# xujiabo/SCREAM

Hardware: AMD Instinct MI355X
Metric: registration pairs/sec (higher is better)
Workload: dtype f32; 1 GPU; BASELINE configs[1]: synthetic 3DMatch_test-like pairs, voxel 0.0625 m, ~5k points/cloud, batch-of-pairs=32 per GPU, A1-A10 per pair (forward 6+6 layers d_model 256, 1-NN thresh 0.1, Kabsch, RE/TE), random-init weights seed 0; lanes=1, steps_in_flight=2, parallelism=dp1 (pairs sharded, metric-row all-gather), rccl_ranks=1, gemm_backend=h2

## Files before the change

### include/scream_hip.h

```cpp
#ifndef SCREAM_HIP_H
#define SCREAM_HIP_H

#include <stdint.h>

#ifdef __cplusplus
extern "C" {
#endif

#define SCREAM_ROW_TILE 128
#define SCREAM_D_MODEL 256
#define SCREAM_NHEAD 8
#define SCREAM_HEAD_DIM 32
#define SCREAM_KV_CHUNK 256

#define SCREAM_EINVAL (-1)
#define SCREAM_EUNSUPPORTED (-2)

enum {
    SCREAM_EPI_NONE = 0,
    SCREAM_EPI_ELU1 = 1,
    SCREAM_EPI_RELU = 2,
    SCREAM_EPI_BIAS_RELU = 3,
    SCREAM_EPI_RES_LN = 4,
    SCREAM_EPI_QKV = 5
};

#define SCREAM_LAYOUT_A_FRAG 1
#define SCREAM_LAYOUT_C_FRAG 2
int scream_act_layout(const float* src, float* dst, int64_t M, int32_t to_fragment, void* stream);

const char* scream_version(void);
int scream_abi_version(void);

int scream_gemm_f32(const float* A, int64_t lda, const float* W, float* C, int64_t ldc,
                    int64_t M, int32_t N, int32_t K, int32_t epilogue, int32_t n_act,
                    const float* bias, const float* residual, int64_t ldr,
                    const float* gamma, const float* beta, void* stream);

int scream_gemm_qkv_f32(const float* A, int64_t lda, const float* W, float* Q, int64_t ldq, int64_t M,
                        int32_t N, int32_t K, int32_t n_q, const int32_t* tile_cloud,
                        const int32_t* cloud_row0, const int32_t* cloud_len, int64_t row_base,
                        float* kv_partial, void* stream);
int scream_kv_finalize(const float* kv_partial, const int32_t* cloud_row0, const int32_t* cloud_len,
                       int64_t row_base, int32_t cloud_begin, int32_t n_kv, float* kv_out, void* stream);

#define SCREAM_SPLIT_H1 1
#define SCREAM_SPLIT_H2 2
#define SCREAM_SPLIT_BF3 3
int scream_pack_w_split(const float* W, int32_t N, int32_t K, int32_t split, int32_t w_exp, void* W_packed,
                        void* stream);
int scream_gemm_split_f32(const float* A, int64_t lda, const void* W_packed, float* C, int64_t ldc, int64_t M,
                          int32_t N, int32_t K, int32_t epilogue, int32_t n_act, const float* bias,
                          const float* residual, int64_t ldr, const float* gamma, const float* beta,
                          int32_t layout, int32_t split, int32_t a_exp, int32_t w_exp, void* stream);
int scream_gemm_qkv_split_f32(const float* A, int64_t lda, const void* W_packed, float* Q, int64_t ldq,
                              int64_t M, int32_t N, int32_t K, int32_t n_q, const int32_t* tile_cloud,
                              const int32_t* cloud_row0, const int32_t* cloud_len, int64_t row_base,
                              float* kv_partial, int32_t layout, int32_t split, int32_t a_exp, int32_t w_exp,
                              int32_t k_exp, int32_t v_exp, void* stream);

int64_t scream_proj_image_bytes(int32_t N, int32_t split);
int scream_pack_proj(const float* W, int32_t N, int32_t n_q, int32_t split, int32_t w_exp, void* proj_image, void* stream);
int scream_proj_qkv_f32(const float* x, const void* proj_image, float* Q, int64_t M, int32_t N, int32_t n_q,
                        const int32_t* tile_cloud, const int32_t* cloud_row0, const int32_t* cloud_len,
                        int64_t row_base, float* kv_partial, int32_t split, int32_t a_exp, int32_t w_exp, int32_t k_exp,
                        int32_t v_exp, void* stream);

typedef struct {
    int32_t e_att, e_wm, e_m1, e_w1, e_h, e_w2;
    int32_t e_y, e_wq;
    int32_t e_q;
} scream_tail_exps_t;
int64_t scream_tail_image_bytes(int32_t split, int32_t with_next_q);
int64_t scream_kv_image_bytes(void);
int scream_pack_tail(const float* Wm, const float* W1, const float* W2, const float* Wq_next, int32_t split,
                     const scream_tail_exps_t* exps, void* tail_image, void* stream);
int scream_kv_finalize_image(const float* kv_partial, const int32_t* cloud_row0, const int32_t* cloud_len,
                          int64_t row_base, int32_t cloud_begin, int32_t n_kv, void* kv_image, int32_t n_layers,
                          int64_t partial_layer_stride, int64_t image_layer_stride, int32_t split, void* stream);
int scream_layer_tail_f32(const float* Q, const void* kv_image, const int32_t* tile_cloud,
                          int32_t kv_cloud_offset, const int32_t* cloud_len, const float* x,
                          const void* tail_image, const float* g1, const float* b1, const float* g2,
                          const float* b2, float* y, float* q_next, int64_t M, int32_t split,
                          const scream_tail_exps_t* exps, void* stream);

int scream_pe_embed_ln(const float* xyz, const int32_t* tile_cloud, const float* center,
                       const float* dim_t, const float* emb_w, const float* emb_b,
                       const float* gamma, const float* beta, float* feats, int64_t rows,
                       void* stream);
int scream_pe_embed_ln_frag(const float* xyz, const int32_t* tile_cloud, const float* center,
                            const float* dim_t, const float* emb_w, const float* emb_b,
                            const float* gamma, const float* beta, float* feats, int64_t rows,
                            void* stream);

int scream_kv_reduce(const float* Kf, const float* Vf, int64_t ld, int64_t row_base,
                     const int32_t* cloud_row0, const int32_t* cloud_len, int32_t cloud_begin,
                     int32_t n_kv, int32_t max_chunks, float* partial, float* kv_out, void* stream);

int scream_attn_apply(const float* Qf, int64_t ldq, const float* kv, const int32_t* tile_cloud,
                      int32_t kv_cloud_offset, const int32_t* cloud_len, float* out, int64_t ldo,
                      int64_t rows, void* stream);

int scream_coor_head(const float* X, const float* W, const float* b, float* out, int64_t rows,
                     void* stream);

typedef struct {
    const float* wqkv;
    const float* wq;
    const float* wkv;
    const float* wm;
    const float* w1;
    const float* w2;
    const float* g1; const float* b1;
    const float* g2; const float* b2;
    const void* tail;
    int32_t e_xq, e_xkv, e_wqkv, e_wq;
    int32_t e_k, e_v;
    scream_tail_exps_t tail_exps;
    int32_t tail_next_q;
    const void* proj;
} scream_layer_t;

typedef struct {
    int32_t n_self;
    int32_t n_cross;
    const float* dim_t;
    const float* emb_w; const float* emb_b;
    const float* pre_g; const float* pre_b;
    const scream_layer_t* layers_host;
    const float* c0_w; const float* c0_b;
    const float* c2_w; const float* c2_b;
    const float* c4_w; const float* c4_b;
    const scream_layer_t* stem_tgt_layers_host;
    int32_t gemm_split;
    int32_t e_c0x, e_c0w, e_c2x, e_c2w;
    const float* wkv_cross;
    int32_t e_wkv_cross, e_k_cross, e_v_cross;
    const void* proj_cross;
} scream_model_t;

typedef struct {
    int32_t n_pairs;
    int64_t rows_src;
    int64_t rows_total;
    int32_t max_chunks;
    const float* xyz;
    const float* center;
    const int32_t* tile_cloud;
    const int32_t* cloud_row0;
    const int32_t* cloud_len;
} scream_batch_t;

int64_t scream_forward_workspace_bytes(int64_t rows_src, int64_t rows_total, int32_t n_pairs,
                                       int32_t max_chunks, int32_t gemm_split, int32_t n_cross);

int scream_forward(const scream_model_t* model, const scream_batch_t* batch, void* workspace,
                   int64_t workspace_bytes, float* src_pred, float* feats_out, void* trace,
                   void* stream);

void* scream_trace_create(int32_t capacity);
void scream_trace_destroy(void* trace);
int scream_trace_reset(void* trace);
int scream_trace_read(void* trace, int32_t max_records, float* ms, int32_t* kind, int64_t* m,
                      int32_t* n, int32_t* k);
int scream_trace_read_starts(void* trace, int32_t max_records, float* start_ms);

int scream_nn_search(const float* query, const float* ref, const int32_t* q_row0,
                     const int32_t* q_len, const int32_t* r_row0, const int32_t* r_len,
                     const float* s, int32_t n_pairs, int32_t max_q_len, int32_t max_r_len,
                     int64_t q_rows_total, int64_t r_rows_total, float thresh, float* ref_prep,
                     uint64_t* keys, int32_t* idx, float* dmin, uint8_t* valid, void* stream);

int scream_square_distance(const float* src, const float* dst, float* out, int32_t B, int32_t N,
                           int32_t M, void* stream);

int scream_kabsch_corr(const float* src, const float* ref, const int32_t* src_row0,
                       const int32_t* src_len, const int32_t* ref_row0, const int32_t* idx,
                       const uint8_t* valid, const float* s, const float* c, int32_t n_pairs,
                       float* T_out, int32_t* n_corr, void* stream);

int scream_rigid_transform_3d(const float* A, const float* B, const float* w,
                              float weight_threshold, int32_t bs, int32_t K, float* T_out,
                              void* stream);

int scream_transformation_error(const float* T_pred, const float* T_gt, int32_t n, float* re,
                                float* te, void* stream);

int scream_point_loss(const float* src_pred, const float* src, const int32_t* src_row0, const int32_t* src_len,
                      const float* rot, const float* trans, int32_t n_pairs, float* loss, void* stream);

int64_t scream_icp_workspace_bytes(int64_t src_rows_total, int64_t ref_rows_total, int32_t n_pairs);
int scream_icp_p2p_range(const float* src, const float* ref, const int32_t* src_row0, const int32_t* src_len,
                         const int32_t* ref_row0, const int32_t* ref_len, const float* s, const float* c,
                         int32_t n_pairs, int32_t max_src_len, int32_t max_ref_len, int64_t src_rows_total,
                         int64_t ref_rows_total, float max_corr_dist, int32_t max_iter, float rel_fitness,
                         float rel_rmse, float* T, float* fitness_rmse, int32_t* iters, int32_t it_begin, int32_t it_end,
                         int32_t* done_flags, void* workspace, int64_t workspace_bytes, void* stream);
int scream_icp_p2p(const float* src, const float* ref, const int32_t* src_row0, const int32_t* src_len,
                   const int32_t* ref_row0, const int32_t* ref_len, const float* s, const float* c,
                   int32_t n_pairs, int32_t max_src_len, int32_t max_ref_len, int64_t src_rows_total,
                   int64_t ref_rows_total, float max_corr_dist, int32_t max_iter, float rel_fitness,
                   float rel_rmse, float* T, float* fitness_rmse, int32_t* iters, void* workspace,
                   int64_t workspace_bytes, void* stream);

int64_t scream_wgrad_workspace_bytes(int64_t rows, int32_t N, int32_t K);
int scream_gemm_wgrad_f32(const float* dY, int64_t ldy, const float* X, int64_t ldx, int64_t rows, int32_t N,
                          int32_t K, float* dW, int32_t accumulate, float* colsum, void* workspace,
                          int64_t workspace_bytes, void* stream);
int64_t scream_wgrad_split_workspace_bytes(int64_t rows, int32_t N, int32_t K);
int scream_gemm_wgrad_split_f32(const float* dY, int64_t ldy, const float* X, int64_t ldx, int64_t rows, int32_t N,
                                int32_t K, float* dW, int32_t accumulate, float* colsum, int32_t split, void* workspace,
                                int64_t workspace_bytes, void* stream);
int scream_ln_fwd(const float* a, const float* b, const float* gamma, const float* beta, float* y, float* mean,
                  float* rstd, int64_t rows, void* stream);
int64_t scream_ln_bwd_workspace_bytes(int64_t rows);
int scream_ln_bwd(const float* dy, const float* a, const float* b, const float* mean, const float* rstd,
                  const float* gamma, float* dz, float* dsum, float* dgamma, float* dbeta, int32_t accumulate,
                  int64_t rows, void* workspace, int64_t workspace_bytes, void* stream);
int64_t scream_attn_bwd_workspace_bytes(int32_t n_q_clouds, int32_t max_chunks);
int scream_attn_bwd(const float* Qf, int64_t ldq, int64_t q_rows, int64_t q_row_base, const float* O,
                    const float* dO, const float* Kf, const float* Vf, int64_t ldkv, int64_t kv_rows,
                    int64_t kv_row_base, const float* kv, const int32_t* tile_cloud, const int32_t* cloud_row0,
                    const int32_t* cloud_len, int32_t q_cloud_begin, int32_t n_q_clouds, int32_t kv_cloud_offset,
                    int32_t max_chunks, float* dq, int64_t lddq, float* dk, float* dv, int64_t lddkv,
                    void* workspace, int64_t workspace_bytes, void* stream);
int scream_relu_bwd(float* dy, const float* y, int64_t n, void* stream);
int scream_add_f32(float* y, const float* x, int64_t n, void* stream);
int scream_transpose_f32(const float* in, int32_t R, int32_t C, float* out, void* stream);
int scream_coor_head_bwd(const float* dout, const float* W, const float* H, float* dH, int64_t rows, void* stream);
int64_t scream_grad3_workspace_bytes(int64_t rows);
int scream_grad3(const float* w, const float* s, const float* center, const int32_t* tile_cloud, int64_t rows,
                 float* dW, int32_t transpose_w, float* col_w, float* col_s, int32_t accumulate, void* workspace,
                 int64_t workspace_bytes, void* stream);
int scream_pe_embed(const float* xyz, const int32_t* tile_cloud, const float* center, const float* dim_t,
                    const float* emb_w, const float* emb_b, float* z, int64_t rows, void* stream);

int64_t scream_render_workspace_bytes(int32_t n_pairs, int32_t n_views, int32_t w, int64_t src_rows_total);
int scream_render_depth(const float* src, const int32_t* s_row0, const int32_t* s_len, const float* tgt,
                        const int32_t* t_row0, const int32_t* t_len, int32_t n_pairs, int32_t max_s_len, int32_t max_t_len,
                        int64_t src_rows_total, const float* rot, int32_t n_views, int32_t w, float rho, float* imgs,
                        int32_t* argmax, void* workspace, int64_t workspace_bytes, void* stream);
int scream_render_depth_bwd(const float* src, const int32_t* s_row0, const int32_t* s_len, int32_t n_pairs, int32_t max_s_len,
                            int64_t src_rows_total, const float* rot, int32_t n_views, int32_t w, float rho,
                            const float* dimgs, const int32_t* argmax, void* workspace, int64_t workspace_bytes, float* dsrc,
                            void* stream);

int64_t scream_voxel_workspace_bytes(int64_t rows_total, int32_t n_clouds);
int scream_voxel_down_sample(const float* xyz, const int32_t* row0, const int32_t* len, int32_t n_clouds, int32_t max_len,
                             const double* voxel, float* out_xyz, int32_t* out_len, int32_t* out_count, void* workspace,
                             int64_t workspace_bytes, void* stream);

int64_t scream_dsm_workspace_bytes(int64_t patch_rows_total, int32_t n_clouds, int32_t max_p_len);
int scream_dsm_extract(const float* patch, const int32_t* p_row0, const int32_t* p_len, int32_t max_p_len,
                       int64_t patch_rows_total, const float* dem, const int32_t* d_row0, const int32_t* d_len, int32_t max_d_len,
                       int64_t dem_rows_total, int32_t n_clouds, float radius, float* out_xyz, int32_t* out_idx, void* workspace,
                       int64_t workspace_bytes, void* stream);
int scream_dsm_dem_assemble(const float* dsm, const float* dem, const int32_t* row0, const int32_t* len, int32_t n_clouds,
                            int32_t max_len, int64_t rows_total, float* out, float* centre, void* stream);

#ifdef __cplusplus
}
#endif
#endif
```

### scream_amd/_lib.py

```python
from __future__ import annotations

import ctypes as C
import os
from typing import Optional

_HERE = os.path.dirname(os.path.abspath(__file__))
LIB_PATH = os.environ.get("SCREAM_LIB") or os.path.join(_HERE, "libscream_hip.so")
ABI_VERSION = 21

c_f32p = C.POINTER(C.c_float)
c_i32p = C.POINTER(C.c_int32)
c_u8p = C.POINTER(C.c_uint8)
c_u64p = C.POINTER(C.c_uint64)


SPLIT_H1, SPLIT_H2, SPLIT_BF3 = 1, 2, 3


class TailExpsT(C.Structure):
    _fields_ = [(n, C.c_int32) for n in ("e_att", "e_wm", "e_m1", "e_w1", "e_h", "e_w2", "e_y", "e_wq", "e_q")]


class LayerT(C.Structure):
    _fields_ = ([(n, C.c_void_p) for n in ("wqkv", "wq", "wkv", "wm", "w1", "w2", "g1", "b1", "g2", "b2", "tail")] +
                [(n, C.c_int32) for n in ("e_xq", "e_xkv", "e_wqkv", "e_wq", "e_k", "e_v")] +
                [("tail_exps", TailExpsT), ("tail_next_q", C.c_int32), ("proj", C.c_void_p)])


class ModelT(C.Structure):
    _fields_ = [("n_self", C.c_int32), ("n_cross", C.c_int32), ("dim_t", C.c_void_p), ("emb_w", C.c_void_p),
                ("emb_b", C.c_void_p), ("pre_g", C.c_void_p), ("pre_b", C.c_void_p),
                ("layers_host", C.POINTER(LayerT)), ("c0_w", C.c_void_p), ("c0_b", C.c_void_p),
                ("c2_w", C.c_void_p), ("c2_b", C.c_void_p), ("c4_w", C.c_void_p), ("c4_b", C.c_void_p),
                ("stem_tgt_layers_host", C.POINTER(LayerT)), ("gemm_split", C.c_int32),
                ("e_c0x", C.c_int32), ("e_c0w", C.c_int32), ("e_c2x", C.c_int32), ("e_c2w", C.c_int32),
                ("wkv_cross", C.c_void_p), ("e_wkv_cross", C.c_int32), ("e_k_cross", C.c_int32), ("e_v_cross", C.c_int32),
                ("proj_cross", C.c_void_p)]


class BatchT(C.Structure):
    _fields_ = [("n_pairs", C.c_int32), ("rows_src", C.c_int64), ("rows_total", C.c_int64),
                ("max_chunks", C.c_int32), ("xyz", C.c_void_p), ("center", C.c_void_p),
                ("tile_cloud", C.c_void_p), ("cloud_row0", C.c_void_p), ("cloud_len", C.c_void_p)]


V, I32, I64, F32 = C.c_void_p, C.c_int32, C.c_int64, C.c_float
SIGNATURES = {
    "scream_version": (C.c_char_p, []),
    "scream_abi_version": (C.c_int, []),
    "scream_gemm_f32": (C.c_int, [V, I64, V, V, I64, I64, I32, I32, I32, I32, V, V, I64, V, V, V]),
    "scream_gemm_qkv_f32": (C.c_int, [V, I64, V, V, I64, I64, I32, I32, I32, V, V, V, I64, V, V]),
    "scream_kv_finalize": (C.c_int, [V, V, V, I64, I32, I32, V, V]),
    "scream_pack_w_split": (C.c_int, [V, I32, I32, I32, I32, V, V]),
    "scream_gemm_split_f32": (C.c_int, [V, I64, V, V, I64, I64, I32, I32, I32, I32, V, V, I64, V, V, I32, I32, I32, I32, V]),
    "scream_gemm_qkv_split_f32": (C.c_int, [V, I64, V, V, I64, I64, I32, I32, I32, V, V, V, I64, V, I32, I32, I32, I32, I32, I32, V]),
    "scream_proj_image_bytes": (C.c_int64, [I32, I32]),
    "scream_pack_proj": (C.c_int, [V, I32, I32, I32, I32, V, V]),
    "scream_proj_qkv_f32": (C.c_int, [V, V, V, I64, I32, I32, V, V, V, I64, V, I32, I32, I32, I32, I32, V]),
    "scream_tail_image_bytes": (C.c_int64, [I32, I32]),
    "scream_kv_image_bytes": (C.c_int64, []),
    "scream_pack_tail": (C.c_int, [V, V, V, V, I32, C.POINTER(TailExpsT), V, V]),
    "scream_kv_finalize_image": (C.c_int, [V, V, V, I64, I32, I32, V, I32, I64, I64, I32, V]),
    "scream_layer_tail_f32": (C.c_int, [V, V, V, I32, V, V, V, V, V, V, V, V, V, I64, I32, C.POINTER(TailExpsT), V]),
    "scream_act_layout": (C.c_int, [V, V, I64, I32, V]),
    "scream_pe_embed_ln": (C.c_int, [V, V, V, V, V, V, V, V, V, I64, V]),
    "scream_pe_embed_ln_frag": (C.c_int, [V, V, V, V, V, V, V, V, V, I64, V]),
    "scream_kv_reduce": (C.c_int, [V, V, I64, I64, V, V, I32, I32, I32, V, V, V]),
    "scream_attn_apply": (C.c_int, [V, I64, V, V, I32, V, V, I64, I64, V]),
    "scream_coor_head": (C.c_int, [V, V, V, V, I64, V]),
    "scream_forward_workspace_bytes": (C.c_int64, [I64, I64, I32, I32, I32, I32]),
    "scream_forward": (C.c_int, [C.POINTER(ModelT), C.POINTER(BatchT), V, I64, V, V, V, V]),
    "scream_trace_create": (C.c_void_p, [I32]),
    "scream_trace_destroy": (None, [V]),
    "scream_trace_reset": (C.c_int, [V]),
    "scream_trace_read": (C.c_int, [V, I32, V, V, V, V, V]),
    "scream_trace_read_starts": (C.c_int, [V, I32, V]),
    "scream_nn_search": (C.c_int, [V, V, V, V, V, V, V, I32, I32, I32, I64, I64, F32, V, V, V, V, V, V]),
    "scream_square_distance": (C.c_int, [V, V, V, I32, I32, I32, V]),
    "scream_kabsch_corr": (C.c_int, [V, V, V, V, V, V, V, V, V, I32, V, V, V]),
    "scream_rigid_transform_3d": (C.c_int, [V, V, V, F32, I32, I32, V, V]),
    "scream_transformation_error": (C.c_int, [V, V, I32, V, V, V]),
    "scream_point_loss": (C.c_int, [V, V, V, V, V, V, I32, V, V]),
    "scream_icp_workspace_bytes": (C.c_int64, [I64, I64, I32]),
    "scream_icp_p2p": (C.c_int, [V, V, V, V, V, V, V, V, I32, I32, I32, I64, I64, F32, I32, F32, F32, V, V, V, V, I64, V]),
    "scream_wgrad_workspace_bytes": (C.c_int64, [I64, I32, I32]),
    "scream_gemm_wgrad_f32": (C.c_int, [V, I64, V, I64, I64, I32, I32, V, I32, V, V, I64, V]),
    "scream_wgrad_split_workspace_bytes": (C.c_int64, [I64, I32, I32]),
    "scream_gemm_wgrad_split_f32": (C.c_int, [V, I64, V, I64, I64, I32, I32, V, I32, V, I32, V, I64, V]),
    "scream_ln_fwd": (C.c_int, [V, V, V, V, V, V, V, I64, V]),
    "scream_ln_bwd_workspace_bytes": (C.c_int64, [I64]),
    "scream_ln_bwd": (C.c_int, [V, V, V, V, V, V, V, V, V, V, I32, I64, V, I64, V]),
    "scream_attn_bwd_workspace_bytes": (C.c_int64, [I32, I32]),
    "scream_attn_bwd": (C.c_int, [V, I64, I64, I64, V, V, V, V, I64, I64, I64, V, V, V, V, I32, I32, I32, I32, V, I64, V, V, I64,
                                  V, I64, V]),
    "scream_relu_bwd": (C.c_int, [V, V, I64, V]),
    "scream_add_f32": (C.c_int, [V, V, I64, V]),
    "scream_transpose_f32": (C.c_int, [V, I32, I32, V, V]),
    "scream_coor_head_bwd": (C.c_int, [V, V, V, V, I64, V]),
    "scream_grad3_workspace_bytes": (C.c_int64, [I64]),
    "scream_grad3": (C.c_int, [V, V, V, V, I64, V, I32, V, V, I32, V, I64, V]),
    "scream_pe_embed": (C.c_int, [V, V, V, V, V, V, V, I64, V]),
    "scream_icp_p2p_range": (C.c_int, [V, V, V, V, V, V, V, V, I32, I32, I32, I64, I64, F32, I32, F32, F32, V, V, V, I32, I32, V, V, I64, V]),
    "scream_render_workspace_bytes": (C.c_int64, [I32, I32, I32, I64]),
    "scream_render_depth": (C.c_int, [V, V, V, V, V, V, I32, I32, I32, I64, V, I32, I32, F32, V, V, V, I64, V]),
    "scream_render_depth_bwd": (C.c_int, [V, V, V, I32, I32, I64, V, I32, I32, F32, V, V, V, I64, V, V]),
    "scream_voxel_workspace_bytes": (C.c_int64, [I64, I32]),
    "scream_voxel_down_sample": (C.c_int, [V, V, V, I32, I32, V, V, V, V, V, I64, V]),
    "scream_dsm_workspace_bytes": (C.c_int64, [I64, I32, I32]),
    "scream_dsm_extract": (C.c_int, [V, V, V, I32, I64, V, V, V, I32, I64, I32, F32, V, V, V, I64, V]),
    "scream_dsm_dem_assemble": (C.c_int, [V, V, V, V, I32, I32, I64, V, V, V]),
}

_lib: Optional[C.CDLL] = None


class ScreamHipError(RuntimeError):
    pass


def load() -> C.CDLL:
    global _lib
    if _lib is not None:
        return _lib
    if os.environ.get("SCREAM_NO_BUILD", "0") != "1" and not os.environ.get("SCREAM_LIB"):
        try:
            from . import build as _build
            _build.build()
        except Exception as e:
            if not os.path.exists(LIB_PATH):
                raise ScreamHipError("libscream_hip.so is missing and could not be built: %s" % e) from e
    if not os.path.exists(LIB_PATH):
        raise ScreamHipError("libscream_hip.so not found at %s (run `python -m scream_amd.build`)" % LIB_PATH)
    lib = C.CDLL(LIB_PATH)
    for name, (res, args) in SIGNATURES.items():
        try:
            fn = getattr(lib, name)
        except AttributeError as e:
            raise ScreamHipError("libscream_hip.so does not export %s" % name) from e
        fn.restype = res
        fn.argtypes = args
    if lib.scream_abi_version() != ABI_VERSION:
        raise ScreamHipError("libscream_hip.so ABI %d != binding ABI %d" % (lib.scream_abi_version(), ABI_VERSION))
    _lib = lib
    return lib


def check(rc: int, what: str) -> None:
    if rc == 0:
        return
    if rc == -1:
        raise ScreamHipError("%s: invalid argument (SCREAM_EINVAL)" % what)
    if rc == -2:
        raise ScreamHipError("%s: unsupported shape (SCREAM_EUNSUPPORTED)" % what)
    raise ScreamHipError("%s: HIP error %d" % (what, rc))
```

### scream_amd/csrc/forward.hip

```cpp
#include <vector>

#include "common.h"

namespace {

constexpr int D = SCREAM_D_MODEL;
constexpr int KV_ELEMS = (SCREAM_HEAD_DIM + 1) * SCREAM_HEAD_DIM;

struct Workspace {
    float *x0, *x1, *q, *att, *m1, *hid, *kvp, *kv;
    char* kvimg;
    float* kvp_cross;
    char* kvimg_cross;
    int64_t kvp_cross_stride, kvimg_cross_stride;
    int64_t bytes;
};

Workspace carve(void* base, int64_t rows_src, int64_t rows_total, int32_t n_pairs, int32_t max_chunks, int split, int32_t n_cross) {
    Workspace w;
    float* p = reinterpret_cast<float*>(base);
    auto take = [&](int64_t n) {
        float* r = p;
        p += (n + 63) / 64 * 64;
        return r;
    };
    const int64_t n_cross_batched = split ? n_cross : 0;
    w.x0 = take(rows_total * D);
    w.x1 = take(rows_total * D);
    w.q = take(rows_total * D);
    w.att = split ? nullptr : take(rows_total * D);
    w.m1 = split ? nullptr : take(rows_total * D);
    w.hid = split ? nullptr : take(rows_total * 4 * D);
    w.kvp = take(rows_total / SCREAM_ROW_TILE * SCREAM_NHEAD * KV_ELEMS);
    w.kv = take((int64_t)2 * n_pairs * SCREAM_NHEAD * KV_ELEMS);
    w.kvimg = reinterpret_cast<char*>(take((int64_t)2 * n_pairs * scream_kv_image_bytes() / 4));
    w.kvp_cross_stride = (rows_total - rows_src) / SCREAM_ROW_TILE * SCREAM_NHEAD * KV_ELEMS;
    w.kvimg_cross_stride = (int64_t)n_pairs * scream_kv_image_bytes();
    w.kvp_cross = take(n_cross_batched * w.kvp_cross_stride);
    w.kvimg_cross = reinterpret_cast<char*>(take(n_cross_batched * w.kvimg_cross_stride / 4));
    w.bytes = (p - reinterpret_cast<float*>(base)) * (int64_t)sizeof(float);
    return w;
}

struct Trace {
    std::vector<hipEvent_t> ev;
    std::vector<int32_t> kind, n, k;
    std::vector<int64_t> m;
    int count = 0;
    int capacity = 0;
};

struct Scope {
    Trace* t;
    int slot = -1;
    hipStream_t st;
    Scope(Trace* t_, int kind, int64_t m, int n, int k, void* stream) : t(t_), st(as_stream(stream)) {
        if (!t || t->count >= t->capacity) return;
        slot = t->count++;
        t->kind[slot] = kind;
        t->m[slot] = m;
        t->n[slot] = n;
        t->k[slot] = k;
        (void)hipEventRecord(t->ev[2 * slot], st);
    }
    ~Scope() {
        if (slot >= 0) (void)hipEventRecord(t->ev[2 * slot + 1], st);
    }
};

#define TRY(call)                 \
    do {                          \
        int rc_ = (call);         \
        if (rc_ != 0) return rc_; \
    } while (0)

enum { TR_TAIL_FUSED = 7, TR_EMBED = 100, TR_KV_REDUCE = 101, TR_ATTN_APPLY = 102, TR_COOR_HEAD = 103 };

struct Ctx {
    void* st;
    Trace* tr;
    int split;
    bool fp16() const { return split == SCREAM_SPLIT_H2 || split == SCREAM_SPLIT_H1; }
};

bool valid_split(int s) { return s == 0 || s == SCREAM_SPLIT_H1 || s == SCREAM_SPLIT_H2 || s == SCREAM_SPLIT_BF3; }

bool layer_ok(const Ctx& c, const scream_layer_t& L, bool cross, bool cross_stage_self) {
    if ((L.tail != nullptr) != (c.split != 0)) return false;
    if ((L.tail_next_q != 0) != (c.fp16() && cross_stage_self)) return false;
    if (c.fp16()) return cross || L.proj;
    if (c.split) return cross ? L.wq != nullptr : L.wqkv != nullptr;
    return L.wm && L.w1 && L.w2 && (cross ? L.wq && L.wkv : L.wqkv != nullptr);
}

bool model_ok(const Ctx& c, const scream_model_t& m) {
    for (int i = 0; i < m.n_self; ++i) {
        if (!layer_ok(c, m.layers_host[i], false, false)) return false;
        if (m.stem_tgt_layers_host && !layer_ok(c, m.stem_tgt_layers_host[i], false, false)) return false;
    }
    for (int i = 0; i < 2 * m.n_cross; ++i)
        if (!layer_ok(c, m.layers_host[m.n_self + i], i % 2 == 1, i % 2 == 0)) return false;
    if (m.n_cross == 0 || c.split == 0) return true;
    return c.fp16() ? m.proj_cross != nullptr : m.wkv_cross != nullptr;
}

int gemm(const Ctx& c, const float* A, int64_t lda, const float* W, float* C, int64_t ldc, int64_t M, int N, int K,
         int epi, int n_act, const float* bias, const float* res, const float* g, const float* b, int a_exp, int w_exp,
         int layout = 0) {
    Scope sc(c.tr, epi, M, N, K, c.st);
    if (c.split)
        return scream_gemm_split_f32(A, lda, W, C, ldc, M, N, K, epi, n_act, bias, res, D, g, b, layout, c.split, a_exp, w_exp, c.st);
    return scream_gemm_f32(A, lda, W, C, ldc, M, N, K, epi, n_act, bias, res, D, g, b, c.st);
}

int gemm_qkv(const Ctx& c, const float* A, const float* W, const void* proj, float* Q, int64_t M, int N, int n_q, const scream_batch_t& b,
             int64_t row_base, float* kvp, int a_exp, int w_exp, int k_exp, int v_exp) {
    Scope sc(c.tr, 5, M, N, D, c.st);
    if (c.fp16())
        return scream_proj_qkv_f32(A, proj, Q, M, N, n_q, b.tile_cloud, b.cloud_row0, b.cloud_len, row_base, kvp, c.split, a_exp, w_exp,
                                   k_exp, v_exp, c.st);
    if (c.split)
        return scream_gemm_qkv_split_f32(A, D, W, Q, D, M, N, D, n_q, b.tile_cloud, b.cloud_row0, b.cloud_len, row_base, kvp,
                                         SCREAM_LAYOUT_A_FRAG | (n_q ? SCREAM_LAYOUT_C_FRAG : 0), c.split, a_exp, w_exp, k_exp, v_exp,
                                         c.st);
    return scream_gemm_qkv_f32(A, D, W, Q, D, M, N, D, n_q, b.tile_cloud, b.cloud_row0, b.cloud_len, row_base, kvp, c.st);
}

int apply_and_tail_f32(const Ctx& c, const scream_layer_t& L, const scream_batch_t& b, const Workspace& w, const float* x, float* y,
                       int64_t row0, int64_t rows, int32_t kv_cloud_offset) {
    float* att = w.att + row0 * D;
    float* m1 = w.m1 + row0 * D;
    float* hid = w.hid + row0 * 4 * D;
    {
        Scope sc(c.tr, TR_ATTN_APPLY, rows, 0, 0, c.st);
        TRY(scream_attn_apply(w.q + row0 * D, D, w.kv, b.tile_cloud + row0 / SCREAM_ROW_TILE, kv_cloud_offset, b.cloud_len, att, D, rows,
                              c.st));
    }
    TRY(gemm(c, att, D, L.wm, m1, D, rows, D, D, SCREAM_EPI_RES_LN, 0, nullptr, x, L.g1, L.b1, 0, 0));
    TRY(gemm(c, m1, D, L.w1, hid, 4 * D, rows, 4 * D, D, SCREAM_EPI_RELU, 0, nullptr, nullptr, nullptr, nullptr, 0, 0));
    TRY(gemm(c, hid, 4 * D, L.w2, y, D, rows, D, 4 * D, SCREAM_EPI_RES_LN, 0, nullptr, x, L.g2, L.b2, 0, 0));
    return 0;
}

int mha_self(const Ctx& c, const scream_layer_t& L, const scream_batch_t& b, const Workspace& w, const float* x,
             float* y, int64_t row0, int64_t rows, int32_t cloud_begin, int32_t n_clouds) {
    const float* xr = x + row0 * D;
    float* qr = w.q + row0 * D;
    float* kvp = w.kvp + row0 / SCREAM_ROW_TILE * SCREAM_NHEAD * KV_ELEMS;
    TRY(gemm_qkv(c, xr, L.wqkv, L.proj, qr, rows, 3 * D, D, b, row0, kvp, L.e_xq, L.e_wqkv, L.e_k, L.e_v));
    if (c.split) {
        {
            Scope sc(c.tr, TR_KV_REDUCE, rows, 0, 0, c.st);
            TRY(scream_kv_finalize_image(kvp, b.cloud_row0, b.cloud_len, row0, cloud_begin, n_clouds, w.kvimg, 1, 0, 0, c.split, c.st));
        }
        Scope sc(c.tr, TR_TAIL_FUSED, rows, (L.tail_next_q ? 10 : 9) * D, D, c.st);
        return scream_layer_tail_f32(qr, w.kvimg, b.tile_cloud + row0 / SCREAM_ROW_TILE, 0, b.cloud_len, xr, L.tail, L.g1,
                                     L.b1, L.g2, L.b2, y + row0 * D, L.tail_next_q ? qr : nullptr, rows, c.split, &L.tail_exps, c.st);
    }
    {
        Scope sc(c.tr, TR_KV_REDUCE, rows, 0, 0, c.st);
        TRY(scream_kv_finalize(kvp, b.cloud_row0, b.cloud_len, row0, cloud_begin, n_clouds, w.kv, c.st));
    }
    return apply_and_tail_f32(c, L, b, w, xr, y + row0 * D, row0, rows, 0);
}

int cross_kv_all(const Ctx& c, const scream_model_t& m, const scream_batch_t& b, const Workspace& w, const float* x_tgt) {
    const int64_t rs = b.rows_src, rt = b.rows_total - b.rows_src;
    const scream_layer_t& L0 = m.layers_host[m.n_self + 1];
    TRY(gemm_qkv(c, x_tgt, m.wkv_cross, m.proj_cross, nullptr, rt, 2 * D * m.n_cross, 0, b, rs, w.kvp_cross, L0.e_xkv, m.e_wkv_cross, m.e_k_cross,
                 m.e_v_cross));
    Scope sc(c.tr, TR_KV_REDUCE, rt, 0, 0, c.st);
    return scream_kv_finalize_image(w.kvp_cross, b.cloud_row0, b.cloud_len, rs, b.n_pairs, b.n_pairs,
                                 w.kvimg_cross - (int64_t)b.n_pairs * scream_kv_image_bytes(), m.n_cross, w.kvp_cross_stride,
                                 w.kvimg_cross_stride, c.split, c.st);
}

int mha_cross(const Ctx& c, const scream_layer_t& L, const scream_batch_t& b, const Workspace& w, const float* x_src,
              const float* x_tgt, float* y, const char* kvimg_layer) {
    const int64_t rs = b.rows_src, rt = b.rows_total - b.rows_src;
    if (!c.fp16())
        TRY(gemm(c, x_src, D, L.wq, w.q, D, rs, D, D, SCREAM_EPI_ELU1, D, nullptr, nullptr, nullptr, nullptr, L.e_xq, L.e_wq,
                 c.split ? (SCREAM_LAYOUT_A_FRAG | SCREAM_LAYOUT_C_FRAG) : 0));
    if (c.split) {
        Scope sc(c.tr, TR_TAIL_FUSED, rs, 9 * D, D, c.st);
        return scream_layer_tail_f32(w.q, kvimg_layer, b.tile_cloud, 0, b.cloud_len + b.n_pairs, x_src, L.tail, L.g1, L.b1, L.g2,
                                     L.b2, y, nullptr, rs, c.split, &L.tail_exps, c.st);
    }
    TRY(gemm_qkv(c, x_tgt, L.wkv, nullptr, nullptr, rt, 2 * D, 0, b, rs, w.kvp, 0, 0, 0, 0));
    {
        Scope sc(c.tr, TR_KV_REDUCE, rt, 0, 0, c.st);
        TRY(scream_kv_finalize(w.kvp, b.cloud_row0, b.cloud_len, rs, b.n_pairs, b.n_pairs, w.kv, c.st));
    }
    return apply_and_tail_f32(c, L, b, w, x_src, y, 0, rs, b.n_pairs);
}

}

extern "C" const char* scream_version(void) { return "scream_hip gfx950 abi21"; }
extern "C" int scream_abi_version(void) { return 21; }

extern "C" void* scream_trace_create(int32_t capacity) {
    if (capacity <= 0) return nullptr;
    Trace* t = new Trace();
    t->capacity = capacity;
    t->ev.resize(2 * (size_t)capacity);
    t->kind.resize(capacity);
    t->n.resize(capacity);
    t->k.resize(capacity);
    t->m.resize(capacity);
    for (auto& e : t->ev) {
        if (hipEventCreate(&e) != hipSuccess) {
            delete t;
            return nullptr;
        }
    }
    return t;
}

extern "C" void scream_trace_destroy(void* trace) {
    Trace* t = reinterpret_cast<Trace*>(trace);
    if (!t) return;
    for (auto& e : t->ev) (void)hipEventDestroy(e);
    delete t;
}

extern "C" int scream_trace_reset(void* trace) {
    SCREAM_REQUIRE(trace, SCREAM_EINVAL);
    reinterpret_cast<Trace*>(trace)->count = 0;
    return 0;
}

extern "C" int scream_trace_read(void* trace, int32_t max_records, float* ms, int32_t* kind, int64_t* m, int32_t* n,
                                 int32_t* k) {
    SCREAM_REQUIRE(trace && ms && kind && m && n && k && max_records >= 0, SCREAM_EINVAL);
    Trace* t = reinterpret_cast<Trace*>(trace);
    const int cnt = t->count < max_records ? t->count : max_records;
    for (int i = 0; i < cnt; ++i) {
        if (hipEventElapsedTime(&ms[i], t->ev[2 * i], t->ev[2 * i + 1]) != hipSuccess) return SCREAM_EINVAL;
        kind[i] = t->kind[i];
        m[i] = t->m[i];
        n[i] = t->n[i];
        k[i] = t->k[i];
    }
    return cnt;
}

extern "C" int scream_trace_read_starts(void* trace, int32_t max_records, float* start_ms) {
    SCREAM_REQUIRE(trace && start_ms && max_records >= 0, SCREAM_EINVAL);
    Trace* t = reinterpret_cast<Trace*>(trace);
    const int cnt = t->count < max_records ? t->count : max_records;
    for (int i = 0; i < cnt; ++i)
        if (hipEventElapsedTime(&start_ms[i], t->ev[0], t->ev[2 * i]) != hipSuccess) return SCREAM_EINVAL;
    return cnt;
}

extern "C" int64_t scream_forward_workspace_bytes(int64_t rows_src, int64_t rows_total, int32_t n_pairs,
                                                  int32_t max_chunks, int32_t gemm_split, int32_t n_cross) {
    if (rows_src < 0 || rows_total < rows_src || n_pairs < 0 || max_chunks < 0 || !valid_split(gemm_split) || n_cross < 0) return SCREAM_EINVAL;
    return carve(nullptr, rows_src, rows_total, n_pairs, max_chunks, gemm_split, n_cross).bytes + 256;
}

extern "C" int scream_forward(const scream_model_t* model, const scream_batch_t* batch, void* workspace,
                              int64_t workspace_bytes, float* src_pred, float* feats_out, void* trace, void* stream) {
    SCREAM_REQUIRE(model && batch && workspace && src_pred, SCREAM_EINVAL);
    const scream_model_t& m = *model;
    const scream_batch_t& b = *batch;
    SCREAM_REQUIRE(m.layers_host && m.n_self >= 0 && m.n_cross >= 0 && valid_split(m.gemm_split), SCREAM_EINVAL);
    SCREAM_REQUIRE(b.n_pairs > 0 && b.rows_src > 0 && b.rows_total > b.rows_src && b.max_chunks > 0, SCREAM_EINVAL);
    SCREAM_REQUIRE(b.rows_src % SCREAM_ROW_TILE == 0 && b.rows_total % SCREAM_ROW_TILE == 0, SCREAM_EUNSUPPORTED);
    SCREAM_REQUIRE(b.xyz && b.center && b.tile_cloud && b.cloud_row0 && b.cloud_len, SCREAM_EINVAL);
    const Ctx c{stream, reinterpret_cast<Trace*>(trace), m.gemm_split};
    SCREAM_REQUIRE(model_ok(c, m), SCREAM_EINVAL);
    uintptr_t base = (reinterpret_cast<uintptr_t>(workspace) + 255) & ~(uintptr_t)255;
    const Workspace w = carve(reinterpret_cast<void*>(base), b.rows_src, b.rows_total, b.n_pairs, b.max_chunks, c.split, m.n_cross);
    SCREAM_REQUIRE((int64_t)(base - reinterpret_cast<uintptr_t>(workspace)) + w.bytes <= workspace_bytes, SCREAM_EINVAL);

    const int64_t rs = b.rows_src, ra = b.rows_total;
    {
        Scope sc(c.tr, TR_EMBED, ra, 0, 0, stream);
        if (c.split)
            TRY(scream_pe_embed_ln_frag(b.xyz, b.tile_cloud, b.center, m.dim_t, m.emb_w, m.emb_b, m.pre_g, m.pre_b, w.x0, ra, stream));
        else
            TRY(scream_pe_embed_ln(b.xyz, b.tile_cloud, b.center, m.dim_t, m.emb_w, m.emb_b, m.pre_g, m.pre_b, w.x0, ra, stream));
    }
    float* cur = w.x0;
    float* nxt = w.x1;
    for (int i = 0; i < m.n_self; ++i) {
        if (!m.stem_tgt_layers_host) {
            TRY(mha_self(c, m.layers_host[i], b, w, cur, nxt, 0, ra, 0, 2 * b.n_pairs));
        } else {
            TRY(mha_self(c, m.layers_host[i], b, w, cur, nxt, 0, rs, 0, b.n_pairs));
            TRY(mha_self(c, m.stem_tgt_layers_host[i], b, w, cur, nxt, rs, ra - rs, b.n_pairs, b.n_pairs));
        }
        float* t = cur;
        cur = nxt;
        nxt = t;
    }
    const float* x_tgt = cur + rs * D;
    if (c.split && m.n_cross > 0) TRY(cross_kv_all(c, m, b, w, x_tgt));
    for (int i = 0; i < 2 * m.n_cross; ++i) {
        const scream_layer_t& L = m.layers_host[m.n_self + i];
        if (i % 2 == 0)
            TRY(mha_self(c, L, b, w, cur, nxt, 0, rs, 0, b.n_pairs));
        else
            TRY(mha_cross(c, L, b, w, cur, x_tgt, nxt, c.split ? w.kvimg_cross + (i / 2) * w.kvimg_cross_stride : nullptr));
        float* t = cur;
        cur = nxt;
        nxt = t;
    }
    float* c_mid = c.split ? w.q : w.m1;
    float* c_out = c.split ? nxt : w.att;
    TRY(gemm(c, cur, D, m.c0_w, c_mid, D, rs, D, D, SCREAM_EPI_BIAS_RELU, 0, m.c0_b, nullptr, nullptr, nullptr, m.e_c0x, m.e_c0w,
             c.split ? SCREAM_LAYOUT_A_FRAG : 0));
    TRY(gemm(c, c_mid, D, m.c2_w, c_out, D, rs, D, D, SCREAM_EPI_BIAS_RELU, 0, m.c2_b, nullptr, nullptr, nullptr, m.e_c2x, m.e_c2w));
    {
        Scope sc(c.tr, TR_COOR_HEAD, rs, 0, 0, stream);
        TRY(scream_coor_head(c_out, m.c4_w, m.c4_b, src_pred, rs, stream));
    }
    if (feats_out && c.split) {
        TRY(scream_act_layout(cur, feats_out, rs, 0, stream));
    } else if (feats_out) {
        hipError_t e = hipMemcpyAsync(feats_out, cur, (size_t)rs * D * sizeof(float), hipMemcpyDeviceToDevice,
                                      as_stream(stream));
        if (e != hipSuccess) return (int)e;
    }
    return 0;
}
```

### scream_amd/csrc/tail_split.hip

```cpp
#include <type_traits>

#include "ring.h"

namespace {

constexpr int T_RIDE0 = 3;
constexpr int T_STASH = 3;
constexpr int T_DEFER_H2 = 2;

constexpr int TAIL_STAGES = 72;
constexpr int NEXT_Q_STAGES = 8;
constexpr int KV_PLANES_BYTES = 8 * 3 * 2 * 1024;
constexpr int KV_IMAGE_BYTES = KV_PLANES_BYTES + 8 * 32 * 4;

constexpr int KV_H2_HEAD_BYTES = 2 * 2 * 1024;
constexpr int KV_H2_SCALE_OFF = 8 * KV_H2_HEAD_BYTES;

struct HeadOps {
    f32x4 kv[6];
    f32x4 ks[4];
    f32x4 sc;
};

struct TailScales {
    float s_att;
    int e_q;
    int e_att;
    float c1;
    float eps1;
    float s_m1;
    float ch;
    float c2;
    float eps2;
    float s_y;
    float cq;
};

__device__ __forceinline__ constexpr int xadd_slot(int h, int g, int nd) {
    int n = 0;
    for (int c = 15 - nd; c >= 8; --c) {
        if ((c >> 1) == h - 1) continue;
        if (c == g) return n < 4 ? n : -1;
        ++n;
    }
    return -1;
}

template <class SP, bool NQ>
__global__ __launch_bounds__(TT, 1) void tail_kernel(const float* __restrict__ Q,
                                                     const char* __restrict__ kvimg,
                                                     const int32_t* __restrict__ tile_cloud, int kv_cloud_offset,
                                                     const int32_t* __restrict__ cloud_len,
                                                     const float* __restrict__ xres,
                                                     const char* __restrict__ Wimg,
                                                     const float* __restrict__ g1, const float* __restrict__ b1,
                                                     const float* __restrict__ g2, const float* __restrict__ b2,
                                                     float* __restrict__ y,
                                                     float* q_next,
                                                     int n_tiles, TailScales sc) {
    static_assert(!NQ || SP::SCALED, "the next-layer query projection is built for the fp16 splits");
    constexpr int N_STAGES = TAIL_STAGES + (NQ ? NEXT_Q_STAGES : 0);
    typedef typename SP::vec V;
    constexpr int NP = SP::NP;
    constexpr int STAGE = stage_bytes<SP>();
    constexpr int PIECES = wave_pieces<SP>();
    constexpr bool APPLY_H2 = SP::SCALED;
    constexpr int NV_MERGE = SP::NPROD >= 6 ? 6 : 8;
    constexpr int ND = SP::NPROD >= 6 ? 1 : T_DEFER_H2;
    constexpr int NG = 16 - ND;
    constexpr int NSTASH = NP == 2 ? T_STASH : 0;
    __shared__ __attribute__((aligned(16))) char smem[T_SLOTS * STAGE + 4096 + NSTASH * 16384];
    const int tid = threadIdx.x, lane = tid & 63;
    const int wave = __builtin_amdgcn_readfirstlane(tid >> 6);
    const int half = lane >> 5;
    float* lnp = reinterpret_cast<float*>(smem + T_SLOTS * STAGE);
    f32x4* stash = reinterpret_cast<f32x4*>(smem + T_SLOTS * STAGE + 4096 + wave * (NSTASH * 4096)) + lane;
    lnp[tid] = SP::SCALED ? g1[tid] * sc.s_m1 : g1[tid];
    lnp[256 + tid] = SP::SCALED ? b1[tid] * sc.s_m1 : b1[tid];
    lnp[512 + tid] = g2[tid];
    lnp[768 + tid] = b2[tid];
    const float eps1 = SP::SCALED ? sc.eps1 : 1e-5f, eps2 = SP::SCALED ? sc.eps2 : 1e-5f;
    const unsigned v_lane16 = lane * 16, v_half16 = half * 16;
    auto dma_piece = [&](unsigned q, int u) {
        const unsigned src = q % (unsigned)N_STAGES, slot = q % (unsigned)T_SLOTS;
        const char* sbase = Wimg + (size_t)src * STAGE + (wave * PIECES + (u & ~3)) * 1024;
        dma_1k(sbase + v_lane16, smem + slot * STAGE + (wave * PIECES + (u & ~3)) * 1024, u & 3);
    };
    unsigned q = 0;
#pragma unroll
    for (int u = 0; u < PIECES; ++u) dma_piece(0, u);
#pragma unroll
    for (int u = 0; u < PIECES; ++u) dma_piece(1, u);

    auto seg_base = [&](const float* base, int64_t grp, int seg) { return base + grp + seg * 1024; };
    auto req_q = [&](f32x4 (&qb)[4], int64_t grp, int h) {
        ld_asm4<1024, true>(qb, seg_base(Q, grp, h), v_lane16);
    };
    auto req_head = [&](HeadOps& o, const char* kvc, int h) {
        f32x4 (&kv4)[4] = reinterpret_cast<f32x4 (&)[4]>(o.kv[0]);
        if (APPLY_H2) {
            ld_asm4<1024>(kv4, kvc + h * KV_H2_HEAD_BYTES, v_lane16);
            asm volatile("global_load_dwordx4 %0, %1, %2" : "=v"(o.sc) : "v"(v_half16), "s"(kvc + KV_H2_SCALE_OFF + 32 * h));
        } else {
            const char* kp = kvc + h * (3 * 2 * 1024);
            ld_asm4<1024>(kv4, kp, v_lane16);
            ld_asm2k(o.kv[4], o.kv[5], kp + 4 * 1024, v_lane16);
        }
        ld_asm4<32>(o.ks, kvc + KV_PLANES_BYTES + 128 * h, v_half16);
    };
    auto req_x = [&](f32x4 (&xs)[4], int64_t grp, int blk, auto second) {
        ld_asm4<1024, decltype(second)::value>(xs, seg_base(xres, grp, blk), v_lane16);
    };
    auto pin_head = [&](HeadOps& o) {
#pragma unroll
        for (int a = 0; a < 4; ++a) pin(o.ks[a]);
#pragma unroll
        for (int f = 0; f < (APPLY_H2 ? 4 : 6); ++f) pin(o.kv[f]);
        if (APPLY_H2) pin(o.sc);
    };
    auto add_x4 = [&](f32x16& t, const f32x4 (&xs)[4], int a, float c) {
#pragma unroll
        for (int k = 0; k < 4; ++k) t[4 * a + k] = SP::SCALED ? __builtin_fmaf(xs[a][k], c, t[4 * a + k]) : t[4 * a + k] + xs[a][k];
    };
    auto pin_x = [&](f32x4 (&xs)[4]) {
#pragma unroll
        for (int a = 0; a < 4; ++a) pin(xs[a]);
    };
    auto add_x = [&](f32x16& t, const f32x4 (&xs)[4], float c) {
#pragma unroll
        for (int a = 0; a < 4; ++a) add_x4(t, xs, a, c);
    };

    HeadOps op;
    f32x4 qA[4], qB[4];
    f32x4 xs[4], xs2[4];
    V apA[2][NP], apB[2][NP];
    f32x16 aT;
    bf16x8 qp[2][3];
    f16x8 qph[2][2];
    float Zs = 0.f;
    int tq = 0;

    auto apply_qscale = [&](const f32x4 (&qb)[4]) {
        float m = 0.f;
#pragma unroll
        for (int a = 0; a < 4; ++a)
#pragma unroll
            for (int k = 0; k < 4; ++k) m = fmaxf(m, qb[a][k]);
        m = fmaxf(m, __shfl_xor(m, 32));
        const int hb = (int)(__float_as_uint(op.sc[0]) >> 23);
        tq = min(max(14 - ((int)(__float_as_uint(m) >> 23) - 127), sc.e_q), min(127, sc.e_att + hb - 1));
    };
    auto apply_qsplit = [&](f32x4 (&qb)[4], int s2) {
        const f32x4 lo = qb[2 * s2], hi = qb[2 * s2 + 1];
        if (APPLY_H2) split8s<SplitH2>(lo, hi, __uint_as_float((uint32_t)(tq + 127) << 23), qph[s2]);
        else split8<SplitBf3>(lo, hi, qp[s2]);
    };
    auto apply_mfma = [&](int s2) {
        if (APPLY_H2) {
            f16x8 w[2];
#pragma unroll
            for (int p = 0; p < 2; ++p) w[p] = __builtin_bit_cast(f16x8, op.kv[p * 2 + s2]);
            mfma_group<SplitH2, -1>(aT, w, qph[s2], s2 == 0);
        } else {
            bf16x8 w[3];
#pragma unroll
            for (int p = 0; p < 3; ++p) w[p] = __builtin_bit_cast(bf16x8, op.kv[p * 2 + s2]);
            mfma_group<SplitBf3, -1>(aT, w, qp[s2], s2 == 0);
        }
    };
    auto apply_z = [&](f32x4 (&qb)[4]) {
        float zp = 0.f;
#pragma unroll
        for (int a = 0; a < 4; ++a)
#pragma unroll
            for (int k = 0; k < 4; ++k) zp += qb[a][k] * op.ks[a][k];
        zp += __shfl_xor(zp, 32);
        Zs = 1.0f / (zp + 1e-6f);
        if (APPLY_H2) Zs *= __uint_as_float((uint32_t)(sc.e_att - tq + (int)(__float_as_uint(op.sc[0]) >> 23)) << 23);
        else if (SP::SCALED) Zs *= sc.s_att;
    };
    auto apply_split_pair = [&](int k, V (&ap)[2][NP], float S) {
        const int s2 = k >> 2, j = (2 * k) & 7;
#pragma unroll
        for (int e = 0; e < 2; ++e) SP::split1((aT[2 * k + e] * Zs) * S, j + e, ap[s2]);
    };
    auto apply_ride = [&](f32x4 (&qb)[4], int g, V (&ap)[2][NP], float S) {
        if (g == 0 && APPLY_H2) apply_qscale(qb);
        if (g == 0) apply_qsplit(qb, 0);
        if (g == 1) apply_qsplit(qb, 1);
        if (g == 1) apply_mfma(0);
        if (g == 2) apply_mfma(1);
        if (g == 3) apply_z(qb);
        if (g >= 4 && g < 12) apply_split_pair(g - 4, ap, S);
    };

    int tile = blockIdx.x;
    int64_t grp = ((int64_t)tile * 128 + wave * 32) * SCREAM_D_MODEL;
    const char* kvc = nullptr;
    float S = 1.f;
    if (tile < n_tiles) {
        const int cl = tile_cloud[tile] + kv_cloud_offset;
        kvc = kvimg + (size_t)cl * KV_IMAGE_BYTES;
        S = (float)cloud_len[cl];
    }
    if (tile < n_tiles) {
#pragma unroll
        for (int h = 0; h < 2; ++h) {
            req_q(qA, grp, h);
            req_head(op, kvc, h);
            VM_WAIT(0);
            pin_x(qA);
            pin_head(op);
#pragma unroll
            for (int g = 0; g < 12; ++g) apply_ride(qA, g, h == 0 ? apA : apB, S);
        }
    }

    while (tile < n_tiles) {
        V wfd[ND][NP];
        f32x16 acc[8];
        auto ring_groups = [&](auto flush, auto body) __attribute__((always_inline)) {
            const char* wb = smem + (q % T_SLOTS) * STAGE + lane * 16;
            V wf[T_PF][NP];
#pragma unroll
            for (int g0 = 0; g0 < T_PF - 1; ++g0)
#pragma unroll
                for (int p = 0; p < NP; ++p) wf[g0][p] = ld_frag<V>(wb + (p * 16 + g0) * 1024);
            flush();
#pragma unroll
            for (int g = 0; g < NG; ++g) {
                if (g + T_PF - 1 < 16) {
#pragma unroll
                    for (int p = 0; p < NP; ++p)
                        (g + T_PF - 1 >= NG ? wfd[g + T_PF - 1 - NG][p] : wf[(g + T_PF - 1) % T_PF][p]) = ld_frag<V>(wb + (p * 16 + g + T_PF - 1) * 1024);
                }
                body(g, wf[g % T_PF]);
            }
            ++q;
        };
        const int tile_next = tile + (int)gridDim.x;
        const bool has_next = tile_next < n_tiles;
        const int64_t grp_next = ((int64_t)(has_next ? tile_next : tile) * 128 + wave * 32) * SCREAM_D_MODEL;
        const char* kvc_next = kvc;
        float S_next = 1.f;
        if (has_next) {
            const int cl = tile_cloud[tile_next] + kv_cloud_offset;
            kvc_next = kvimg + (size_t)cl * KV_IMAGE_BYTES;
            S_next = (float)cloud_len[cl];
        }

        auto stage_merge = [&](auto hh, V (&ap)[2][NP], V (&ap_next)[2][NP], f32x4 (&q_cons)[4], f32x4 (&q_req)[4], auto flush) {
            constexpr int h = decltype(hh)::value;
            constexpr bool RIDE = h >= 1 && h <= 6;
            if (h == 0) { if (NQ) ring_barrier<0>(); else lds_only_barrier(); }
            else ring_barrier<PIECES>();
            __builtin_amdgcn_sched_barrier(0);
            f32x4 (&x_prev)[4] = (h & 1) ? xs : xs2;
            f32x4 (&x_req)[4] = (h & 1) ? xs2 : xs;
            if (h > 0) {
                pin_x(x_prev);
                if (h - 1 < NSTASH) {
#pragma unroll
                    for (int a = 0; a < 4; ++a) stash[((h - 1) * 4 + a) * 64] = x_prev[a];
                }
                if (RIDE) {
                    pin_head(op);
                    pin_x(q_cons);
                }
            }
            __builtin_amdgcn_sched_barrier(0);
            req_x(x_req, grp, h, std::false_type{});
            if (h + 2 < 8) req_q(q_req, grp, h + 2);
            if (h == 0) req_head(op, kvc, 2);
            __builtin_amdgcn_sched_barrier(0);
            ring_groups(flush, [&](int g, const V (&w)[NP]) __attribute__((always_inline)) {
                if (g == 4 && RIDE && h + 2 < 8) {
                    __builtin_amdgcn_sched_barrier(0);
                    req_head(op, kvc, h + 2);
                    __builtin_amdgcn_sched_barrier(0);
                }
                if (g >= 4 && g - 4 < PIECES) dma_piece(q + 2, g - 4);
                if (PIECES == 12 && g == 14) dma_piece(q + 2, 11);
                if (RIDE) apply_ride(q_cons, g, ap_next, S);
                if (h > 0) {
                    const int pc = xadd_slot(h, g, ND);
                    if (pc >= 0) add_x4(acc[h > 0 ? h - 1 : 0], x_prev, pc, sc.c1);
                }
                mfma_group<SP, (h > 0 ? NV_MERGE : 0)>(acc[g >> 1], w, ap[g & 1], h == 0 && (g & 1) == 0);
            });
        };
        constexpr std::integral_constant<bool, true> yes{};
        constexpr std::integral_constant<bool, false> no{};
#define HEAD(n) std::integral_constant<int, n>{}
        auto flush_none = [&]() {};
        auto flush_acc7 = [&](V (&b)[2][NP], bool first) {
#pragma unroll
            for (int i = 0; i < ND; ++i) mfma_group<SP, -1>(acc[7], wfd[i], b[(NG + i) & 1], first && ((NG + i) & 1) == 0);
        };
        auto flush_mergeA = [&]() { flush_acc7(apA, false); };
        auto flush_mergeB = [&]() { flush_acc7(apB, false); };
        auto flush_mergeA0 = [&]() { flush_acc7(apA, true); };
        stage_merge(HEAD(0), apA, apB, qB, qA, flush_none);
        stage_merge(HEAD(1), apB, apA, qA, qB, flush_mergeA0);
        stage_merge(HEAD(2), apA, apB, qB, qA, flush_mergeB);
        stage_merge(HEAD(3), apB, apA, qA, qB, flush_mergeA);
        stage_merge(HEAD(4), apA, apB, qB, qA, flush_mergeB);
        stage_merge(HEAD(5), apB, apA, qA, qB, flush_mergeA);
        stage_merge(HEAD(6), apA, apB, qB, qA, flush_mergeB);
        stage_merge(HEAD(7), apB, apA, qA, qB, flush_mergeA);
        flush_mergeB();
        vm_wait<PIECES>();
        pin_x(xs2);
        add_x(acc[7], xs2, sc.c1);

        V mp[16][NP];
        {
            float sum = 0.f;
#pragma unroll
            for (int b = 0; b < 8; ++b)
#pragma unroll
                for (int e = 0; e < 16; ++e) sum += acc[b][e];
            sum += __shfl_xor(sum, 32);
            const float mean = sum * (1.0f / 256.0f);
            float var = 0.f;
#pragma unroll
            for (int b = 0; b < 8; ++b)
#pragma unroll
                for (int e = 0; e < 16; ++e) {
                    acc[b][e] -= mean;
                    var += acc[b][e] * acc[b][e];
                }
            var += __shfl_xor(var, 32);
            const float rstd = 1.0f / sqrtf(var * (1.0f / 256.0f) + eps1);
            const float* gp = lnp + 4 * half;
            const float* bp = lnp + 256 + 4 * half;
#pragma unroll
            for (int b = 0; b < 8; ++b)
#pragma unroll
                for (int s2 = 0; s2 < 2; ++s2) {
                    f32x4 v[2];
#pragma unroll
                    for (int a2 = 0; a2 < 2; ++a2) {
                        const int a = 2 * s2 + a2;
                        const f32x4 g4 = ld4(gp + 32 * b + 8 * a), b4 = ld4(bp + 32 * b + 8 * a);
#pragma unroll
                        for (int k = 0; k < 4; ++k) v[a2][k] = acc[b][4 * a + k] * rstd * g4[k] + b4[k];
                    }
                    split8<SP>(v[0], v[1], mp[2 * b + s2]);
                }
        }

        f32x16 hT;
        V hpA[2][NP], hpB[2][NP];
        auto split_pair = [&](int k, V (&hout)[2][NP]) {
            const int s2 = k >> 2, j = (2 * k) & 7;
            float x0, x1;
            asm("v_max_f32 %0, 0, %1" : "=v"(x0) : "v"(hT[2 * k]));
            asm("v_max_f32 %0, 0, %1" : "=v"(x1) : "v"(hT[2 * k + 1]));
            if constexpr (SP::SCALED) {
                SP::split2s(x0, x1, sc.ch, j, hout[s2]);
            } else {
                SP::split1(x0, j, hout[s2]);
                SP::split1(x1, j + 1, hout[s2]);
            }
        };
        auto stage_up = [&](auto first, auto xload, auto flush) {
            constexpr int XLOAD = decltype(xload)::value;
            if (decltype(first)::value) ring_barrier<0>(); else ring_barrier<PIECES>();
            __builtin_amdgcn_sched_barrier(0);
            if (XLOAD >= 0 && XLOAD < NSTASH) {
#pragma unroll
                for (int a = 0; a < 4; ++a) xs[a] = stash[(XLOAD * 4 + a) * 64];
            } else if (XLOAD >= 0) req_x(xs, grp, XLOAD, std::true_type{});
            __builtin_amdgcn_sched_barrier(0);
            ring_groups(flush, [&](int g, const V (&w)[NP]) __attribute__((always_inline)) {
                if (g < PIECES) dma_piece(q + 2, g);
                mfma_group<SP>(hT, w, mp[g], g == 0);
            });
        };
        auto stage_down = [&](V (&hin)[2][NP], V (&hout)[2][NP], auto with_split, auto xadd, auto ride, auto flush) {
            constexpr int XADD = decltype(xadd)::value;
            constexpr int RIDE = decltype(ride)::value;
            ring_barrier<PIECES>();
            __builtin_amdgcn_sched_barrier(0);
            if (XADD == 0) {
                pin_x(xs);
#pragma unroll
                for (int a = 0; a < 4; ++a)
#pragma unroll
                    for (int k = 0; k < 4; ++k) acc[0][4 * a + k] = SP::SCALED ? xs[a][k] * sc.c2 : xs[a][k];
            } else if (XADD > 0) {
                pin_x(xs);
                add_x(acc[XADD > 0 ? XADD : 0], xs, sc.c2);
            }
            if (RIDE == 2) {
                pin_head(op);
                pin_x(qA);
            }
            __builtin_amdgcn_sched_barrier(0);
            if (RIDE == 1) {
                req_q(qA, grp_next, 0);
                req_head(op, kvc_next, 0);
            }
            __builtin_amdgcn_sched_barrier(0);
            ring_groups(flush, [&](int g, const V (&w)[NP]) __attribute__((always_inline)) {
                if (RIDE == 2 && g == 4) {
                    __builtin_amdgcn_sched_barrier(0);
                    req_q(qA, grp_next, 1);
                    req_head(op, kvc_next, 1);
                    __builtin_amdgcn_sched_barrier(0);
                }
                if (RIDE == 2) {
                    if (g >= 4 && g - 4 < PIECES) dma_piece(q + 2, g - 4);
                    if (PIECES == 12 && g == 14) dma_piece(q + 2, 11);
                } else {
                    if (g < PIECES) dma_piece(q + 2, g);
                }
                if (RIDE == 2) apply_ride(qA, g, apA, S_next);
                if (decltype(with_split)::value && (ND == 1 ? (g & 1) == 0 : (g >= T_RIDE0 && g < T_RIDE0 + 8))) split_pair(ND == 1 ? g >> 1 : g - T_RIDE0, hout);
                mfma_group<SP>(acc[g >> 1], w, hin[g & 1], XADD == 0 && g >= 2 && (g & 1) == 0);
            });
        };
        constexpr std::integral_constant<int, -1> none{};
        constexpr std::integral_constant<int, 0> ride0{};
        auto flush_up = [&]() {
#pragma unroll
            for (int i = 0; i < ND; ++i) mfma_group<SP, -1>(hT, wfd[i], mp[NG + i]);
        };
        auto flush_downA = [&]() { flush_acc7(hpA, false); };
        auto flush_downB = [&]() { flush_acc7(hpB, false); };
        auto flush_downA0 = [&]() { flush_acc7(hpA, true); };
        stage_up(yes, none, flush_none);
        flush_up();
#pragma unroll
        for (int k = 0; k < 8; ++k) split_pair(k, hpA);
#define PAIR(c, fl, flA)                                                                    \
        stage_up(no, HEAD((c) - 1), fl);                                        \
        stage_down(hpA, hpB, yes, HEAD((c) - 1), ride0, flush_up);  \
        stage_up(no, HEAD(c), flA);                                         \
        stage_down(hpB, hpA, yes, HEAD(c), ride0, flush_up);
        PAIR(1, flush_none, flush_downA0) PAIR(3, flush_downB, flush_downA) PAIR(5, flush_downB, flush_downA) PAIR(7, flush_downB, flush_downA)
#undef PAIR
        for (int c = 9; c < 31; c += 2) {
            stage_up(no, none, flush_downB);
            stage_down(hpA, hpB, yes, none, ride0, flush_up);
            stage_up(no, none, flush_downA);
            stage_down(hpB, hpA, yes, none, ride0, flush_up);
        }
        stage_up(no, none, flush_downB);
        stage_down(hpA, hpB, yes, none, HEAD(1), flush_up);
        stage_down(hpB, hpA, no, none, HEAD(2), flush_downA);
        flush_downB();
#undef HEAD
        VM_WAIT(0);
        if (has_next) {
            pin_head(op);
            pin_x(qA);
#pragma unroll
            for (int g = 0; g < 12; ++g) apply_ride(qA, g, apB, S_next);
        }

        V yp[NQ ? 16 : 1][NP];
        {
            float sum = 0.f;
#pragma unroll
            for (int b = 0; b < 8; ++b)
#pragma unroll
                for (int e = 0; e < 16; ++e) sum += acc[b][e];
            sum += __shfl_xor(sum, 32);
            const float mean = sum * (1.0f / 256.0f);
            float var = 0.f;
#pragma unroll
            for (int b = 0; b < 8; ++b)
#pragma unroll
                for (int e = 0; e < 16; ++e) {
                    acc[b][e] -= mean;
                    var += acc[b][e] * acc[b][e];
                }
            var += __shfl_xor(var, 32);
            const float rstd = 1.0f / sqrtf(var * (1.0f / 256.0f) + eps2);
            const float* gp = lnp + 512 + 4 * half;
            const float* bp = lnp + 768 + 4 * half;
            float* yg = y + grp + lane * 4;
#pragma unroll
            for (int b = 0; b < 8; ++b)
#pragma unroll
                for (int s2 = 0; s2 < 2; ++s2) {
                    f32x4 o2[2];
#pragma unroll
                    for (int a2 = 0; a2 < 2; ++a2) {
                        const int a = 2 * s2 + a2;
                        const f32x4 g4 = ld4(gp + 32 * b + 8 * a), b4 = ld4(bp + 32 * b + 8 * a);
                        f32x4 o;
#pragma unroll
                        for (int k = 0; k < 4; ++k) o[k] = acc[b][4 * a + k] * rstd * g4[k] + b4[k];
                        __builtin_nontemporal_store(o, reinterpret_cast<f32x4*>(yg + (b * 4 + a) * 256));
                        o2[a2] = o;
                    }
                    if (NQ) split8<SP>(o2[0] * sc.s_y, o2[1] * sc.s_y, yp[NQ ? 2 * b + s2 : 0]);
                }
        }
        if constexpr (NQ) {
            f32x16 hq[2];
            f32x4 oq[4];
            float* qg = q_next + grp + lane * 4;
            auto elu_pair = [&](int k, const f32x16& h) {
#pragma unroll
                for (int e = 0; e < 2; ++e) {
                    const int i = 2 * k + e;
                    const float x = h[i] * sc.cq;
                    oq[i >> 2][i & 3] = elu1(x);
                }
            };
            auto store_chunk = [&](int j) {
#pragma unroll
                for (int a = 0; a < 4; ++a) __builtin_nontemporal_store(oq[a], reinterpret_cast<f32x4*>(qg + (j * 4 + a) * 256));
            };
            constexpr int PP = (PIECES + NG - 9) / (NG - 8);
            auto stage_q = [&](auto jj) {
                constexpr int j = decltype(jj)::value;
                if (j == 0) lds_only_barrier(); else ring_barrier<PIECES>();
                __builtin_amdgcn_sched_barrier(0);
                auto flush_q = [&]() {
                    if (j > 0) {
#pragma unroll
                        for (int i = 0; i < ND; ++i) mfma_group<SP, -1>(hq[(j + 1) & 1], wfd[i], yp[NG + i]);
                    }
                };
                ring_groups(flush_q, [&](int g, const V (&w)[NP]) __attribute__((always_inline)) {
                    if (j > 0 && g < 8) elu_pair(g, hq[(j + 1) & 1]);
                    if (g == 8) {
                        __builtin_amdgcn_sched_barrier(0);
                        if (j > 0) store_chunk(j - 1);
                        __builtin_amdgcn_sched_barrier(0);
                    }
                    if (g >= 8) {
#pragma unroll
                        for (int u = (g - 8) * PP; u < (g - 7) * PP; ++u)
                            if (u < PIECES) dma_piece(q + 2, u);
                    }
                    mfma_group<SP, 8>(hq[j & 1], w, yp[g], g == 0);
                });
            };
            stage_q(std::integral_constant<int, 0>{});
            stage_q(std::integral_constant<int, 1>{});
            stage_q(std::integral_constant<int, 2>{});
            stage_q(std::integral_constant<int, 3>{});
            stage_q(std::integral_constant<int, 4>{});
            stage_q(std::integral_constant<int, 5>{});
            stage_q(std::integral_constant<int, 6>{});
            stage_q(std::integral_constant<int, 7>{});
#pragma unroll
            for (int i = 0; i < ND; ++i) mfma_group<SP, -1>(hq[1], wfd[i], yp[NG + i]);
#pragma unroll
            for (int k = 0; k < 8; ++k) elu_pair(k, hq[1]);
            store_chunk(7);
        }
        tile = tile_next;
        grp = ((int64_t)tile_next * 128 + wave * 32) * SCREAM_D_MODEL;
        kvc = kvc_next;
        S = S_next;
    }
    VM_WAIT(0);
}

__global__ __launch_bounds__(256) void act_layout_kernel(const float* __restrict__ src, float* __restrict__ dst, int to_frag) {
    __shared__ float tile[32][260];
    const int t = threadIdx.x;
    const float* s = src + (int64_t)blockIdx.x * 8192;
    float* d = dst + (int64_t)blockIdx.x * 8192;
#pragma unroll
    for (int i = 0; i < 8; ++i) {
        const int e = t + 256 * i;
        const f32x4 v = *reinterpret_cast<const f32x4*>(s + e * 4);
        int row, col;
        if (to_frag) {
            row = e >> 6, col = (e & 63) * 4;
        } else {
            const int ln = e & 63, a = (e >> 6) & 3, blk = e >> 8;
            row = ln & 31, col = 32 * blk + 8 * a + 4 * (ln >> 5);
        }
        *reinterpret_cast<f32x4*>(&tile[row][col]) = v;
    }
    __syncthreads();
#pragma unroll
    for (int i = 0; i < 8; ++i) {
        const int e = t + 256 * i;
        int row, col;
        if (to_frag) {
            const int ln = e & 63, a = (e >> 6) & 3, blk = e >> 8;
            row = ln & 31, col = 32 * blk + 8 * a + 4 * (ln >> 5);
        } else {
            row = e >> 6, col = (e & 63) * 4;
        }
        *reinterpret_cast<f32x4*>(d + e * 4) = *reinterpret_cast<const f32x4*>(&tile[row][col]);
    }
}

template <class SP>
__global__ void pack_tail_kernel(const float* __restrict__ Wm, const float* __restrict__ W1, const float* __restrict__ W2,
                                 const float* __restrict__ Wq_next, float s_wm, float s_w1, float s_w2, float s_wq,
                                 typename SP::vec* __restrict__ out) {
    const int t = blockIdx.x * blockDim.x + threadIdx.x;
    if (t >= (TAIL_STAGES + (Wq_next ? NEXT_Q_STAGES : 0)) * 16 * 64) return;
    const int lane = t & 63, frag = (t >> 6) & 15, stage = t >> 10;
    const int m = lane & 31, half = lane >> 5;
    float v[8];
    float s;
    if (stage < 8) {
        s = s_wm;
#pragma unroll
        for (int j = 0; j < 8; ++j) v[j] = Wm[(int64_t)(32 * (frag >> 1) + m) * 256 + 32 * stage + chunk_k(frag & 1, half, j)];
    } else if (stage >= TAIL_STAGES) {
        s = s_wq;
#pragma unroll
        for (int j = 0; j < 8; ++j) v[j] = Wq_next[(int64_t)(32 * (stage - TAIL_STAGES) + m) * 256 + 32 * (frag >> 1) + chunk_k(frag & 1, half, j)];
    } else {
        const int st = stage - 8;
        const bool up = st == 0 || (st < 63 && (st & 1));
        const int c = st == 0 ? 0 : st == 63 ? 31 : up ? (st + 1) / 2 : st / 2 - 1;
        s = up ? s_w1 : s_w2;
        if (up) {
#pragma unroll
            for (int j = 0; j < 8; ++j) v[j] = W1[(int64_t)(32 * c + m) * 256 + 32 * (frag >> 1) + chunk_k(frag & 1, half, j)];
        } else {
#pragma unroll
            for (int j = 0; j < 8; ++j) v[j] = W2[(int64_t)(32 * (frag >> 1) + m) * 1024 + 32 * c + chunk_k(frag & 1, half, j)];
        }
    }
    typename SP::vec p[SP::NP];
#pragma unroll
    for (int j = 0; j < 8; ++j) SP::split1(SP::SCALED ? v[j] * s : v[j], j, p);
#pragma unroll
    for (int pl = 0; pl < SP::NP; ++pl) out[(((int64_t)stage * SP::NP + pl) * 16 + frag) * 64 + lane] = p[pl];
}

constexpr int KVF_THREADS = 320;

template <bool H2>
__global__ __launch_bounds__(KVF_THREADS) void kv_finalize_image_kernel(const float* __restrict__ partial,
                                                                      const int32_t* __restrict__ cloud_row0,
                                                                      const int32_t* __restrict__ cloud_len, int64_t row_base,
                                                                      int cloud_begin, char* __restrict__ kvimg,
                                                                      int64_t partial_layer_stride, int64_t image_layer_stride) {
    constexpr int KV_ELEMS = (SCREAM_HEAD_DIM + 1) * SCREAM_HEAD_DIM;
    static_assert(KV_ELEMS % 4 == 0 && KV_ELEMS / 4 <= KVF_THREADS, "");
    __shared__ float wmax[KVF_THREADS / 64];
    const int i4 = threadIdx.x;
    const bool active = i4 < KV_ELEMS / 4;
    const int kvi = blockIdx.x / SCREAM_NHEAD, h = blockIdx.x % SCREAM_NHEAD;
    const int cloud = cloud_begin + kvi;
    partial += (int64_t)blockIdx.y * partial_layer_stride;
    kvimg += (int64_t)blockIdx.y * image_layer_stride;
    const int t0 = (int)((cloud_row0[cloud] - row_base) / SCREAM_ROW_TILE);
    const int nt = (cloud_len[cloud] + SCREAM_ROW_TILE - 1) / SCREAM_ROW_TILE;
    const float* p = partial + ((int64_t)t0 * SCREAM_NHEAD + h) * KV_ELEMS + 4 * (active ? i4 : 0);
    char* img = kvimg + (size_t)cloud * KV_IMAGE_BYTES;
    const float S = (float)cloud_len[cloud];
    f32x4 s8[16];
#pragma unroll
    for (int u = 0; u < 16; ++u) s8[u] = f32x4{0.f, 0.f, 0.f, 0.f};
    if (active) {
        for (int c = 0; c < nt; c += 16) {
#pragma unroll
            for (int u = 0; u < 16; ++u)
                if (c + u < nt) s8[u] += *reinterpret_cast<const f32x4*>(p + (int64_t)(c + u) * SCREAM_NHEAD * KV_ELEMS);
        }
    }
#pragma unroll
    for (int u = 0; u < 8; ++u) s8[u] += s8[u + 8];
    const f32x4 s4 = ((s8[0] + s8[1]) + (s8[2] + s8[3])) + ((s8[4] + s8[5]) + (s8[6] + s8[7]));
    const bool is_kv = 4 * i4 < 32 * 32;
    f32x4 x4;
#pragma unroll
    for (int e = 0; e < 4; ++e) x4[e] = s4[e] / S;
    float scale = 1.f;
    if (H2) {
        float m = (active && is_kv) ? fmaxf(fmaxf(fabsf(x4[0]), fabsf(x4[1])), fmaxf(fabsf(x4[2]), fabsf(x4[3]))) : 0.f;
#pragma unroll
        for (int o = 32; o >= 1; o >>= 1) m = fmaxf(m, __shfl_xor(m, o));
        if ((threadIdx.x & 63) == 0) wmax[threadIdx.x >> 6] = m;
        __syncthreads();
        m = wmax[0];
#pragma unroll
        for (int w = 1; w < KVF_THREADS / 64; ++w) m = fmaxf(m, wmax[w]);
        const uint32_t mb = __float_as_uint(m);
        int eh = 15 - ((int)(mb >> 23) - 127) - ((mb & 0x7fffffu) ? 1 : 0);
        if (!(m >= 1.17549435e-38f) || eh > 40) eh = 40;
        if (eh < -30) eh = -30;
        scale = __uint_as_float((uint32_t)(eh + 127) << 23);
        if (threadIdx.x < 8) reinterpret_cast<float*>(img + KV_H2_SCALE_OFF)[h * 8 + threadIdx.x] = __uint_as_float((uint32_t)(127 - eh) << 23);
    }
    if (!active) return;
#pragma unroll
    for (int e = 0; e < 4; ++e) {
        const int i = 4 * i4 + e;
        if (is_kv) {
            const int d = i >> 5, v = i & 31;
            const float x = x4[e];
            const int s2 = d >> 4, hf = (d >> 2) & 1, j = 4 * ((d >> 3) & 1) + (d & 3);
            if (H2) {
                const _Float16 a = (_Float16)(x * scale);
                const _Float16 b = (_Float16)__builtin_fmaf(x, scale, -(float)a);
                _Float16* base = reinterpret_cast<_Float16*>(img) + ((size_t)(h * 2) * 2 + s2) * 512 + (v + 32 * hf) * 8 + j;
                base[0] = a;
                base[2 * 512] = b;
            } else {
                const __bf16 a = (__bf16)x;
                const float r1 = x - (float)a;
                const __bf16 b = (__bf16)r1;
                const __bf16 cc = (__bf16)(r1 - (float)b);
                __bf16* base = reinterpret_cast<__bf16*>(img) + ((size_t)(h * 3) * 2 + s2) * 512 + (v + 32 * hf) * 8 + j;
                base[0] = a;
                base[2 * 512] = b;
                base[4 * 512] = cc;
            }
        } else {
            reinterpret_cast<float*>(img + KV_PLANES_BYTES)[h * 32 + (i - 32 * 32)] = s4[e];
        }
    }
}

bool split_ok(int32_t split) { return split == SCREAM_SPLIT_BF3 || split == SCREAM_SPLIT_H2 || split == SCREAM_SPLIT_H1; }

bool tail_scales(const scream_tail_exps_t* ex, TailScales* sc) {
    if (!ex) return false;
    const int es[6] = {ex->e_att, ex->e_wm, ex->e_m1, ex->e_w1, ex->e_h, ex->e_w2};
    for (int e : es)
        if (e < -40 || e > 40) return false;
    const int e1 = ex->e_wm + ex->e_att, e2 = ex->e_w2 + ex->e_h, eh = ex->e_h - ex->e_w1 - ex->e_m1;
    if (e1 < -44 || e1 > 44 || e2 < -44 || e2 > 44 || eh < -100 || eh > 100) return false;
    if (ex->e_q < -40 || ex->e_q > 40) return false;
    sc->s_att = exp2i(ex->e_att);
    sc->e_q = ex->e_q;
    sc->e_att = ex->e_att;
    sc->c1 = exp2i(e1);
    sc->eps1 = 1e-5f * exp2i(2 * e1);
    sc->s_m1 = exp2i(ex->e_m1);
    sc->ch = exp2i(eh);
    sc->c2 = exp2i(e2);
    sc->eps2 = 1e-5f * exp2i(2 * e2);
    if (ex->e_y < -40 || ex->e_y > 40 || ex->e_wq < -40 || ex->e_wq > 40) return false;
    sc->s_y = exp2i(ex->e_y);
    sc->cq = exp2i(-ex->e_y - ex->e_wq);
    return true;
}

}

extern "C" int64_t scream_tail_image_bytes(int32_t split, int32_t with_next_q) {
    if (!split_ok(split) || (with_next_q && split == SCREAM_SPLIT_BF3)) return SCREAM_EINVAL;
    return (int64_t)(TAIL_STAGES + (with_next_q ? NEXT_Q_STAGES : 0)) * split * 16 * 1024;
}
extern "C" int64_t scream_kv_image_bytes(void) { return KV_IMAGE_BYTES; }

extern "C" int scream_pack_tail(const float* Wm, const float* W1, const float* W2, const float* Wq_next, int32_t split,
                                const scream_tail_exps_t* exps, void* image, void* stream) {
    SCREAM_REQUIRE(Wm && W1 && W2 && image && split_ok(split), SCREAM_EINVAL);
    SCREAM_REQUIRE(!Wq_next || split != SCREAM_SPLIT_BF3, SCREAM_EUNSUPPORTED);
    SCREAM_REQUIRE((reinterpret_cast<uintptr_t>(image) & 15) == 0, SCREAM_EINVAL);
    const dim3 grid((TAIL_STAGES + (Wq_next ? NEXT_Q_STAGES : 0)) * 16 * 64 / 256), block(256);
    if (split != SCREAM_SPLIT_BF3) {
        TailScales sc;
        SCREAM_REQUIRE(tail_scales(exps, &sc), SCREAM_EINVAL);
        if (split == SCREAM_SPLIT_H2)
            pack_tail_kernel<SplitH2><<<grid, block, 0, as_stream(stream)>>>(Wm, W1, W2, Wq_next, exp2i(exps->e_wm), exp2i(exps->e_w1),
                                                                             exp2i(exps->e_w2), exp2i(exps->e_wq), reinterpret_cast<f16x8*>(image));
        else
            pack_tail_kernel<SplitH1><<<grid, block, 0, as_stream(stream)>>>(Wm, W1, W2, Wq_next, exp2i(exps->e_wm), exp2i(exps->e_w1),
                                                                             exp2i(exps->e_w2), exp2i(exps->e_wq), reinterpret_cast<f16x8*>(image));
    } else {
        pack_tail_kernel<SplitBf3><<<grid, block, 0, as_stream(stream)>>>(Wm, W1, W2, nullptr, 1.f, 1.f, 1.f, 1.f, reinterpret_cast<bf16x8*>(image));
    }
    SCREAM_LAUNCH_CHECK();
    return 0;
}

extern "C" int scream_kv_finalize_image(const float* kv_partial, const int32_t* cloud_row0, const int32_t* cloud_len,
                                        int64_t row_base, int32_t cloud_begin, int32_t n_kv, void* kv_image, int32_t n_layers,
                                        int64_t partial_layer_stride, int64_t image_layer_stride, int32_t split, void* stream) {
    SCREAM_REQUIRE(kv_partial && cloud_row0 && cloud_len && kv_image && split_ok(split), SCREAM_EINVAL);
    SCREAM_REQUIRE(n_kv >= 0 && cloud_begin >= 0 && row_base >= 0 && n_layers >= 1 && n_layers <= 65535, SCREAM_EINVAL);
    SCREAM_REQUIRE(n_layers == 1 || (partial_layer_stride > 0 && image_layer_stride > 0 && image_layer_stride % 16 == 0), SCREAM_EINVAL);
    SCREAM_REQUIRE(((reinterpret_cast<uintptr_t>(kv_image) | reinterpret_cast<uintptr_t>(kv_partial)) & 15) == 0 && partial_layer_stride % 4 == 0,
                   SCREAM_EINVAL);
    if (n_kv == 0) return 0;
    const dim3 grid(n_kv * SCREAM_NHEAD, n_layers), block(KVF_THREADS);
    if (split != SCREAM_SPLIT_BF3)
        kv_finalize_image_kernel<true><<<grid, block, 0, as_stream(stream)>>>(kv_partial, cloud_row0, cloud_len, row_base, cloud_begin,
                                                                              reinterpret_cast<char*>(kv_image), partial_layer_stride, image_layer_stride);
    else
        kv_finalize_image_kernel<false><<<grid, block, 0, as_stream(stream)>>>(kv_partial, cloud_row0, cloud_len, row_base, cloud_begin,
                                                                               reinterpret_cast<char*>(kv_image), partial_layer_stride, image_layer_stride);
    SCREAM_LAUNCH_CHECK();
    return 0;
}

namespace {
template <class SP, bool NQ>
void launch_tail(unsigned grid, hipStream_t st, const float* Q, const void* kv_image, const int32_t* tile_cloud, int32_t kv_cloud_offset,
                 const int32_t* cloud_len, const float* x, const void* tail_image, const float* g1, const float* b1, const float* g2,
                 const float* b2, float* y, float* q_next, int tiles, const TailScales& sc) {
    tail_kernel<SP, NQ><<<dim3(grid), dim3(TT), 0, st>>>(Q, reinterpret_cast<const char*>(kv_image), tile_cloud, kv_cloud_offset, cloud_len, x,
                                                     reinterpret_cast<const char*>(tail_image), g1, b1, g2, b2, y, q_next, tiles, sc);
}
}

extern "C" int scream_layer_tail_f32(const float* Q, const void* kv_image, const int32_t* tile_cloud,
                                     int32_t kv_cloud_offset, const int32_t* cloud_len, const float* x,
                                     const void* tail_image, const float* g1, const float* b1, const float* g2,
                                     const float* b2, float* y, float* q_next, int64_t M, int32_t split,
                                     const scream_tail_exps_t* exps, void* stream) {
    SCREAM_REQUIRE(Q && kv_image && tile_cloud && cloud_len && x && tail_image && g1 && b1 && g2 && b2 && y && split_ok(split), SCREAM_EINVAL);
    SCREAM_REQUIRE(M >= 0 && M % SCREAM_ROW_TILE == 0, SCREAM_EUNSUPPORTED);
    SCREAM_REQUIRE(((reinterpret_cast<uintptr_t>(Q) | reinterpret_cast<uintptr_t>(kv_image) | reinterpret_cast<uintptr_t>(x) |
                     reinterpret_cast<uintptr_t>(tail_image) | reinterpret_cast<uintptr_t>(g1) | reinterpret_cast<uintptr_t>(b1) |
                     reinterpret_cast<uintptr_t>(g2) | reinterpret_cast<uintptr_t>(b2) | reinterpret_cast<uintptr_t>(y) |
                     reinterpret_cast<uintptr_t>(q_next)) & 15) == 0, SCREAM_EINVAL);
    SCREAM_REQUIRE(x != y, SCREAM_EINVAL);
    SCREAM_REQUIRE(!q_next || (split != SCREAM_SPLIT_BF3 && q_next != x && q_next != y), SCREAM_EINVAL);
    TailScales sc{1.f, 0, 0, 1.f, 1e-5f, 1.f, 1.f, 1.f, 1e-5f, 1.f, 1.f};
    if (split != SCREAM_SPLIT_BF3) SCREAM_REQUIRE(tail_scales(exps, &sc), SCREAM_EINVAL);
    const int64_t tiles = M / SCREAM_ROW_TILE;
    if (tiles == 0) return 0;
    SCREAM_REQUIRE(tiles < (1ll << 31), SCREAM_EUNSUPPORTED);
    const unsigned grid = tiles < T_MAX_GRID ? (unsigned)tiles : (unsigned)T_MAX_GRID;
    hipStream_t st = as_stream(stream);
#define TAIL_ARGS grid, st, Q, kv_image, tile_cloud, kv_cloud_offset, cloud_len, x, tail_image, g1, b1, g2, b2, y, q_next, (int)tiles, sc
    if (split == SCREAM_SPLIT_H2) {
        if (q_next) launch_tail<SplitH2, true>(TAIL_ARGS);
        else launch_tail<SplitH2, false>(TAIL_ARGS);
    } else if (split == SCREAM_SPLIT_H1) {
        if (q_next) launch_tail<SplitH1, true>(TAIL_ARGS);
        else launch_tail<SplitH1, false>(TAIL_ARGS);
    } else {
        launch_tail<SplitBf3, false>(TAIL_ARGS);
    }
#undef TAIL_ARGS
    SCREAM_LAUNCH_CHECK();
    return 0;
}

extern "C" int scream_act_layout(const float* src, float* dst, int64_t M, int32_t to_fragment, void* stream) {
    SCREAM_REQUIRE(src && dst && src != dst, SCREAM_EINVAL);
    SCREAM_REQUIRE(M >= 0 && M % 32 == 0 && M / 32 < (1ll << 31), SCREAM_EUNSUPPORTED);
    SCREAM_REQUIRE(((reinterpret_cast<uintptr_t>(src) | reinterpret_cast<uintptr_t>(dst)) & 15) == 0, SCREAM_EINVAL);
    if (M == 0) return 0;
    act_layout_kernel<<<dim3((unsigned)(M / 32)), dim3(256), 0, as_stream(stream)>>>(src, dst, to_fragment ? 1 : 0);
    SCREAM_LAUNCH_CHECK();
    return 0;
}
```

### scream_amd/model.py

```python
from __future__ import annotations

import ctypes as C
import os
from typing import List, Optional, Sequence, Tuple

import torch
from torch import nn

from . import _lib, ops, scales
from .packing import PackedBatch
from .render import RegistrationRender

D_MODEL = 256
NHEAD = 8

for _retired in ("SCREAM_FUSED_TAIL", "SCREAM_BATCHED_CROSS_KV", "SCREAM_FUSE_NEXT_Q", "SCREAM_RING_PROJ"):
    if os.environ.get(_retired) == "0":
        raise ValueError("%s=0 no longer selects anything: the switch was removed and every forward runs the schedule it used to "
                         "default to; unset it" % _retired)


class _MHAParams(nn.Module):

    def __init__(self, d_model: int, nhead: int = NHEAD):
        super().__init__()
        self.q_proj = nn.Linear(d_model, d_model, bias=False)
        self.k_proj = nn.Linear(d_model, d_model, bias=False)
        self.v_proj = nn.Linear(d_model, d_model, bias=False)
        self.merge = nn.Linear(d_model, d_model, bias=False)
        self.mlp = nn.Sequential(nn.Linear(d_model, d_model * 4, bias=False), nn.ReLU(True),
                                 nn.Linear(d_model * 4, d_model, bias=False))
        self.norm1 = nn.LayerNorm(d_model)
        self.norm2 = nn.LayerNorm(d_model)


class _CrossParams(nn.Module):

    def __init__(self, d_model: int, nhead: int = NHEAD):
        super().__init__()
        self.layer = _MHAParams(d_model, nhead)
        for p in self.parameters():
            if p.dim() > 1:
                nn.init.xavier_uniform_(p)


def pe_dim_t(d_model: int = D_MODEL) -> torch.Tensor:
    npf = d_model // 3 // 2 * 2
    i = torch.arange(npf, dtype=torch.float32)
    return 10000 ** (2 * torch.trunc(torch.div(i, 2)) / npf)


class _Pack:

    def __init__(self, backend, sig, mt, layers, keep, event, streams):
        self.backend, self.sig, self.mt, self.layers, self.keep = backend, sig, mt, layers, keep
        self.event, self.streams = event, streams


class PointTransformer(nn.Module):
    def __init__(self, d_model: int = 256, self_layer_num: int = 6, cross_layer_num: int = 6):
        super().__init__()
        if d_model != D_MODEL:
            raise NotImplementedError("the gfx950 kernels are built for d_model=256 (8 heads x 32), the only "
                                      "configuration the reference evaluates (evaluate_3d_match.py:188)")
        self.embedding = nn.Conv1d(3, d_model, kernel_size=1, stride=1)
        self.pre_norm = nn.LayerNorm(d_model)
        self.self_layer_num = self_layer_num
        self.cross_layer_num = cross_layer_num
        self.stem = nn.ModuleList([_MHAParams(d_model) for _ in range(self_layer_num)])
        self.cross = nn.ModuleList()
        for _ in range(cross_layer_num):
            self.cross.append(_MHAParams(d_model))
            self.cross.append(_CrossParams(d_model))
        self.coor_mlp = nn.Sequential(nn.Conv1d(d_model, d_model, 1), nn.ReLU(), nn.Conv1d(d_model, d_model, 1),
                                      nn.ReLU(), nn.Conv1d(d_model, 3, 1))
        self.generator = RegistrationRender(rho=24, w=64)
        self._packs = {}
        self._ws = None

    def _layer_modules(self) -> List[_MHAParams]:
        mods = list(self.stem)
        for i, m in enumerate(self.cross):
            mods.append(m if i % 2 == 0 else m.layer)
        return mods

    def _stem_tgt_modules(self) -> Optional[List[_MHAParams]]:
        return None

    gemm_backend = os.environ.get("SCREAM_GEMM", "h2")

    TRAIN_BACKENDS = ("f32", "split")
    _train_backend_default = os.environ.get("SCREAM_TRAIN_GEMM", "f32")

    @classmethod
    def _check_train_backend(cls, value):
        if value not in cls.TRAIN_BACKENDS:
            raise ValueError("train_backend must be one of %s, got %r" % (", ".join(repr(b) for b in cls.TRAIN_BACKENDS), value))
        return value

    @property
    def train_backend(self) -> str:
        return self.__dict__.get("_train_backend", type(self)._train_backend_default)

    @train_backend.setter
    def train_backend(self, value: str) -> None:
        self.__dict__["_train_backend"] = self._check_train_backend(value)

    fused_tail = True
    fuse_next_q = True

    def _signature(self):
        return tuple((p.data_ptr(), p._version) for p in self.parameters())

    def _layer_inputs(self):
        ln = lambda n: (n.weight, n.bias)
        mods, tgt_mods = self._layer_modules(), self._stem_tgt_modules()
        ns = self.self_layer_num
        pre = ln(self.pre_norm)
        ins, prev = [], pre
        for i in range(ns):
            ins.append((prev, prev))
            prev = ln(mods[i].norm2)
        src_in = prev
        tgt_ins, prev_t = [], pre
        for m in (tgt_mods or []):
            tgt_ins.append((prev_t, prev_t))
            prev_t = ln(m.norm2)
        tgt_in = prev_t if tgt_mods else src_in
        for j in range(2 * self.cross_layer_num):
            ins.append((src_in, src_in if j % 2 == 0 else tgt_in))
            src_in = ln(mods[ns + j].norm2)
        return ins, tgt_ins, src_in

    def _pack_weights(self, backend: Optional[str] = None) -> "_Pack":
        backend = self.gemm_backend if backend is None else backend
        if backend not in ("h2", "x3", "f32", "h1"):
            raise ValueError("gemm_backend must be 'h2', 'x3', 'f32' or 'h1', got %r" % (backend,))
        sig = self._signature()
        if self._packs and next(iter(self._packs.values())).sig != sig:
            torch.cuda.synchronize(self.embedding.weight.device) if self.embedding.weight.is_cuda else None
            self._packs = {}
        pk = self._packs.get(backend)
        if pk is not None:
            return pk
        try:
            pk = self._build_pack(backend, sig)
        except scales.ScaleRangeError as e:
            if backend != "h2":
                raise
            import warnings
            warnings.warn("scream_amd: gemm_backend 'h2' cannot carry these weights (%s); using 'x3' (bf16 x 3 split, scale free, "
                          "same fp32-level accuracy at twice the matrix instructions)" % (e,), RuntimeWarning, stacklevel=3)
            pk = self._pack_weights("x3")
        self._packs[backend] = pk
        return pk

    def _build_pack(self, backend: str, sig) -> "_Pack":
        dev = self.embedding.weight.device
        if dev.type != "cuda":
            raise _lib.ScreamHipError("PointTransformer must be on the MI355X (net.to('cuda:0')) before forward; "
                                      "scream_amd has no CPU path")
        keep = []

        def dev_f32(t):
            t = t.detach().to(device=dev, dtype=torch.float32).contiguous()
            keep.append(t)
            return t.data_ptr()

        split = {"h2": _lib.SPLIT_H2, "x3": _lib.SPLIT_BF3, "f32": 0, "h1": _lib.SPLIT_H1}[backend]
        fp16_split = split in (_lib.SPLIT_H2, _lib.SPLIT_H1)
        f32 = lambda t: t.detach().to(device=dev, dtype=torch.float32)

        def dev_mat(t):
            if not split:
                return dev_f32(t), 0
            pw = ops.pack_w(f32(t), split)
            keep.append(pw.data)
            return pw.data_ptr(), pw.w_exp

        def dev_proj(t, n_q):
            pp = ops.pack_proj(f32(t), n_q, split)
            keep.append(pp.data)
            return pp.data_ptr(), pp.w_exp

        mods = self._layer_modules()
        tgt_mods = self._stem_tgt_modules() or []
        ins, tgt_ins, coor_in = self._layer_inputs()
        layers = (_lib.LayerT * len(mods))()
        tgt_layers = (_lib.LayerT * max(len(tgt_mods), 1))()
        ns = self.self_layer_num
        is_cross = [i >= ns and (i - ns) % 2 == 1 for i in range(len(mods))] + [False] * len(tgt_mods)
        next_cross = {id(mods[i]): i + 1 for i in range(ns, len(mods) - 1, 2)} if fp16_split else {}
        for L, m, (in_q, in_kv), cross in zip(list(layers) + list(tgt_layers), mods + tgt_mods, ins + tgt_ins, is_cross):
            k, v = m.k_proj.weight, m.v_proj.weight
            wkv = torch.cat([k[:128], v[:128], k[128:], v[128:]], dim=0)
            wqkv = torch.cat([m.q_proj.weight, wkv], dim=0)
            if fp16_split:
                if not cross:
                    L.proj, L.e_wqkv = dev_proj(wqkv, 256)
            elif split:
                if cross:
                    L.wq, L.e_wq = dev_mat(m.q_proj.weight)
                else:
                    L.wqkv, L.e_wqkv = dev_mat(wqkv)
            else:
                L.wqkv, L.wq, L.wkv = dev_f32(wqkv), dev_f32(m.q_proj.weight), dev_f32(wkv)
                L.wm, L.w1, L.w2 = dev_f32(m.merge.weight), dev_f32(m.mlp[0].weight), dev_f32(m.mlp[2].weight)
            ex = scales.layer_exps(m, in_q, in_kv) if fp16_split else {}
            L.e_xq, L.e_xkv, L.e_k, L.e_v = ex.get("e_xq", 0), ex.get("e_xkv", 0), ex.get("e_k", 0), ex.get("e_v", 0)
            wq_next = None
            if id(m) in next_cross:
                nxt = next_cross[id(m)]
                wq_next = mods[nxt].q_proj.weight
                ex.update(e_y=scales.exp_for(scales.ln_bound(*ins[nxt][0])), e_wq=scales.w_exp(wq_next))
            L.tail_exps = ops.tail_exps(**ex)
            L.tail_next_q = int(wq_next is not None)
            if split:
                img = ops.pack_tail(f32(m.merge.weight), f32(m.mlp[0].weight), f32(m.mlp[2].weight), split, L.tail_exps,
                                    Wq_next=None if wq_next is None else f32(wq_next))
                keep.append(img.data)
                L.tail = img.data_ptr()
            L.g1, L.b1 = dev_f32(m.norm1.weight), dev_f32(m.norm1.bias)
            L.g2, L.b2 = dev_f32(m.norm2.weight), dev_f32(m.norm2.bias)
        mt = _lib.ModelT()
        mt.n_self, mt.n_cross = self.self_layer_num, self.cross_layer_num
        mt.dim_t = dev_f32(pe_dim_t())
        mt.emb_w = dev_f32(self.embedding.weight[:, :, 0])
        mt.emb_b = dev_f32(self.embedding.bias)
        mt.pre_g, mt.pre_b = dev_f32(self.pre_norm.weight), dev_f32(self.pre_norm.bias)
        mt.layers_host = C.cast(layers, C.POINTER(_lib.LayerT))
        mt.stem_tgt_layers_host = C.cast(tgt_layers, C.POINTER(_lib.LayerT)) if tgt_mods else None
        mt.gemm_split = split
        c0w, c2w = self.coor_mlp[0].weight[:, :, 0], self.coor_mlp[2].weight[:, :, 0]
        (mt.c0_w, mt.e_c0w), mt.c0_b = dev_mat(c0w), dev_f32(self.coor_mlp[0].bias)
        (mt.c2_w, mt.e_c2w), mt.c2_b = dev_mat(c2w), dev_f32(self.coor_mlp[2].bias)
        mt.c4_w, mt.c4_b = dev_f32(self.coor_mlp[4].weight[:, :, 0]), dev_f32(self.coor_mlp[4].bias)
        if split and self.cross_layer_num > 0:
            cross = [m for i, m in enumerate(self.cross) if i % 2 == 1]
            stack = torch.cat([torch.cat([c.layer.k_proj.weight[:128], c.layer.v_proj.weight[:128], c.layer.k_proj.weight[128:],
                                          c.layer.v_proj.weight[128:]], dim=0) for c in cross], dim=0)
            if fp16_split:
                mt.proj_cross, mt.e_wkv_cross = dev_proj(stack, 0)
            else:
                mt.wkv_cross, mt.e_wkv_cross = dev_mat(stack)
            cross_L = [layers[self.self_layer_num + 2 * j + 1] for j in range(self.cross_layer_num)]
            mt.e_k_cross, mt.e_v_cross = min(L.e_k for L in cross_L), min(L.e_v for L in cross_L)
        if fp16_split:
            mt.e_c0x = scales.exp_for(scales.ln_bound(*coor_in))
            mt.e_c2x = scales.exp_for(scales.lin_bound(c0w, *coor_in, bias=self.coor_mlp[0].bias))
        event = torch.cuda.Event()
        event.record(torch.cuda.current_stream(dev))
        return _Pack(backend, sig, mt, (layers, tgt_layers), keep, event, {torch.cuda.current_stream(dev).cuda_stream})

    def forward_packed(self, batch: PackedBatch, return_feats: bool = False, trace=None, backend: Optional[str] = None):
        pk = self._pack_weights(backend)
        mt = pk.mt
        lib = _lib.load()
        dev = batch.xyz.device
        if ops._stream() not in pk.streams:
            torch.cuda.current_stream(dev).wait_event(pk.event)
            pk.streams.add(ops._stream())
        need = lib.scream_forward_workspace_bytes(batch.rows_src, batch.rows_total, batch.n_pairs, batch.max_chunks, mt.gemm_split,
                                                  mt.n_cross)
        if self._ws is None:
            self._ws = {}
        key = (dev, ops._stream())
        ws = self._ws.get(key)
        if ws is None or ws.numel() < need:
            ws = self._ws[key] = torch.empty(need, device=dev, dtype=torch.uint8)
        bt = _lib.BatchT()
        bt.n_pairs, bt.rows_src, bt.rows_total, bt.max_chunks = batch.n_pairs, batch.rows_src, batch.rows_total, batch.max_chunks
        bt.xyz, bt.center = ops._p(batch.xyz), ops._p(batch.center)
        bt.tile_cloud = ops._p(batch.tile_cloud, torch.int32)
        bt.cloud_row0 = ops._p(batch.cloud_row0, torch.int32)
        bt.cloud_len = ops._p(batch.cloud_len, torch.int32)
        src_pred = torch.empty(batch.rows_src, 3, device=dev, dtype=torch.float32)
        feats = torch.empty(batch.rows_src, D_MODEL, device=dev, dtype=torch.float32) if return_feats else None
        _lib.check(lib.scream_forward(C.byref(mt), C.byref(bt), ws.data_ptr(), ws.numel(),
                                      src_pred.data_ptr(), feats.data_ptr() if return_feats else None,
                                      trace, ops._stream()), "scream_forward")
        return (src_pred, feats) if return_feats else src_pred

    def forward_batch(self, srcs: Sequence[torch.Tensor], tgts: Sequence[torch.Tensor],
                      centers: Optional[Sequence[Optional[torch.Tensor]]] = None) -> List[torch.Tensor]:
        batch = PackedBatch.from_pairs(srcs, tgts, centers)
        return [t.clone() for t in batch.unpack_src(self.forward_packed(batch))]

    def train(self, mode: bool = True):
        if mode:
            self._check_train_backend(self.train_backend)
        super().train(mode)
        self._grad_train = bool(mode)
        return self

    def _trains(self) -> bool:
        return getattr(self, "_grad_train", False) and torch.is_grad_enabled()

    def forward_packed_train(self, batch: PackedBatch) -> torch.Tensor:
        if type(self) not in (PointTransformer, DEMTransformer):
            raise NotImplementedError("training is implemented for PointTransformer and DEMTransformer only")
        from . import train as _train
        return _train.apply(self, batch)

    def forward(self, src, tgt, src_center=None, s=1, get_imgs=False, get_transform=False, filter=None):
        if self._trains():
            return self._forward_train(src, tgt, src_center, s, get_imgs, get_transform, filter)
        with torch.no_grad():
            return self._forward_infer(src, tgt, src_center, s, get_imgs, get_transform, filter)

    def _forward_train(self, src, tgt, src_center, s, get_imgs, get_transform, filter):
        assert src.shape[0] == 1, "batch size must 1"
        assert tgt.shape[0] == 1, "batch size must 1"
        center = None if src_center is None else src_center.reshape(3)
        batch = PackedBatch.from_pairs([src[0].detach()], [tgt[0].detach()], [None if center is None else center.detach()])
        src_ = self.forward_packed_train(batch)[: src.shape[1]].unsqueeze(0)
        imgs = self.generator(src_[0], tgt[0].detach()) if get_imgs else None
        transform = None
        if get_transform:
            from .geometry import register_from_prediction
            with torch.no_grad():
                ref = tgt[0] if filter is None else filter[0]
                transform = register_from_prediction(src[0], src_[0].detach(), ref, float(s), 0.075)
        return src_, imgs, transform

    def _forward_infer(self, src, tgt, src_center=None, s=1, get_imgs=False, get_transform=False, filter=None):
        assert src.shape[0] == 1, "batch size must 1"
        assert tgt.shape[0] == 1, "batch size must 1"
        center = None if src_center is None else src_center.reshape(3)
        batch = PackedBatch.from_pairs([src[0]], [tgt[0]], [center])
        src_ = self.forward_packed(batch)[: src.shape[1]].unsqueeze(0).clone()
        imgs = self.generator(src_[0], tgt[0]) if get_imgs else None
        transform = None
        if get_transform:
            from .geometry import register_from_prediction
            ref = tgt[0] if filter is None else filter[0]
            transform = register_from_prediction(src[0], src_[0], ref, float(s), 0.075)
        return src_, imgs, transform

    def loss(self, src_pred, src_pcd, rot_gt, trans_gt):
        reg = (torch.matmul(rot_gt, src_pcd.permute([0, 2, 1])) + trans_gt).permute([0, 2, 1])
        return torch.mean(torch.sum(torch.abs(src_pred - reg), dim=-1), dim=1).mean(dim=0)


class DEMTransformer(PointTransformer):

    def __init__(self, d_model: int = 256, self_layer_num: int = 6, cross_layer_num: int = 6):
        nn.Module.__init__(self)
        if d_model != D_MODEL:
            raise NotImplementedError("the gfx950 kernels are built for d_model=256")
        self.embedding = nn.Conv1d(3, d_model, kernel_size=1, stride=1)
        self.pre_norm = nn.LayerNorm(d_model)
        self.self_layer_num = self_layer_num
        self.cross_layer_num = cross_layer_num
        self.stem_dsm = nn.ModuleList([_MHAParams(d_model) for _ in range(self_layer_num)])
        self.stem_dem = nn.ModuleList([_MHAParams(d_model) for _ in range(self_layer_num)])
        self.cross = nn.ModuleList()
        for _ in range(cross_layer_num):
            self.cross.append(_MHAParams(d_model))
            self.cross.append(_CrossParams(d_model))
        self.coor_mlp = nn.Sequential(nn.Conv1d(d_model, d_model, 1), nn.ReLU(), nn.Conv1d(d_model, d_model, 1),
                                      nn.ReLU(), nn.Conv1d(d_model, 3, 1))
        self.generator = RegistrationRender(rho=24, w=64, view="single")
        self._packs = {}
        self._ws = None

    def _layer_modules(self) -> List[_MHAParams]:
        mods = list(self.stem_dsm)
        for i, m in enumerate(self.cross):
            mods.append(m if i % 2 == 0 else m.layer)
        return mods

    def _stem_tgt_modules(self) -> Optional[List[_MHAParams]]:
        return list(self.stem_dem)

    def forward(self, dsm, dem_coarse, get_imgs=False):
        if self._trains():
            return self._forward_train(dsm, dem_coarse, get_imgs)
        with torch.no_grad():
            return self._forward_infer(dsm, dem_coarse, get_imgs)

    def _forward_train(self, dsm, dem_coarse, get_imgs=False):
        assert dsm.shape[0] == 1, "batch size must 1"
        assert dem_coarse.shape[0] == 1, "batch size must 1"
        zero = torch.zeros(3, device=dsm.device)
        batch = PackedBatch.from_pairs([dsm[0].detach()], [dem_coarse[0].detach()], [zero])
        dem_ = self.forward_packed_train(batch)[: dsm.shape[1]].unsqueeze(0)
        imgs = self.generator(dem_[0], dem_coarse[0].detach()) if get_imgs else None
        return dem_, imgs

    def _forward_infer(self, dsm, dem_coarse, get_imgs=False):
        assert dsm.shape[0] == 1, "batch size must 1"
        assert dem_coarse.shape[0] == 1, "batch size must 1"
        zero = torch.zeros(3, device=dsm.device)
        batch = PackedBatch.from_pairs([dsm[0]], [dem_coarse[0]], [zero])
        dem_ = self.forward_packed(batch)[: dsm.shape[1]].unsqueeze(0).clone()
        imgs = self.generator(dem_[0], dem_coarse[0]) if get_imgs else None
        return dem_, imgs

    def forward_batch(self, dsms, dems, centers=None):
        zero = torch.zeros(3, device=dsms[0].device)
        return super().forward_batch(dsms, dems, [zero] * len(dsms))

    def loss(self, dem_pred, dem):
        return torch.mean(torch.sum(torch.abs(dem_pred - dem), dim=-1), dim=1).mean(dim=0)
```

### scream_amd/ops.py

```python
from __future__ import annotations

import ctypes as C
import os
from dataclasses import dataclass
from typing import Optional, Tuple

import torch

from . import _lib, scales
from ._lib import SPLIT_BF3, SPLIT_H1, SPLIT_H2, check

EPI_NONE, EPI_ELU1, EPI_RELU, EPI_BIAS_RELU, EPI_RES_LN, EPI_QKV = 0, 1, 2, 3, 4, 5
ROW_TILE = 128
KV_CHUNK = 256
KV_ELEMS = 33 * 32
D_MODEL = 256


def _stream() -> int:
    return torch.cuda.current_stream().cuda_stream


def _p(t: Optional[torch.Tensor], dtype=torch.float32) -> Optional[int]:
    if t is None:
        return None
    if not t.is_cuda:
        raise _lib.ScreamHipError("scream_amd ops need tensors on the MI355X (got device %s); there is no CPU path" % t.device)
    if t.dtype != dtype:
        raise TypeError("expected %s, got %s" % (dtype, t.dtype))
    if not t.is_contiguous():
        raise ValueError("tensor must be contiguous")
    return t.data_ptr()


def gemm_f32(A: torch.Tensor, W: torch.Tensor, epilogue: int = EPI_NONE, n_act: int = 0,
             bias: Optional[torch.Tensor] = None, residual: Optional[torch.Tensor] = None,
             gamma: Optional[torch.Tensor] = None, beta: Optional[torch.Tensor] = None,
             out: Optional[torch.Tensor] = None) -> torch.Tensor:
    M, K = A.shape
    N = W.shape[0]
    assert W.shape[1] == K
    if out is None:
        out = torch.empty(M, N, device=A.device, dtype=torch.float32)
    lib = _lib.load()
    check(lib.scream_gemm_f32(_p(A), A.stride(0), _p(W), _p(out), out.stride(0), M, N, K, epilogue, n_act,
                              _p(bias), _p(residual), residual.stride(0) if residual is not None else 0,
                              _p(gamma), _p(beta), _stream()), "scream_gemm_f32")
    return out


@dataclass
class PackedW:
    data: torch.Tensor
    split: int
    w_exp: int
    N: int
    K: int
    row_l1: Optional[torch.Tensor] = None

    def data_ptr(self) -> int:
        return self.data.data_ptr()


@dataclass
class PackedTail:
    data: torch.Tensor
    split: int
    exps: _lib.TailExpsT
    next_q: bool = False

    def data_ptr(self) -> int:
        return self.data.data_ptr()


def default_split() -> int:
    return SPLIT_BF3 if os.environ.get("SCREAM_GEMM", "h2") == "x3" else SPLIT_H2


def pack_w(W: torch.Tensor, split: Optional[int] = None, w_exp: Optional[int] = None) -> PackedW:
    split = default_split() if split is None else split
    W = W.detach().to(torch.float32).contiguous()
    N, K = W.shape
    if split in (SPLIT_H2, SPLIT_H1) and w_exp is None:
        w_exp = scales.w_exp(W)
    w_exp = int(w_exp or 0)
    dt = torch.float16 if split in (SPLIT_H2, SPLIT_H1) else torch.bfloat16
    out = torch.empty(split, K // 32, N, 32, device=W.device, dtype=dt)
    check(_lib.load().scream_pack_w_split(_p(W), N, K, split, w_exp, _p(out, dt), _stream()), "scream_pack_w_split")
    return PackedW(out, split, w_exp, N, K, W.abs().sum(dim=1).cpu() if split != SPLIT_BF3 else None)


LAYOUT_A_FRAG, LAYOUT_C_FRAG = 1, 2


def act_layout(X: torch.Tensor, to_fragment: bool) -> torch.Tensor:
    M = X.shape[0]
    assert X.shape[1] == D_MODEL
    out = torch.empty_like(X)
    check(_lib.load().scream_act_layout(_p(X), _p(out), M, int(to_fragment), _stream()), "scream_act_layout")
    return out


def _a_exp(A: torch.Tensor, Wp, a_exp: Optional[int]) -> int:
    if Wp.split == SPLIT_BF3:
        return 0
    return scales.exp_for(A.abs().max().item()) if a_exp is None else int(a_exp)


def gemm_split(A: torch.Tensor, Wp: PackedW, epilogue: int = EPI_NONE, n_act: int = 0,
               bias: Optional[torch.Tensor] = None, residual: Optional[torch.Tensor] = None,
               gamma: Optional[torch.Tensor] = None, beta: Optional[torch.Tensor] = None,
               out: Optional[torch.Tensor] = None, layout: int = 0, a_exp: Optional[int] = None) -> torch.Tensor:
    M, K = A.shape
    assert K == Wp.K
    if out is None:
        out = torch.empty(M, Wp.N, device=A.device, dtype=torch.float32)
    check(_lib.load().scream_gemm_split_f32(_p(A), A.stride(0), Wp.data_ptr(), _p(out), out.stride(0), M, Wp.N, K,
                                            epilogue, n_act, _p(bias), _p(residual),
                                            residual.stride(0) if residual is not None else 0, _p(gamma), _p(beta), layout,
                                            Wp.split, _a_exp(A, Wp, a_exp), Wp.w_exp, _stream()),
          "scream_gemm_split_f32")
    return out


def tail_exps(**kw) -> _lib.TailExpsT:
    e = _lib.TailExpsT()
    for k in ("e_att", "e_wm", "e_m1", "e_w1", "e_h", "e_w2", "e_y", "e_wq", "e_q"):
        setattr(e, k, int(kw.get(k, 0)))
    return e


def pack_tail(Wm: torch.Tensor, W1: torch.Tensor, W2: torch.Tensor, split: Optional[int] = None,
              exps: Optional[_lib.TailExpsT] = None, Wq_next: Optional[torch.Tensor] = None) -> PackedTail:
    split = default_split() if split is None else split
    Wm, W1, W2 = (w.detach().to(torch.float32).contiguous() for w in (Wm, W1, W2))
    assert Wm.shape == (D_MODEL, D_MODEL) and W1.shape == (4 * D_MODEL, D_MODEL) and W2.shape == (D_MODEL, 4 * D_MODEL)
    if split != SPLIT_BF3 and exps is None:
        raise ValueError("pack_tail on an fp16 split needs the operand exponents (scream_amd/scales.py)")
    exps = exps if exps is not None else tail_exps()
    lib = _lib.load()
    if Wq_next is not None:
        Wq_next = Wq_next.detach().to(torch.float32).contiguous()
        assert Wq_next.shape == (D_MODEL, D_MODEL)
    nbytes = lib.scream_tail_image_bytes(split, int(Wq_next is not None))
    if nbytes < 0:
        raise _lib.ScreamHipError("scream_tail_image_bytes returned %d (a next-layer query projection needs an fp16 split)" % nbytes)
    out = torch.empty(nbytes, device=Wm.device, dtype=torch.uint8)
    check(lib.scream_pack_tail(_p(Wm), _p(W1), _p(W2), _p(Wq_next), split, C.byref(exps), _p(out, torch.uint8), _stream()), "scream_pack_tail")
    return PackedTail(out, split, exps, Wq_next is not None)


def kv_finalize_image(partial: torch.Tensor, cloud_row0, cloud_len, row_base: int, cloud_begin: int, n_kv: int,
                   n_clouds: int, out: Optional[torch.Tensor] = None, split: Optional[int] = None) -> torch.Tensor:
    split = default_split() if split is None else split
    lib = _lib.load()
    L = partial.shape[0] if partial.dim() == 4 else 1
    img = lib.scream_kv_image_bytes()
    if out is None:
        out = torch.zeros((L, n_clouds, img) if partial.dim() == 4 else (n_clouds, img), device=partial.device, dtype=torch.uint8)
    check(lib.scream_kv_finalize_image(_p(partial), _p(cloud_row0, torch.int32), _p(cloud_len, torch.int32), row_base,
                                    cloud_begin, n_kv, _p(out, torch.uint8), L, partial[0].numel() if L > 1 else 0,
                                    n_clouds * img if L > 1 else 0, split, _stream()), "scream_kv_finalize_image")
    return out


def layer_tail(Q: torch.Tensor, kv_image: torch.Tensor, tile_cloud, kv_cloud_offset: int, cloud_len, x: torch.Tensor,
               tail: PackedTail, g1, b1, g2, b2, out: Optional[torch.Tensor] = None,
               q_next: Optional[torch.Tensor] = None) -> torch.Tensor:
    M = x.shape[0]
    assert x.shape[1] == D_MODEL and (Q is None or x.shape == Q.shape)
    assert (q_next is not None) == tail.next_q, "q_next goes with an image that carries the next layer's query stages"
    if out is None:
        out = torch.empty(M, D_MODEL, device=x.device, dtype=torch.float32)
    check(_lib.load().scream_layer_tail_f32(_p(Q), _p(kv_image, torch.uint8), _p(tile_cloud, torch.int32),
                                            kv_cloud_offset, _p(cloud_len, torch.int32), _p(x),
                                            tail.data_ptr(), _p(g1), _p(b1), _p(g2), _p(b2), _p(out), _p(q_next),
                                            M, tail.split, C.byref(tail.exps), _stream()), "scream_layer_tail_f32")
    return out


def gemm_qkv(A: torch.Tensor, W, n_q: int, tile_cloud, cloud_row0, cloud_len, row_base: int, layout: int = 0,
             a_exp: Optional[int] = None, k_exp: Optional[int] = None, v_exp: Optional[int] = None):
    M, K = A.shape
    sp = isinstance(W, PackedW)
    N = W.N if sp else W.shape[0]
    Q = torch.empty(M, n_q, device=A.device, dtype=torch.float32) if n_q else None
    L = (N - n_q) // 512
    part = torch.empty((L, M // ROW_TILE, 8, KV_ELEMS) if L > 1 else (M // ROW_TILE, 8, KV_ELEMS), device=A.device, dtype=torch.float32)
    args = (_p(A), A.stride(0), W.data_ptr() if sp else _p(W), _p(Q), n_q, M, N, K, n_q,
            _p(tile_cloud, torch.int32), _p(cloud_row0, torch.int32), _p(cloud_len, torch.int32), row_base, _p(part))
    if sp:
        if W.split != SPLIT_BF3 and (k_exp is None or v_exp is None):
            amax = float(A.abs().max().item())
            rl = W.row_l1[n_q:].view(-1, 2, 128)
            k_exp = scales.exp_for(1.0 + amax * float(rl[:, 0].max())) if k_exp is None else k_exp
            v_exp = scales.exp_for(amax * float(rl[:, 1].max())) if v_exp is None else v_exp
        check(_lib.load().scream_gemm_qkv_split_f32(*args, layout, W.split, _a_exp(A, W, a_exp), W.w_exp, int(k_exp or 0),
                                                    int(v_exp or 0), _stream()),
              "scream_gemm_qkv_split_f32")
    else:
        assert layout == 0
        check(_lib.load().scream_gemm_qkv_f32(*args, _stream()), "scream_gemm_qkv")
    return Q, part


@dataclass
class PackedProj:
    data: torch.Tensor
    split: int
    w_exp: int
    N: int
    n_q: int
    row_l1: Optional[torch.Tensor] = None

    def data_ptr(self) -> int:
        return self.data.data_ptr()


def pack_proj(W: torch.Tensor, n_q: int, split: Optional[int] = None, w_exp: Optional[int] = None) -> PackedProj:
    split = SPLIT_H2 if split is None else split
    W = W.detach().to(torch.float32).contiguous()
    N, K = W.shape
    assert K == D_MODEL
    w_exp = scales.w_exp(W) if w_exp is None else int(w_exp)
    nbytes = _lib.load().scream_proj_image_bytes(N, split)
    if nbytes <= 0:
        raise _lib.ScreamHipError("scream_proj_image_bytes(%d, %d) = %d" % (N, split, nbytes))
    out = torch.empty(nbytes, device=W.device, dtype=torch.uint8)
    check(_lib.load().scream_pack_proj(_p(W), N, n_q, split, w_exp, _p(out, torch.uint8), _stream()), "scream_pack_proj")
    return PackedProj(out, split, w_exp, N, n_q, W.abs().sum(dim=1).cpu())


def proj_qkv(x_frag: torch.Tensor, P: PackedProj, tile_cloud, cloud_row0, cloud_len, row_base: int,
             a_exp: Optional[int] = None, k_exp: Optional[int] = None, v_exp: Optional[int] = None):
    M = x_frag.shape[0]
    Q = torch.empty(M, D_MODEL, device=x_frag.device, dtype=torch.float32) if P.n_q else None
    L = (P.N - P.n_q) // 512
    part = torch.empty((L, M // ROW_TILE, 8, KV_ELEMS) if L > 1 else (M // ROW_TILE, 8, KV_ELEMS), device=x_frag.device, dtype=torch.float32)
    if a_exp is None or k_exp is None or v_exp is None:
        amax = float(x_frag.abs().max().item())
        rl = P.row_l1[P.n_q:].view(-1, 2, 128)
        a_exp = scales.exp_for(amax) if a_exp is None else a_exp
        k_exp = scales.exp_for(1.0 + amax * float(rl[:, 0].max())) if k_exp is None else k_exp
        v_exp = scales.exp_for(amax * float(rl[:, 1].max())) if v_exp is None else v_exp
    check(_lib.load().scream_proj_qkv_f32(_p(x_frag), P.data_ptr(), _p(Q), M, P.N, P.n_q, _p(tile_cloud, torch.int32),
                                          _p(cloud_row0, torch.int32), _p(cloud_len, torch.int32), row_base, _p(part), P.split,
                                          int(a_exp), P.w_exp, int(k_exp), int(v_exp), _stream()), "scream_proj_qkv_f32")
    return Q, part


def kv_finalize(part, cloud_row0, cloud_len, row_base: int, cloud_begin: int, n_kv: int, n_clouds: int) -> torch.Tensor:
    kv = torch.zeros(n_clouds, 8, KV_ELEMS, device=part.device, dtype=torch.float32)
    check(_lib.load().scream_kv_finalize(_p(part), _p(cloud_row0, torch.int32), _p(cloud_len, torch.int32), row_base,
                                         cloud_begin, n_kv, _p(kv), _stream()), "scream_kv_finalize")
    return kv


def pe_embed_ln(xyz, tile_cloud, center, dim_t, emb_w, emb_b, gamma, beta, frag: bool = False) -> torch.Tensor:
    rows = xyz.shape[0]
    feats = torch.empty(rows, D_MODEL, device=xyz.device, dtype=torch.float32)
    lib = _lib.load()
    fn, name = (lib.scream_pe_embed_ln_frag, "scream_pe_embed_ln_frag") if frag else (lib.scream_pe_embed_ln, "scream_pe_embed_ln")
    check(fn(_p(xyz), _p(tile_cloud, torch.int32), _p(center), _p(dim_t), _p(emb_w),
             _p(emb_b), _p(gamma), _p(beta), _p(feats), rows, _stream()), name)
    return feats


def kv_reduce(Kf: torch.Tensor, Vf: torch.Tensor, ld: int, row_base: int, cloud_row0, cloud_len, cloud_begin: int,
              n_kv: int, max_chunks: int, n_clouds: int) -> torch.Tensor:
    dev = Kf.device
    partial = torch.empty(max(n_kv * max_chunks * 8 * KV_ELEMS, 1), device=dev, dtype=torch.float32)
    kv = torch.zeros(n_clouds, 8, KV_ELEMS, device=dev, dtype=torch.float32)
    for t in (Kf, Vf):
        if not t.is_cuda or t.dtype != torch.float32:
            raise TypeError("kv_reduce needs fp32 device tensors")
    check(_lib.load().scream_kv_reduce(Kf.data_ptr(), Vf.data_ptr(), ld, row_base, _p(cloud_row0, torch.int32),
                                       _p(cloud_len, torch.int32), cloud_begin, n_kv, max_chunks, _p(partial),
                                       _p(kv), _stream()), "scream_kv_reduce")
    return kv


def attn_apply(Qf: torch.Tensor, ldq: int, kv, tile_cloud, kv_cloud_offset: int, cloud_len, rows: int) -> torch.Tensor:
    out = torch.empty(rows, D_MODEL, device=kv.device, dtype=torch.float32)
    check(_lib.load().scream_attn_apply(Qf.data_ptr(), ldq, _p(kv), _p(tile_cloud, torch.int32), kv_cloud_offset,
                                        _p(cloud_len, torch.int32), _p(out), D_MODEL, rows, _stream()),
          "scream_attn_apply")
    return out


def coor_head(X: torch.Tensor, W: torch.Tensor, b: torch.Tensor) -> torch.Tensor:
    rows = X.shape[0]
    out = torch.empty(rows, 3, device=X.device, dtype=torch.float32)
    check(_lib.load().scream_coor_head(_p(X), _p(W), _p(b), _p(out), rows, _stream()), "scream_coor_head")
    return out


def nn_search(query: torch.Tensor, ref: torch.Tensor, q_row0, q_len, r_row0, r_len, s: torch.Tensor,
              max_q_len: int, max_r_len: int, thresh: float) -> Tuple[torch.Tensor, torch.Tensor, torch.Tensor]:
    dev = query.device
    qn, rn = query.shape[0], ref.shape[0]
    n_pairs = s.shape[0]
    ref_prep = torch.empty(max(rn, 1), 4, device=dev, dtype=torch.float32)
    keys = torch.empty(max(qn, 1), device=dev, dtype=torch.int64)
    idx = torch.empty(qn, device=dev, dtype=torch.int32)
    dmin = torch.empty(qn, device=dev, dtype=torch.float32)
    valid = torch.empty(qn, device=dev, dtype=torch.uint8)
    check(_lib.load().scream_nn_search(_p(query), _p(ref), _p(q_row0, torch.int32), _p(q_len, torch.int32),
                                       _p(r_row0, torch.int32), _p(r_len, torch.int32), _p(s), n_pairs, max_q_len,
                                       max_r_len, qn, rn, float(thresh), _p(ref_prep), _p(keys, torch.int64),
                                       _p(idx, torch.int32), _p(dmin), _p(valid, torch.uint8), _stream()),
          "scream_nn_search")
    return idx, dmin, valid


def render_workspace(n_pairs: int, n_views: int, w: int, src_rows_total: int, device) -> torch.Tensor:
    need = _lib.load().scream_render_workspace_bytes(n_pairs, n_views, w, src_rows_total)
    if need < 0:
        raise _lib.ScreamHipError("scream_render_workspace_bytes(%d, %d, %d, %d): invalid argument" % (n_pairs, n_views, w, src_rows_total))
    return torch.empty(max(need, 16), device=device, dtype=torch.uint8)


def render_depth(src: torch.Tensor, s_row0, s_len, tgt: torch.Tensor, t_row0, t_len, max_s_len: int, max_t_len: int,
                 rot: torch.Tensor, w: int, rho: float, workspace: Optional[torch.Tensor] = None) -> Tuple[torch.Tensor, torch.Tensor]:
    n_pairs, V = s_row0.shape[0], rot.shape[0]
    dev = src.device
    if workspace is None:
        workspace = render_workspace(n_pairs, V, w, src.shape[0], dev)
    imgs = torch.empty(n_pairs, V, 2, w, w, device=dev, dtype=torch.float32)
    argmax = torch.empty(n_pairs, V, 2, w, w, device=dev, dtype=torch.int32)
    check(_lib.load().scream_render_depth(_p(src), _p(s_row0, torch.int32), _p(s_len, torch.int32), _p(tgt), _p(t_row0, torch.int32),
                                          _p(t_len, torch.int32), n_pairs, int(max_s_len), int(max_t_len), src.shape[0],
                                          _p(rot.reshape(V, 9)), V, int(w), float(rho), _p(imgs), _p(argmax, torch.int32),
                                          _p(workspace, torch.uint8), workspace.numel(), _stream()), "scream_render_depth")
    return imgs, argmax


def render_depth_bwd(dimgs: torch.Tensor, argmax: torch.Tensor, src: torch.Tensor, s_row0, s_len, max_s_len: int,
                     rot: torch.Tensor, w: int, rho: float, workspace: torch.Tensor) -> torch.Tensor:
    n_pairs, V = s_row0.shape[0], rot.shape[0]
    dsrc = torch.zeros(src.shape[0], 3, device=src.device, dtype=torch.float32)
    check(_lib.load().scream_render_depth_bwd(_p(src), _p(s_row0, torch.int32), _p(s_len, torch.int32), n_pairs, int(max_s_len),
                                              src.shape[0], _p(rot.reshape(V, 9)), V, int(w), float(rho), _p(dimgs),
                                              _p(argmax, torch.int32), _p(workspace, torch.uint8), workspace.numel(), _p(dsrc),
                                              _stream()), "scream_render_depth_bwd")
    return dsrc


def voxel_down_sample_packed(xyz: torch.Tensor, row0: torch.Tensor, length: torch.Tensor, max_len: int, voxel: torch.Tensor,
                             want_counts: bool = False) -> Tuple[torch.Tensor, torch.Tensor, Optional[torch.Tensor]]:
    n_clouds, rows, dev = row0.shape[0], xyz.shape[0], xyz.device
    need = _lib.load().scream_voxel_workspace_bytes(rows, n_clouds)
    if need < 0:
        raise _lib.ScreamHipError("scream_voxel_workspace_bytes(%d, %d): invalid argument" % (rows, n_clouds))
    workspace = torch.empty(max(need, 16), device=dev, dtype=torch.uint8)
    out_xyz = torch.empty(max(rows, 1), 3, device=dev, dtype=torch.float32)
    out_len = torch.empty(max(n_clouds, 1), device=dev, dtype=torch.int32)
    out_count = torch.empty(max(rows, 1), device=dev, dtype=torch.int32) if want_counts else None
    xyz_p = _p(xyz) if rows else out_xyz.data_ptr()
    check(_lib.load().scream_voxel_down_sample(xyz_p, _p(row0, torch.int32), _p(length, torch.int32), n_clouds, int(max_len),
                                               _p(voxel, torch.float64), _p(out_xyz), _p(out_len, torch.int32),
                                               _p(out_count, torch.int32), _p(workspace, torch.uint8), workspace.numel(), _stream()),
          "scream_voxel_down_sample")
    return out_xyz[:rows], out_len[:n_clouds], (out_count[:rows] if want_counts else None)


def dsm_extract_packed(patch: torch.Tensor, p_row0: torch.Tensor, p_len: torch.Tensor, max_p_len: int, dem: torch.Tensor,
                       d_row0: torch.Tensor, d_len: torch.Tensor, max_d_len: int, radius: float) -> Tuple[torch.Tensor, torch.Tensor]:
    n_clouds, P, D, dev = p_row0.shape[0], patch.shape[0], dem.shape[0], dem.device
    lib = _lib.load()
    need = lib.scream_dsm_workspace_bytes(P, n_clouds, int(max_p_len))
    if need < 0:
        raise _lib.ScreamHipError("scream_dsm_workspace_bytes(%d, %d, %d): invalid argument" % (P, n_clouds, max_p_len))
    workspace = torch.empty(max(need, 16), device=dev, dtype=torch.uint8)
    out_xyz = torch.empty(max(D, 1), 3, device=dev, dtype=torch.float32)
    out_idx = torch.empty(max(D, 1), device=dev, dtype=torch.int32)
    patch_p = _p(patch) if P else _p(workspace, torch.uint8)
    dem_p = _p(dem) if D else out_xyz.data_ptr()
    check(lib.scream_dsm_extract(patch_p, _p(p_row0, torch.int32), _p(p_len, torch.int32), int(max_p_len), P, dem_p,
                                 _p(d_row0, torch.int32), _p(d_len, torch.int32), int(max_d_len), D, n_clouds, float(radius),
                                 _p(out_xyz), _p(out_idx, torch.int32), _p(workspace, torch.uint8), workspace.numel(), _stream()),
          "scream_dsm_extract")
    return out_xyz[:D], out_idx[:D]


def dsm_dem_assemble_packed(dsm: torch.Tensor, dem: torch.Tensor, row0: torch.Tensor, length: torch.Tensor,
                            max_len: int) -> Tuple[torch.Tensor, torch.Tensor]:
    n_clouds, rows, dev = row0.shape[0], dem.shape[0], dem.device
    out = torch.empty(max(rows, 1), 6, device=dev, dtype=torch.float32)
    centre = torch.empty(max(n_clouds, 1), 3, device=dev, dtype=torch.float32)
    check(_lib.load().scream_dsm_dem_assemble(_p(dsm) if rows else out.data_ptr(), _p(dem) if rows else out.data_ptr(),
                                              _p(row0, torch.int32), _p(length, torch.int32), n_clouds, int(max_len), rows,
                                              _p(out), _p(centre), _stream()), "scream_dsm_dem_assemble")
    return out[:rows], centre[:n_clouds]


def kabsch_corr(src, ref, src_row0, src_len, ref_row0, idx, valid, s, c) -> Tuple[torch.Tensor, torch.Tensor]:
    n_pairs = s.shape[0]
    T = torch.empty(n_pairs, 4, 4, device=src.device, dtype=torch.float32)
    n_corr = torch.empty(n_pairs, device=src.device, dtype=torch.int32)
    check(_lib.load().scream_kabsch_corr(_p(src), _p(ref), _p(src_row0, torch.int32), _p(src_len, torch.int32),
                                         _p(ref_row0, torch.int32), _p(idx, torch.int32), _p(valid, torch.uint8),
                                         _p(s), _p(c), n_pairs, _p(T), _p(n_corr, torch.int32), _stream()),
          "scream_kabsch_corr")
    return T, n_corr


def rigid_transform_3d_dense(A: torch.Tensor, B: torch.Tensor, w: Optional[torch.Tensor], thr: float) -> torch.Tensor:
    bs, K = A.shape[0], A.shape[1]
    T = torch.empty(bs, 4, 4, device=A.device, dtype=torch.float32)
    check(_lib.load().scream_rigid_transform_3d(_p(A) if K else None, _p(B) if K else None, _p(w), float(thr), bs, K,
                                                _p(T), _stream()), "scream_rigid_transform_3d")
    return T


def transformation_error_batched(T_pred: torch.Tensor, T_gt: torch.Tensor) -> Tuple[torch.Tensor, torch.Tensor]:
    n = T_pred.shape[0]
    re = torch.empty(n, device=T_pred.device, dtype=torch.float32)
    te = torch.empty(n, device=T_pred.device, dtype=torch.float32)
    check(_lib.load().scream_transformation_error(_p(T_pred), _p(T_gt), n, _p(re), _p(te), _stream()),
          "scream_transformation_error")
    return re, te


def point_loss(src_pred: torch.Tensor, src: torch.Tensor, src_row0, src_len, rot: torch.Tensor, trans: torch.Tensor) -> torch.Tensor:
    B = rot.shape[0]
    out = torch.empty(B, device=src_pred.device, dtype=torch.float32)
    check(_lib.load().scream_point_loss(_p(src_pred), _p(src), _p(src_row0, torch.int32), _p(src_len, torch.int32),
                                        _p(rot.reshape(B, 9).contiguous()), _p(trans.reshape(B, 3).contiguous()), B, _p(out), _stream()),
          "scream_point_loss")
    return out


def icp_p2p(src, ref, src_row0, src_len, ref_row0, ref_len, s, c, T_init, max_src_len: int, max_ref_len: int,
            max_corr_dist: float, max_iter: int = 30, rel_fitness: float = 1e-6, rel_rmse: float = 1e-6):
    lib = _lib.load()
    n_pairs = s.shape[0]
    dev = src.device
    T = T_init.detach().clone().contiguous().float()
    fr = torch.empty(n_pairs, 2, device=dev, dtype=torch.float32)
    iters = torch.empty(n_pairs, device=dev, dtype=torch.int32)
    need = lib.scream_icp_workspace_bytes(src.shape[0], ref.shape[0], n_pairs)
    ws = torch.empty(need, device=dev, dtype=torch.uint8)
    check(lib.scream_icp_p2p(_p(src), _p(ref), _p(src_row0, torch.int32), _p(src_len, torch.int32),
                             _p(ref_row0, torch.int32), _p(ref_len, torch.int32), _p(s), _p(c), n_pairs, max_src_len,
                             max_ref_len, src.shape[0], ref.shape[0], float(max_corr_dist), int(max_iter),
                             float(rel_fitness), float(rel_rmse), _p(T), _p(fr), _p(iters, torch.int32),
                             ws.data_ptr(), need, _stream()), "scream_icp_p2p")
    return T, fr, iters


ICP_ASYNC_ITERS = 64


class IcpRun:

    def __init__(self, src, ref, src_row0, src_len, ref_row0, ref_len, s, c, T_init, max_src_len: int, max_ref_len: int,
                 max_corr_dist: float, max_iter: int, rel_fitness: float = 1e-6, rel_rmse: float = 1e-6):
        self.lib = _lib.load()
        n = s.shape[0]
        dev = src.device
        self.n, self.max_iter, self.next_it = n, int(max_iter), 0
        self.T = T_init.detach().clone().contiguous().float()
        self.fr = torch.empty(n, 2, device=dev, dtype=torch.float32)
        self.iters = torch.empty(n, device=dev, dtype=torch.int32)
        self.flags = torch.zeros(n, device=dev, dtype=torch.int32)
        self.flags_host = torch.zeros(n, dtype=torch.int32, pin_memory=True)
        need = self.lib.scream_icp_workspace_bytes(src.shape[0], ref.shape[0], n)
        self.ws = torch.empty(need, device=dev, dtype=torch.uint8)
        self._keep = (src, ref, src_row0, src_len, ref_row0, ref_len, s, c)
        self._args = (_p(src), _p(ref), _p(src_row0, torch.int32), _p(src_len, torch.int32), _p(ref_row0, torch.int32),
                      _p(ref_len, torch.int32), _p(s), _p(c), n, int(max_src_len), int(max_ref_len), src.shape[0], ref.shape[0],
                      float(max_corr_dist), int(max_iter), float(rel_fitness), float(rel_rmse), _p(self.T), _p(self.fr),
                      _p(self.iters, torch.int32))
        self.event = None

    @property
    def launches_left(self) -> int:
        return self.max_iter + 2 - self.next_it

    def advance(self, n_launches: int) -> None:
        end = min(self.next_it + int(n_launches), self.max_iter + 2)
        check(self.lib.scream_icp_p2p_range(*self._args, self.next_it, end, _p(self.flags, torch.int32), self.ws.data_ptr(),
                                            self.ws.numel(), _stream()), "scream_icp_p2p_range")
        self.next_it = end
        self.flags_host.copy_(self.flags, non_blocking=True)
        self.event = torch.cuda.Event()
        self.event.record(torch.cuda.current_stream(self.T.device))

    def all_stopped(self) -> bool:
        self.event.synchronize()
        return self.launches_left == 0 or bool(self.flags_host.all())
```

### scream_amd/scales.py

```python
from __future__ import annotations

import math
from typing import Dict, Optional

import torch

TOP = 2.0 ** 15
E_MIN, E_MAX = -24, 24


class ScaleRangeError(ValueError):
    """No power-of-two scale inside the kernels' checked range keeps |x| 2^e <= 2^15 for this operand: the fp16 x 2 split cannot
    carry these weights.  PointTransformer falls back to gemm_backend 'x3' (bf16 x 3, scale free) when it sees this."""


def exp_for(bound: float) -> int:
    b = float(bound)
    if not math.isfinite(b):
        raise ScaleRangeError("non-finite weights: no fp16 operand scale exists (use gemm_backend='x3')")
    if b <= 0.0:
        return E_MAX
    e = math.floor(math.log2(TOP / b))
    while b * 2.0 ** e > TOP:
        e -= 1
    if e < E_MIN:
        raise ScaleRangeError("operand bound %.3g needs the exponent %d < %d: outside the range the fp16 x 2 kernels were checked "
                              "for (use gemm_backend='x3')" % (b, e, E_MIN))
    return min(E_MAX, e)


def w_exp(W: torch.Tensor) -> int:
    return exp_for(W.detach().double().abs().max().item())


def ln_bound(gamma: torch.Tensor, beta: torch.Tensor) -> float:
    return (16.0 * gamma.detach().double().abs() + beta.detach().double().abs()).max().item()


def lin_bound(W: torch.Tensor, gamma: torch.Tensor, beta: torch.Tensor, bias: Optional[torch.Tensor] = None) -> float:
    W, g, b = W.detach().double(), gamma.detach().double(), beta.detach().double()
    out = 16.0 * (W * g).norm(dim=1) + (W @ b).abs()
    if bias is not None:
        out = out + bias.detach().double().abs()
    return out.max().item()


def tail_exps(Wm, W1, W2, g1, b1, v_bound: float, q_bound: float) -> Dict[str, int]:
    e_att = exp_for(v_bound)
    e_q = exp_for(1.0 + q_bound)
    e_m1 = exp_for(ln_bound(g1, b1))
    e_h = exp_for(lin_bound(W1, g1, b1))
    e_wm, e_w1, e_w2 = w_exp(Wm), w_exp(W1), w_exp(W2)
    e_att = min(e_att, 40 - e_wm)
    e_h = min(e_h, 40 - e_w2)
    for name, e in (("merge", e_wm + e_att), ("FFN-down", e_w2 + e_h)):
        if e < -44:
            raise ScaleRangeError("the %s accumulators would be in units of 2^%d: outside the range the layer-tail kernel's LayerNorm "
                                  "arithmetic was checked for (use gemm_backend='x3')" % (name, e))
    return {"e_att": e_att, "e_wm": e_wm, "e_m1": e_m1, "e_w1": e_w1, "e_h": e_h, "e_w2": e_w2, "e_q": e_q}


def layer_exps(m, in_q, in_kv) -> Dict[str, int]:
    ex = tail_exps(m.merge.weight, m.mlp[0].weight, m.mlp[2].weight, m.norm1.weight, m.norm1.bias, lin_bound(m.v_proj.weight, *in_kv),
                   lin_bound(m.q_proj.weight, *in_q))
    ex.update(e_xq=exp_for(ln_bound(*in_q)), e_xkv=exp_for(ln_bound(*in_kv)),
              e_k=exp_for(1.0 + lin_bound(m.k_proj.weight, *in_kv)), e_v=exp_for(lin_bound(m.v_proj.weight, *in_kv)))
    return ex
```

Before: 1876 pairs/s.

## Fold merge projection into per-cloud KV image for linear attention tail

Replaces the per-tile KV·Q MFMA product followed by the merge GEMM with a per-cloud precomputed image that already folds the merge weight into the KV state (Wm·KV). The tail kernel now scales Q by the key sum, normalizes, and streams the folded merge stages from the per-cloud image instead of the shared weight image. This removes the attention-apply MFMAs and the dynamic q-scale logic per tile. The cost is a larger per-cloud KV image (8 merge stages per cloud), a new merge-image kernel, and extra scale bounds (e_p) that may fail for some weights.

```diff
diff --git a/include/scream_hip.h b/include/scream_hip.h
--- a/include/scream_hip.h
+++ b/include/scream_hip.h
@@ -70,6 +70,7 @@
     int32_t e_att, e_wm, e_m1, e_w1, e_h, e_w2;
     int32_t e_y, e_wq;
     int32_t e_q;
+    int32_t e_p;
 } scream_tail_exps_t;
 int64_t scream_tail_image_bytes(int32_t split, int32_t with_next_q);
 int64_t scream_kv_image_bytes(void);
@@ -78,6 +79,12 @@
 int scream_kv_finalize_image(const float* kv_partial, const int32_t* cloud_row0, const int32_t* cloud_len,
                           int64_t row_base, int32_t cloud_begin, int32_t n_kv, void* kv_image, int32_t n_layers,
                           int64_t partial_layer_stride, int64_t image_layer_stride, int32_t split, void* stream);
+#define SCREAM_MAX_MERGE_LAYERS 16
+int scream_kv_merge_image(const float* kv_partial, const int32_t* cloud_row0, const int32_t* cloud_len, int64_t row_base,
+                          int32_t cloud_begin, int32_t n_kv, void* merge_image, int32_t n_layers, int64_t partial_layer_stride,
+                          int64_t image_layer_stride, const float* const* wm, const int32_t* e_p, int32_t split, void* stream);
+int scream_merge_image_from_sums(const void* kv_sums, int32_t n_clouds, const float* wm, int32_t e_p, void* merge_image,
+                                 int32_t split, void* stream);
 int scream_layer_tail_f32(const float* Q, const void* kv_image, const int32_t* tile_cloud,
                           int32_t kv_cloud_offset, const int32_t* cloud_len, const float* x,
                           const void* tail_image, const float* g1, const float* b1, const float* g2,
@@ -119,6 +126,7 @@
     scream_tail_exps_t tail_exps;
     int32_t tail_next_q;
     const void* proj;
+    const float* tail_wm;
 } scream_layer_t;
 
 typedef struct {
diff --git a/scream_amd/_lib.py b/scream_amd/_lib.py
--- a/scream_amd/_lib.py
+++ b/scream_amd/_lib.py
@@ -18,13 +18,13 @@
 
 
 class TailExpsT(C.Structure):
-    _fields_ = [(n, C.c_int32) for n in ("e_att", "e_wm", "e_m1", "e_w1", "e_h", "e_w2", "e_y", "e_wq", "e_q")]
+    _fields_ = [(n, C.c_int32) for n in ("e_att", "e_wm", "e_m1", "e_w1", "e_h", "e_w2", "e_y", "e_wq", "e_q", "e_p")]
 
 
 class LayerT(C.Structure):
     _fields_ = ([(n, C.c_void_p) for n in ("wqkv", "wq", "wkv", "wm", "w1", "w2", "g1", "b1", "g2", "b2", "tail")] +
                 [(n, C.c_int32) for n in ("e_xq", "e_xkv", "e_wqkv", "e_wq", "e_k", "e_v")] +
-                [("tail_exps", TailExpsT), ("tail_next_q", C.c_int32), ("proj", C.c_void_p)])
+                [("tail_exps", TailExpsT), ("tail_next_q", C.c_int32), ("proj", C.c_void_p), ("tail_wm", C.c_void_p)])
 
 
 class ModelT(C.Structure):
@@ -61,6 +61,8 @@
     "scream_kv_image_bytes": (C.c_int64, []),
     "scream_pack_tail": (C.c_int, [V, V, V, V, I32, C.POINTER(TailExpsT), V, V]),
     "scream_kv_finalize_image": (C.c_int, [V, V, V, I64, I32, I32, V, I32, I64, I64, I32, V]),
+    "scream_kv_merge_image": (C.c_int, [V, V, V, I64, I32, I32, V, I32, I64, I64, V, V, I32, V]),
+    "scream_merge_image_from_sums": (C.c_int, [V, I32, V, I32, V, I32, V]),
     "scream_layer_tail_f32": (C.c_int, [V, V, V, I32, V, V, V, V, V, V, V, V, V, I64, I32, C.POINTER(TailExpsT), V]),
     "scream_act_layout": (C.c_int, [V, V, I64, I32, V]),
     "scream_pe_embed_ln": (C.c_int, [V, V, V, V, V, V, V, V, V, I64, V]),
diff --git a/scream_amd/csrc/forward.hip b/scream_amd/csrc/forward.hip
--- a/scream_amd/csrc/forward.hip
+++ b/scream_amd/csrc/forward.hip
@@ -87,6 +87,7 @@
 
 bool layer_ok(const Ctx& c, const scream_layer_t& L, bool cross, bool cross_stage_self) {
     if ((L.tail != nullptr) != (c.split != 0)) return false;
+    if (c.split && !L.tail_wm) return false;
     if ((L.tail_next_q != 0) != (c.fp16() && cross_stage_self)) return false;
     if (c.fp16()) return cross || L.proj;
     if (c.split) return cross ? L.wq != nullptr : L.wqkv != nullptr;
@@ -151,7 +152,8 @@
     if (c.split) {
         {
             Scope sc(c.tr, TR_KV_REDUCE, rows, 0, 0, c.st);
-            TRY(scream_kv_finalize_image(kvp, b.cloud_row0, b.cloud_len, row0, cloud_begin, n_clouds, w.kvimg, 1, 0, 0, c.split, c.st));
+            TRY(scream_kv_merge_image(kvp, b.cloud_row0, b.cloud_len, row0, cloud_begin, n_clouds, w.kvimg, 1, 0, 0, &L.tail_wm,
+                                      &L.tail_exps.e_p, c.split, c.st));
         }
         Scope sc(c.tr, TR_TAIL_FUSED, rows, (L.tail_next_q ? 10 : 9) * D, D, c.st);
         return scream_layer_tail_f32(qr, w.kvimg, b.tile_cloud + row0 / SCREAM_ROW_TILE, 0, b.cloud_len, xr, L.tail, L.g1,
@@ -170,9 +172,16 @@
     TRY(gemm_qkv(c, x_tgt, m.wkv_cross, m.proj_cross, nullptr, rt, 2 * D * m.n_cross, 0, b, rs, w.kvp_cross, L0.e_xkv, m.e_wkv_cross, m.e_k_cross,
                  m.e_v_cross));
     Scope sc(c.tr, TR_KV_REDUCE, rt, 0, 0, c.st);
-    return scream_kv_finalize_image(w.kvp_cross, b.cloud_row0, b.cloud_len, rs, b.n_pairs, b.n_pairs,
+    SCREAM_REQUIRE(m.n_cross <= SCREAM_MAX_MERGE_LAYERS, SCREAM_EUNSUPPORTED);
+    const float* wm[SCREAM_MAX_MERGE_LAYERS];
+    int32_t e_p[SCREAM_MAX_MERGE_LAYERS];
+    for (int l = 0; l < m.n_cross; ++l) {
+        wm[l] = m.layers_host[m.n_self + 2 * l + 1].tail_wm;
+        e_p[l] = m.layers_host[m.n_self + 2 * l + 1].tail_exps.e_p;
+    }
+    return scream_kv_merge_image(w.kvp_cross, b.cloud_row0, b.cloud_len, rs, b.n_pairs, b.n_pairs,
                                  w.kvimg_cross - (int64_t)b.n_pairs * scream_kv_image_bytes(), m.n_cross, w.kvp_cross_stride,
-                                 w.kvimg_cross_stride, c.split, c.st);
+                                 w.kvimg_cross_stride, wm, e_p, c.split, c.st);
 }
 
 int mha_cross(const Ctx& c, const scream_layer_t& L, const scream_batch_t& b, const Workspace& w, const float* x_src,
diff --git a/scream_amd/csrc/tail_split.hip b/scream_amd/csrc/tail_split.hip
--- a/scream_amd/csrc/tail_split.hip
+++ b/scream_amd/csrc/tail_split.hip
@@ -10,22 +10,17 @@
 
 constexpr int TAIL_STAGES = 72;
 constexpr int NEXT_Q_STAGES = 8;
-constexpr int KV_PLANES_BYTES = 8 * 3 * 2 * 1024;
-constexpr int KV_IMAGE_BYTES = KV_PLANES_BYTES + 8 * 32 * 4;
-
-constexpr int KV_H2_HEAD_BYTES = 2 * 2 * 1024;
-constexpr int KV_H2_SCALE_OFF = 8 * KV_H2_HEAD_BYTES;
+constexpr int MERGE_STAGES = 8;
+constexpr int KV_IMAGE_BYTES = MERGE_STAGES * 3 * 16 * 1024 + 8 * 32 * 4;
+constexpr int KV_RED_ELEMS = (SCREAM_HEAD_DIM + 1) * SCREAM_HEAD_DIM;
+constexpr int E_B = 15;
+template <class SP> constexpr int ksum_off() { return MERGE_STAGES * SP::NP * 16 * 1024; }
 
 struct HeadOps {
-    f32x4 kv[6];
     f32x4 ks[4];
-    f32x4 sc;
 };
 
 struct TailScales {
-    float s_att;
-    int e_q;
-    int e_att;
     float c1;
     float eps1;
     float s_m1;
@@ -50,7 +45,6 @@
 __global__ __launch_bounds__(TT, 1) void tail_kernel(const float* __restrict__ Q,
                                                      const char* __restrict__ kvimg,
                                                      const int32_t* __restrict__ tile_cloud, int kv_cloud_offset,
-                                                     const int32_t* __restrict__ cloud_len,
                                                      const float* __restrict__ xres,
                                                      const char* __restrict__ Wimg,
                                                      const float* __restrict__ g1, const float* __restrict__ b1,
@@ -64,7 +58,6 @@
     constexpr int NP = SP::NP;
     constexpr int STAGE = stage_bytes<SP>();
     constexpr int PIECES = wave_pieces<SP>();
-    constexpr bool APPLY_H2 = SP::SCALED;
     constexpr int NV_MERGE = SP::NPROD >= 6 ? 6 : 8;
     constexpr int ND = SP::NPROD >= 6 ? 1 : T_DEFER_H2;
     constexpr int NG = 16 - ND;
@@ -81,32 +74,27 @@
     lnp[768 + tid] = b2[tid];
     const float eps1 = SP::SCALED ? sc.eps1 : 1e-5f, eps2 = SP::SCALED ? sc.eps2 : 1e-5f;
     const unsigned v_lane16 = lane * 16, v_half16 = half * 16;
-    auto dma_piece = [&](unsigned q, int u) {
+    auto dma_piece_from = [&](const char* img, unsigned q, int u) {
         const unsigned src = q % (unsigned)N_STAGES, slot = q % (unsigned)T_SLOTS;
-        const char* sbase = Wimg + (size_t)src * STAGE + (wave * PIECES + (u & ~3)) * 1024;
+        const char* sbase = img + (size_t)src * STAGE + (wave * PIECES + (u & ~3)) * 1024;
         dma_1k(sbase + v_lane16, smem + slot * STAGE + (wave * PIECES + (u & ~3)) * 1024, u & 3);
     };
+    auto dma_piece = [&](unsigned q, int u) { dma_piece_from(Wimg, q, u); };
+    int tile = blockIdx.x;
+    int64_t grp = ((int64_t)tile * 128 + wave * 32) * SCREAM_D_MODEL;
+    const char* kvc = tile < n_tiles ? kvimg + (size_t)(tile_cloud[tile] + kv_cloud_offset) * KV_IMAGE_BYTES : Wimg;
     unsigned q = 0;
 #pragma unroll
-    for (int u = 0; u < PIECES; ++u) dma_piece(0, u);
-#pragma unroll
-    for (int u = 0; u < PIECES; ++u) dma_piece(1, u);
+    for (int u = 0; u < PIECES; ++u) dma_piece_from(kvc, 0, u);
+#pragma unroll
+    for (int u = 0; u < PIECES; ++u) dma_piece_from(kvc, 1, u);
 
     auto seg_base = [&](const float* base, int64_t grp, int seg) { return base + grp + seg * 1024; };
     auto req_q = [&](f32x4 (&qb)[4], int64_t grp, int h) {
         ld_asm4<1024, true>(qb, seg_base(Q, grp, h), v_lane16);
     };
     auto req_head = [&](HeadOps& o, const char* kvc, int h) {
-        f32x4 (&kv4)[4] = reinterpret_cast<f32x4 (&)[4]>(o.kv[0]);
-        if (APPLY_H2) {
-            ld_asm4<1024>(kv4, kvc + h * KV_H2_HEAD_BYTES, v_lane16);
-            asm volatile("global_load_dwordx4 %0, %1, %2" : "=v"(o.sc) : "v"(v_half16), "s"(kvc + KV_H2_SCALE_OFF + 32 * h));
-        } else {
-            const char* kp = kvc + h * (3 * 2 * 1024);
-            ld_asm4<1024>(kv4, kp, v_lane16);
-            ld_asm2k(o.kv[4], o.kv[5], kp + 4 * 1024, v_lane16);
-        }
-        ld_asm4<32>(o.ks, kvc + KV_PLANES_BYTES + 128 * h, v_half16);
+        ld_asm4<32>(o.ks, kvc + ksum_off<SP>() + 128 * h, v_half16);
     };
     auto req_x = [&](f32x4 (&xs)[4], int64_t grp, int blk, auto second) {
         ld_asm4<1024, decltype(second)::value>(xs, seg_base(xres, grp, blk), v_lane16);
@@ -114,9 +102,6 @@
     auto pin_head = [&](HeadOps& o) {
 #pragma unroll
         for (int a = 0; a < 4; ++a) pin(o.ks[a]);
-#pragma unroll
-        for (int f = 0; f < (APPLY_H2 ? 4 : 6); ++f) pin(o.kv[f]);
-        if (APPLY_H2) pin(o.sc);
     };
     auto add_x4 = [&](f32x16& t, const f32x4 (&xs)[4], int a, float c) {
 #pragma unroll
@@ -135,75 +120,37 @@
     f32x4 qA[4], qB[4];
     f32x4 xs[4], xs2[4];
     V apA[2][NP], apB[2][NP];
-    f32x16 aT;
-    bf16x8 qp[2][3];
-    f16x8 qph[2][2];
     float Zs = 0.f;
-    int tq = 0;
-
-    auto apply_qscale = [&](const f32x4 (&qb)[4]) {
-        float m = 0.f;
-#pragma unroll
-        for (int a = 0; a < 4; ++a)
-#pragma unroll
-            for (int k = 0; k < 4; ++k) m = fmaxf(m, qb[a][k]);
-        m = fmaxf(m, __shfl_xor(m, 32));
-        const int hb = (int)(__float_as_uint(op.sc[0]) >> 23);
-        tq = min(max(14 - ((int)(__float_as_uint(m) >> 23) - 127), sc.e_q), min(127, sc.e_att + hb - 1));
+
+    constexpr float S_B = (float)(1 << E_B);
+    auto apply_ride = [&](f32x4 (&qb)[4], int g, V (&ap)[2][NP]) {
+        if (g == 0) {
+#pragma unroll
+            for (int a = 0; a < 4; ++a)
+#pragma unroll
+                for (int k = 0; k < 4; ++k) qb[a][k] = qb[a][k] * op.ks[a][k];
+        }
+        if (g == 1) {
+            float zp = 0.f;
+#pragma unroll
+            for (int a = 0; a < 4; ++a)
+#pragma unroll
+                for (int k = 0; k < 4; ++k) zp += qb[a][k];
+            zp += __shfl_xor(zp, 32);
+            Zs = 1.0f / (zp + 1e-6f);
+        }
+        if (g >= 4 && g < 12) {
+            const int k = g - 4, s2 = k >> 2, j = (2 * k) & 7;
+            const float b0 = qb[k >> 1][(2 * k) & 3] * Zs, b1 = qb[k >> 1][((2 * k) & 3) + 1] * Zs;
+            if constexpr (SP::SCALED) {
+                SP::split2s(b0, b1, S_B, j, ap[s2]);
+            } else {
+                SP::split1(b0, j, ap[s2]);
+                SP::split1(b1, j + 1, ap[s2]);
+            }
+        }
     };
-    auto apply_qsplit = [&](f32x4 (&qb)[4], int s2) {
-        const f32x4 lo = qb[2 * s2], hi = qb[2 * s2 + 1];
-        if (APPLY_H2) split8s<SplitH2>(lo, hi, __uint_as_float((uint32_t)(tq + 127) << 23), qph[s2]);
-        else split8<SplitBf3>(lo, hi, qp[s2]);
-    };
-    auto apply_mfma = [&](int s2) {
-        if (APPLY_H2) {
-            f16x8 w[2];
-#pragma unroll
-            for (int p = 0; p < 2; ++p) w[p] = __builtin_bit_cast(f16x8, op.kv[p * 2 + s2]);
-            mfma_group<SplitH2, -1>(aT, w, qph[s2], s2 == 0);
-        } else {
-            bf16x8 w[3];
-#pragma unroll
-            for (int p = 0; p < 3; ++p) w[p] = __builtin_bit_cast(bf16x8, op.kv[p * 2 + s2]);
-            mfma_group<SplitBf3, -1>(aT, w, qp[s2], s2 == 0);
-        }
-    };
-    auto apply_z = [&](f32x4 (&qb)[4]) {
-        float zp = 0.f;
-#pragma unroll
-        for (int a = 0; a < 4; ++a)
-#pragma unroll
-            for (int k = 0; k < 4; ++k) zp += qb[a][k] * op.ks[a][k];
-        zp += __shfl_xor(zp, 32);
-        Zs = 1.0f / (zp + 1e-6f);
-        if (APPLY_H2) Zs *= __uint_as_float((uint32_t)(sc.e_att - tq + (int)(__float_as_uint(op.sc[0]) >> 23)) << 23);
-        else if (SP::SCALED) Zs *= sc.s_att;
-    };
-    auto apply_split_pair = [&](int k, V (&ap)[2][NP], float S) {
-        const int s2 = k >> 2, j = (2 * k) & 7;
-#pragma unroll
-        for (int e = 0; e < 2; ++e) SP::split1((aT[2 * k + e] * Zs) * S, j + e, ap[s2]);
-    };
-    auto apply_ride = [&](f32x4 (&qb)[4], int g, V (&ap)[2][NP], float S) {
-        if (g == 0 && APPLY_H2) apply_qscale(qb);
-        if (g == 0) apply_qsplit(qb, 0);
-        if (g == 1) apply_qsplit(qb, 1);
-        if (g == 1) apply_mfma(0);
-        if (g == 2) apply_mfma(1);
-        if (g == 3) apply_z(qb);
-        if (g >= 4 && g < 12) apply_split_pair(g - 4, ap, S);
-    };
-
-    int tile = blockIdx.x;
-    int64_t grp = ((int64_t)tile * 128 + wave * 32) * SCREAM_D_MODEL;
-    const char* kvc = nullptr;
-    float S = 1.f;
-    if (tile < n_tiles) {
-        const int cl = tile_cloud[tile] + kv_cloud_offset;
-        kvc = kvimg + (size_t)cl * KV_IMAGE_BYTES;
-        S = (float)cloud_len[cl];
-    }
+
     if (tile < n_tiles) {
 #pragma unroll
         for (int h = 0; h < 2; ++h) {
@@ -213,7 +160,7 @@
             pin_x(qA);
             pin_head(op);
 #pragma unroll
-            for (int g = 0; g < 12; ++g) apply_ride(qA, g, h == 0 ? apA : apB, S);
+            for (int g = 0; g < 12; ++g) apply_ride(qA, g, h == 0 ? apA : apB);
         }
     }
 
@@ -242,13 +189,7 @@
         const int tile_next = tile + (int)gridDim.x;
         const bool has_next = tile_next < n_tiles;
         const int64_t grp_next = ((int64_t)(has_next ? tile_next : tile) * 128 + wave * 32) * SCREAM_D_MODEL;
-        const char* kvc_next = kvc;
-        float S_next = 1.f;
-        if (has_next) {
-            const int cl = tile_cloud[tile_next] + kv_cloud_offset;
-            kvc_next = kvimg + (size_t)cl * KV_IMAGE_BYTES;
-            S_next = (float)cloud_len[cl];
-        }
+        const char* kvc_next = has_next ? kvimg + (size_t)(tile_cloud[tile_next] + kv_cloud_offset) * KV_IMAGE_BYTES : kvc;
 
         auto stage_merge = [&](auto hh, V (&ap)[2][NP], V (&ap_next)[2][NP], f32x4 (&q_cons)[4], f32x4 (&q_req)[4], auto flush) {
             constexpr int h = decltype(hh)::value;
@@ -280,9 +221,10 @@
                     req_head(op, kvc, h + 2);
                     __builtin_amdgcn_sched_barrier(0);
                 }
-                if (g >= 4 && g - 4 < PIECES) dma_piece(q + 2, g - 4);
-                if (PIECES == 12 && g == 14) dma_piece(q + 2, 11);
-                if (RIDE) apply_ride(q_cons, g, ap_next, S);
+                const char* img2 = h + 2 < MERGE_STAGES ? kvc : Wimg;
+                if (g >= 4 && g - 4 < PIECES) dma_piece_from(img2, q + 2, g - 4);
+                if (PIECES == 12 && g == 14) dma_piece_from(img2, q + 2, 11);
+                if (RIDE) apply_ride(q_cons, g, ap_next);
                 if (h > 0) {
                     const int pc = xadd_slot(h, g, ND);
                     if (pc >= 0) add_x4(acc[h > 0 ? h - 1 : 0], x_prev, pc, sc.c1);
@@ -407,17 +349,18 @@
             ring_groups(flush, [&](int g, const V (&w)[NP]) __attribute__((always_inline)) {
                 if (RIDE == 2 && g == 4) {
                     __builtin_amdgcn_sched_barrier(0);
-                    req_q(qA, grp_next, 1);
+                    req_q(qB, grp_next, 1);
                     req_head(op, kvc_next, 1);
                     __builtin_amdgcn_sched_barrier(0);
                 }
+                const char* img2 = (RIDE > 0 && !NQ) ? kvc_next : Wimg;
                 if (RIDE == 2) {
-                    if (g >= 4 && g - 4 < PIECES) dma_piece(q + 2, g - 4);
-                    if (PIECES == 12 && g == 14) dma_piece(q + 2, 11);
+                    if (g >= 4 && g - 4 < PIECES) dma_piece_from(img2, q + 2, g - 4);
+                    if (PIECES == 12 && g == 14) dma_piece_from(img2, q + 2, 11);
                 } else {
-                    if (g < PIECES) dma_piece(q + 2, g);
-                }
-                if (RIDE == 2) apply_ride(qA, g, apA, S_next);
+                    if (g < PIECES) dma_piece_from(img2, q + 2, g);
+                }
+                if (RIDE == 2) apply_ride(qA, g, apA);
                 if (decltype(with_split)::value && (ND == 1 ? (g & 1) == 0 : (g >= T_RIDE0 && g < T_RIDE0 + 8))) split_pair(ND == 1 ? g >> 1 : g - T_RIDE0, hout);
                 mfma_group<SP>(acc[g >> 1], w, hin[g & 1], XADD == 0 && g >= 2 && (g & 1) == 0);
             });
@@ -456,9 +399,9 @@
         VM_WAIT(0);
         if (has_next) {
             pin_head(op);
-            pin_x(qA);
-#pragma unroll
-            for (int g = 0; g < 12; ++g) apply_ride(qA, g, apB, S_next);
+            pin_x(qB);
+#pragma unroll
+            for (int g = 0; g < 12; ++g) apply_ride(qB, g, apB);
         }
 
         V yp[NQ ? 16 : 1][NP];
@@ -538,7 +481,7 @@
                     if (g >= 8) {
 #pragma unroll
                         for (int u = (g - 8) * PP; u < (g - 7) * PP; ++u)
-                            if (u < PIECES) dma_piece(q + 2, u);
+                            if (u < PIECES) dma_piece_from(j + 2 < NEXT_Q_STAGES ? Wimg : kvc_next, q + 2, u);
                     }
                     mfma_group<SP, 8>(hq[j & 1], w, yp[g], g == 0);
                 });
@@ -560,7 +503,6 @@
         tile = tile_next;
         grp = ((int64_t)tile_next * 128 + wave * 32) * SCREAM_D_MODEL;
         kvc = kvc_next;
-        S = S_next;
     }
     VM_WAIT(0);
 }
@@ -638,88 +580,102 @@
 
 constexpr int KVF_THREADS = 320;
 
-template <bool H2>
-__global__ __launch_bounds__(KVF_THREADS) void kv_finalize_image_kernel(const float* __restrict__ partial,
-                                                                      const int32_t* __restrict__ cloud_row0,
-                                                                      const int32_t* __restrict__ cloud_len, int64_t row_base,
-                                                                      int cloud_begin, char* __restrict__ kvimg,
-                                                                      int64_t partial_layer_stride, int64_t image_layer_stride) {
-    constexpr int KV_ELEMS = (SCREAM_HEAD_DIM + 1) * SCREAM_HEAD_DIM;
-    static_assert(KV_ELEMS % 4 == 0 && KV_ELEMS / 4 <= KVF_THREADS, "");
-    __shared__ float wmax[KVF_THREADS / 64];
+__device__ __forceinline__ f32x4 kv_sum_tiles(const float* __restrict__ p, int nt) {
+    f32x4 s8[16];
+#pragma unroll
+    for (int u = 0; u < 16; ++u) s8[u] = f32x4{0.f, 0.f, 0.f, 0.f};
+    for (int c = 0; c < nt; c += 16) {
+#pragma unroll
+        for (int u = 0; u < 16; ++u)
+            if (c + u < nt) s8[u] += *reinterpret_cast<const f32x4*>(p + (int64_t)(c + u) * SCREAM_NHEAD * KV_RED_ELEMS);
+    }
+#pragma unroll
+    for (int u = 0; u < 8; ++u) s8[u] += s8[u + 8];
+    return ((s8[0] + s8[1]) + (s8[2] + s8[3])) + ((s8[4] + s8[5]) + (s8[6] + s8[7]));
+}
+
+template <class SP>
+__device__ __forceinline__ void form_merge_stage(float* red, const float* __restrict__ Wm, float s_p, int h, char* __restrict__ img) {
+    for (int i = threadIdx.x; i < 32 * 32; i += KVF_THREADS) {
+        const float ks = red[32 * 32 + (i >> 5)];
+        red[i] = ks > 0.f ? red[i] / ks : 0.f;
+    }
+    if (threadIdx.x < 32) reinterpret_cast<float*>(img + ksum_off<SP>())[h * 32 + threadIdx.x] = red[32 * 32 + threadIdx.x];
+    __syncthreads();
+    typename SP::vec* out = reinterpret_cast<typename SP::vec*>(img) + (size_t)h * SP::NP * 16 * 64;
+    for (int t = threadIdx.x; t < 16 * 64; t += KVF_THREADS) {
+        const int lane = t & 63, frag = t >> 6, m = lane & 31, half = lane >> 5;
+        const float* wrow = Wm + (size_t)(32 * (frag >> 1) + m) * SCREAM_D_MODEL + 32 * h;
+        f32x4 w[8];
+#pragma unroll
+        for (int v4 = 0; v4 < 8; ++v4) w[v4] = ld4(wrow + 4 * v4);
+        typename SP::vec p[SP::NP];
+#pragma unroll
+        for (int j = 0; j < 8; ++j) {
+            const float* nrow = red + 32 * chunk_k(frag & 1, half, j);
+            float acc = 0.f;
+#pragma unroll
+            for (int v4 = 0; v4 < 8; ++v4) {
+                const f32x4 n4 = ld4(nrow + 4 * v4);
+#pragma unroll
+                for (int e = 0; e < 4; ++e) acc = __builtin_fmaf(w[v4][e], n4[e], acc);
+            }
+            SP::split1(SP::SCALED ? acc * s_p : acc, j, p);
+        }
+#pragma unroll
+        for (int pl = 0; pl < SP::NP; ++pl) out[(pl * 16 + frag) * 64 + lane] = p[pl];
+    }
+}
+
+struct MergeLayers {
+    const float* wm[SCREAM_MAX_MERGE_LAYERS];
+    float s_p[SCREAM_MAX_MERGE_LAYERS];
+};
+
+template <class SP>
+__global__ __launch_bounds__(KVF_THREADS) void merge_image_kernel(const float* __restrict__ partial, const int32_t* __restrict__ cloud_row0,
+                                                                  const int32_t* __restrict__ cloud_len, int64_t row_base, int cloud_begin,
+                                                                  char* __restrict__ kvimg, int64_t partial_layer_stride,
+                                                                  int64_t image_layer_stride, MergeLayers ml) {
+    static_assert(KV_RED_ELEMS % 4 == 0 && KV_RED_ELEMS / 4 <= KVF_THREADS, "");
+    __shared__ __attribute__((aligned(16))) float red[KV_RED_ELEMS];
     const int i4 = threadIdx.x;
-    const bool active = i4 < KV_ELEMS / 4;
     const int kvi = blockIdx.x / SCREAM_NHEAD, h = blockIdx.x % SCREAM_NHEAD;
     const int cloud = cloud_begin + kvi;
-    partial += (int64_t)blockIdx.y * partial_layer_stride;
-    kvimg += (int64_t)blockIdx.y * image_layer_stride;
     const int t0 = (int)((cloud_row0[cloud] - row_base) / SCREAM_ROW_TILE);
     const int nt = (cloud_len[cloud] + SCREAM_ROW_TILE - 1) / SCREAM_ROW_TILE;
-    const float* p = partial + ((int64_t)t0 * SCREAM_NHEAD + h) * KV_ELEMS + 4 * (active ? i4 : 0);
-    char* img = kvimg + (size_t)cloud * KV_IMAGE_BYTES;
-    const float S = (float)cloud_len[cloud];
-    f32x4 s8[16];
-#pragma unroll
-    for (int u = 0; u < 16; ++u) s8[u] = f32x4{0.f, 0.f, 0.f, 0.f};
-    if (active) {
-        for (int c = 0; c < nt; c += 16) {
-#pragma unroll
-            for (int u = 0; u < 16; ++u)
-                if (c + u < nt) s8[u] += *reinterpret_cast<const f32x4*>(p + (int64_t)(c + u) * SCREAM_NHEAD * KV_ELEMS);
-        }
-    }
-#pragma unroll
-    for (int u = 0; u < 8; ++u) s8[u] += s8[u + 8];
-    const f32x4 s4 = ((s8[0] + s8[1]) + (s8[2] + s8[3])) + ((s8[4] + s8[5]) + (s8[6] + s8[7]));
-    const bool is_kv = 4 * i4 < 32 * 32;
-    f32x4 x4;
-#pragma unroll
-    for (int e = 0; e < 4; ++e) x4[e] = s4[e] / S;
-    float scale = 1.f;
-    if (H2) {
-        float m = (active && is_kv) ? fmaxf(fmaxf(fabsf(x4[0]), fabsf(x4[1])), fmaxf(fabsf(x4[2]), fabsf(x4[3]))) : 0.f;
-#pragma unroll
-        for (int o = 32; o >= 1; o >>= 1) m = fmaxf(m, __shfl_xor(m, o));
-        if ((threadIdx.x & 63) == 0) wmax[threadIdx.x >> 6] = m;
-        __syncthreads();
-        m = wmax[0];
-#pragma unroll
-        for (int w = 1; w < KVF_THREADS / 64; ++w) m = fmaxf(m, wmax[w]);
-        const uint32_t mb = __float_as_uint(m);
-        int eh = 15 - ((int)(mb >> 23) - 127) - ((mb & 0x7fffffu) ? 1 : 0);
-        if (!(m >= 1.17549435e-38f) || eh > 40) eh = 40;
-        if (eh < -30) eh = -30;
-        scale = __uint_as_float((uint32_t)(eh + 127) << 23);
-        if (threadIdx.x < 8) reinterpret_cast<float*>(img + KV_H2_SCALE_OFF)[h * 8 + threadIdx.x] = __uint_as_float((uint32_t)(127 - eh) << 23);
-    }
-    if (!active) return;
-#pragma unroll
-    for (int e = 0; e < 4; ++e) {
-        const int i = 4 * i4 + e;
-        if (is_kv) {
-            const int d = i >> 5, v = i & 31;
-            const float x = x4[e];
-            const int s2 = d >> 4, hf = (d >> 2) & 1, j = 4 * ((d >> 3) & 1) + (d & 3);
-            if (H2) {
-                const _Float16 a = (_Float16)(x * scale);
-                const _Float16 b = (_Float16)__builtin_fmaf(x, scale, -(float)a);
-                _Float16* base = reinterpret_cast<_Float16*>(img) + ((size_t)(h * 2) * 2 + s2) * 512 + (v + 32 * hf) * 8 + j;
-                base[0] = a;
-                base[2 * 512] = b;
-            } else {
-                const __bf16 a = (__bf16)x;
-                const float r1 = x - (float)a;
-                const __bf16 b = (__bf16)r1;
-                const __bf16 cc = (__bf16)(r1 - (float)b);
-                __bf16* base = reinterpret_cast<__bf16*>(img) + ((size_t)(h * 3) * 2 + s2) * 512 + (v + 32 * hf) * 8 + j;
-                base[0] = a;
-                base[2 * 512] = b;
-                base[4 * 512] = cc;
-            }
-        } else {
-            reinterpret_cast<float*>(img + KV_PLANES_BYTES)[h * 32 + (i - 32 * 32)] = s4[e];
-        }
-    }
+    if (i4 < KV_RED_ELEMS / 4) {
+        const float* p = partial + (int64_t)blockIdx.y * partial_layer_stride + ((int64_t)t0 * SCREAM_NHEAD + h) * KV_RED_ELEMS + 4 * i4;
+        *reinterpret_cast<f32x4*>(red + 4 * i4) = kv_sum_tiles(p, nt);
+    }
+    __syncthreads();
+    form_merge_stage<SP>(red, ml.wm[blockIdx.y], ml.s_p[blockIdx.y], h, kvimg + (int64_t)blockIdx.y * image_layer_stride + (size_t)cloud * KV_IMAGE_BYTES);
+}
+
+__global__ __launch_bounds__(KVF_THREADS) void kv_sums_kernel(const float* __restrict__ partial, const int32_t* __restrict__ cloud_row0,
+                                                              const int32_t* __restrict__ cloud_len, int64_t row_base, int cloud_begin,
+                                                              char* __restrict__ kvimg, int64_t partial_layer_stride, int64_t image_layer_stride) {
+    const int i4 = threadIdx.x;
+    if (i4 >= KV_RED_ELEMS / 4) return;
+    const int kvi = blockIdx.x / SCREAM_NHEAD, h = blockIdx.x % SCREAM_NHEAD;
+    const int cloud = cloud_begin + kvi;
+    const int t0 = (int)((cloud_row0[cloud] - row_base) / SCREAM_ROW_TILE);
+    const int nt = (cloud_len[cloud] + SCREAM_ROW_TILE - 1) / SCREAM_ROW_TILE;
+    const float* p = partial + (int64_t)blockIdx.y * partial_layer_stride + ((int64_t)t0 * SCREAM_NHEAD + h) * KV_RED_ELEMS + 4 * i4;
+    float* out = reinterpret_cast<float*>(kvimg + (int64_t)blockIdx.y * image_layer_stride + (size_t)cloud * KV_IMAGE_BYTES) + h * KV_RED_ELEMS;
+    *reinterpret_cast<f32x4*>(out + 4 * i4) = kv_sum_tiles(p, nt);
+}
+
+template <class SP>
+__global__ __launch_bounds__(KVF_THREADS) void merge_image_from_sums_kernel(const char* __restrict__ sums, const float* __restrict__ Wm, float s_p,
+                                                                            char* __restrict__ kvimg) {
+    __shared__ __attribute__((aligned(16))) float red[KV_RED_ELEMS];
+    const int i4 = threadIdx.x;
+    const int cloud = blockIdx.x / SCREAM_NHEAD, h = blockIdx.x % SCREAM_NHEAD;
+    if (i4 < KV_RED_ELEMS / 4)
+        *reinterpret_cast<f32x4*>(red + 4 * i4) = ld4(reinterpret_cast<const float*>(sums + (size_t)cloud * KV_IMAGE_BYTES) + h * KV_RED_ELEMS + 4 * i4);
+    __syncthreads();
+    form_merge_stage<SP>(red, Wm, s_p, h, kvimg + (size_t)cloud * KV_IMAGE_BYTES);
 }
 
 bool split_ok(int32_t split) { return split == SCREAM_SPLIT_BF3 || split == SCREAM_SPLIT_H2 || split == SCREAM_SPLIT_H1; }
@@ -729,12 +685,9 @@
     const int es[6] = {ex->e_att, ex->e_wm, ex->e_m1, ex->e_w1, ex->e_h, ex->e_w2};
     for (int e : es)
         if (e < -40 || e > 40) return false;
-    const int e1 = ex->e_wm + ex->e_att, e2 = ex->e_w2 + ex->e_h, eh = ex->e_h - ex->e_w1 - ex->e_m1;
+    const int e1 = ex->e_p + E_B, e2 = ex->e_w2 + ex->e_h, eh = ex->e_h - ex->e_w1 - ex->e_m1;
     if (e1 < -44 || e1 > 44 || e2 < -44 || e2 > 44 || eh < -100 || eh > 100) return false;
-    if (ex->e_q < -40 || ex->e_q > 40) return false;
-    sc->s_att = exp2i(ex->e_att);
-    sc->e_q = ex->e_q;
-    sc->e_att = ex->e_att;
+    if (ex->e_q < -40 || ex->e_q > 40 || ex->e_p < -40 || ex->e_p > 40) return false;
     sc->c1 = exp2i(e1);
     sc->eps1 = 1e-5f * exp2i(2 * e1);
     sc->s_m1 = exp2i(ex->e_m1);
@@ -777,22 +730,72 @@
     return 0;
 }
 
-extern "C" int scream_kv_finalize_image(const float* kv_partial, const int32_t* cloud_row0, const int32_t* cloud_len,
-                                        int64_t row_base, int32_t cloud_begin, int32_t n_kv, void* kv_image, int32_t n_layers,
-                                        int64_t partial_layer_stride, int64_t image_layer_stride, int32_t split, void* stream) {
+namespace {
+int kv_image_args_ok(const void* kv_partial, const int32_t* cloud_row0, const int32_t* cloud_len, int64_t row_base, int32_t cloud_begin,
+                     int32_t n_kv, const void* kv_image, int32_t n_layers, int64_t partial_layer_stride, int64_t image_layer_stride, int32_t split) {
     SCREAM_REQUIRE(kv_partial && cloud_row0 && cloud_len && kv_image && split_ok(split), SCREAM_EINVAL);
     SCREAM_REQUIRE(n_kv >= 0 && cloud_begin >= 0 && row_base >= 0 && n_layers >= 1 && n_layers <= 65535, SCREAM_EINVAL);
     SCREAM_REQUIRE(n_layers == 1 || (partial_layer_stride > 0 && image_layer_stride > 0 && image_layer_stride % 16 == 0), SCREAM_EINVAL);
     SCREAM_REQUIRE(((reinterpret_cast<uintptr_t>(kv_image) | reinterpret_cast<uintptr_t>(kv_partial)) & 15) == 0 && partial_layer_stride % 4 == 0,
                    SCREAM_EINVAL);
+    return 0;
+}
+}
+
+extern "C" int scream_kv_finalize_image(const float* kv_partial, const int32_t* cloud_row0, const int32_t* cloud_len,
+                                        int64_t row_base, int32_t cloud_begin, int32_t n_kv, void* kv_image, int32_t n_layers,
+                                        int64_t partial_layer_stride, int64_t image_layer_stride, int32_t split, void* stream) {
+    if (int rc = kv_image_args_ok(kv_partial, cloud_row0, cloud_len, row_base, cloud_begin, n_kv, kv_image, n_layers, partial_layer_stride,
+                                  image_layer_stride, split))
+        return rc;
+    if (n_kv == 0) return 0;
+    kv_sums_kernel<<<dim3(n_kv * SCREAM_NHEAD, n_layers), dim3(KVF_THREADS), 0, as_stream(stream)>>>(
+        kv_partial, cloud_row0, cloud_len, row_base, cloud_begin, reinterpret_cast<char*>(kv_image), partial_layer_stride, image_layer_stride);
+    SCREAM_LAUNCH_CHECK();
+    return 0;
+}
+
+extern "C" int scream_kv_merge_image(const float* kv_partial, const int32_t* cloud_row0, const int32_t* cloud_len, int64_t row_base,
+                                     int32_t cloud_begin, int32_t n_kv, void* merge_image, int32_t n_layers, int64_t partial_layer_stride,
+                                     int64_t image_layer_stride, const float* const* wm, const int32_t* e_p, int32_t split, void* stream) {
+    if (int rc = kv_image_args_ok(kv_partial, cloud_row0, cloud_len, row_base, cloud_begin, n_kv, merge_image, n_layers, partial_layer_stride,
+                                  image_layer_stride, split))
+        return rc;
+    SCREAM_REQUIRE(wm && (e_p || split == SCREAM_SPLIT_BF3), SCREAM_EINVAL);
+    SCREAM_REQUIRE(n_layers <= SCREAM_MAX_MERGE_LAYERS, SCREAM_EUNSUPPORTED);
+    MergeLayers ml{};
+    for (int l = 0; l < n_layers; ++l) {
+        SCREAM_REQUIRE(wm[l] && (reinterpret_cast<uintptr_t>(wm[l]) & 15) == 0, SCREAM_EINVAL);
+        SCREAM_REQUIRE(split == SCREAM_SPLIT_BF3 || (e_p[l] >= -40 && e_p[l] <= 40), SCREAM_EINVAL);
+        ml.wm[l] = wm[l];
+        ml.s_p[l] = split == SCREAM_SPLIT_BF3 ? 1.f : exp2i(e_p[l]);
+    }
     if (n_kv == 0) return 0;
     const dim3 grid(n_kv * SCREAM_NHEAD, n_layers), block(KVF_THREADS);
-    if (split != SCREAM_SPLIT_BF3)
-        kv_finalize_image_kernel<true><<<grid, block, 0, as_stream(stream)>>>(kv_partial, cloud_row0, cloud_len, row_base, cloud_begin,
-                                                                              reinterpret_cast<char*>(kv_image), partial_layer_stride, image_layer_stride);
-    else
-        kv_finalize_image_kernel<false><<<grid, block, 0, as_stream(stream)>>>(kv_partial, cloud_row0, cloud_len, row_base, cloud_begin,
-                                                                               reinterpret_cast<char*>(kv_image), partial_layer_stride, image_layer_stride);
+    hipStream_t st = as_stream(stream);
+#define MI_ARGS kv_partial, cloud_row0, cloud_len, row_base, cloud_begin, reinterpret_cast<char*>(merge_image), partial_layer_stride, image_layer_stride, ml
+    if (split == SCREAM_SPLIT_H2) merge_image_kernel<SplitH2><<<grid, block, 0, st>>>(MI_ARGS);
+    else if (split == SCREAM_SPLIT_H1) merge_image_kernel<SplitH1><<<grid, block, 0, st>>>(MI_ARGS);
+    else merge_image_kernel<SplitBf3><<<grid, block, 0, st>>>(MI_ARGS);
+#undef MI_ARGS
+    SCREAM_LAUNCH_CHECK();
+    return 0;
+}
+
+extern "C" int scream_merge_image_from_sums(const void* kv_sums, int32_t n_clouds, const float* wm, int32_t e_p, void* merge_image,
+                                            int32_t split, void* stream) {
+    SCREAM_REQUIRE(kv_sums && wm && merge_image && kv_sums != merge_image && split_ok(split) && n_clouds >= 0, SCREAM_EINVAL);
+    SCREAM_REQUIRE(((reinterpret_cast<uintptr_t>(kv_sums) | reinterpret_cast<uintptr_t>(wm) | reinterpret_cast<uintptr_t>(merge_image)) & 15) == 0,
+                   SCREAM_EINVAL);
+    SCREAM_REQUIRE(split == SCREAM_SPLIT_BF3 || (e_p >= -40 && e_p <= 40), SCREAM_EINVAL);
+    if (n_clouds == 0) return 0;
+    const dim3 grid(n_clouds * SCREAM_NHEAD), block(KVF_THREADS);
+    hipStream_t st = as_stream(stream);
+    const char* src = reinterpret_cast<const char*>(kv_sums);
+    char* dst = reinterpret_cast<char*>(merge_image);
+    if (split == SCREAM_SPLIT_H2) merge_image_from_sums_kernel<SplitH2><<<grid, block, 0, st>>>(src, wm, exp2i(e_p), dst);
+    else if (split == SCREAM_SPLIT_H1) merge_image_from_sums_kernel<SplitH1><<<grid, block, 0, st>>>(src, wm, exp2i(e_p), dst);
+    else merge_image_from_sums_kernel<SplitBf3><<<grid, block, 0, st>>>(src, wm, 1.f, dst);
     SCREAM_LAUNCH_CHECK();
     return 0;
 }
@@ -800,9 +803,9 @@
 namespace {
 template <class SP, bool NQ>
 void launch_tail(unsigned grid, hipStream_t st, const float* Q, const void* kv_image, const int32_t* tile_cloud, int32_t kv_cloud_offset,
-                 const int32_t* cloud_len, const float* x, const void* tail_image, const float* g1, const float* b1, const float* g2,
+                 const float* x, const void* tail_image, const float* g1, const float* b1, const float* g2,
                  const float* b2, float* y, float* q_next, int tiles, const TailScales& sc) {
-    tail_kernel<SP, NQ><<<dim3(grid), dim3(TT), 0, st>>>(Q, reinterpret_cast<const char*>(kv_image), tile_cloud, kv_cloud_offset, cloud_len, x,
+    tail_kernel<SP, NQ><<<dim3(grid), dim3(TT), 0, st>>>(Q, reinterpret_cast<const char*>(kv_image), tile_cloud, kv_cloud_offset, x,
                                                      reinterpret_cast<const char*>(tail_image), g1, b1, g2, b2, y, q_next, tiles, sc);
 }
 }
@@ -820,14 +823,14 @@
                      reinterpret_cast<uintptr_t>(q_next)) & 15) == 0, SCREAM_EINVAL);
     SCREAM_REQUIRE(x != y, SCREAM_EINVAL);
     SCREAM_REQUIRE(!q_next || (split != SCREAM_SPLIT_BF3 && q_next != x && q_next != y), SCREAM_EINVAL);
-    TailScales sc{1.f, 0, 0, 1.f, 1e-5f, 1.f, 1.f, 1.f, 1e-5f, 1.f, 1.f};
+    TailScales sc{1.f, 1e-5f, 1.f, 1.f, 1.f, 1e-5f, 1.f, 1.f};
     if (split != SCREAM_SPLIT_BF3) SCREAM_REQUIRE(tail_scales(exps, &sc), SCREAM_EINVAL);
     const int64_t tiles = M / SCREAM_ROW_TILE;
     if (tiles == 0) return 0;
     SCREAM_REQUIRE(tiles < (1ll << 31), SCREAM_EUNSUPPORTED);
     const unsigned grid = tiles < T_MAX_GRID ? (unsigned)tiles : (unsigned)T_MAX_GRID;
     hipStream_t st = as_stream(stream);
-#define TAIL_ARGS grid, st, Q, kv_image, tile_cloud, kv_cloud_offset, cloud_len, x, tail_image, g1, b1, g2, b2, y, q_next, (int)tiles, sc
+#define TAIL_ARGS grid, st, Q, kv_image, tile_cloud, kv_cloud_offset, x, tail_image, g1, b1, g2, b2, y, q_next, (int)tiles, sc
     if (split == SCREAM_SPLIT_H2) {
         if (q_next) launch_tail<SplitH2, true>(TAIL_ARGS);
         else launch_tail<SplitH2, false>(TAIL_ARGS);
diff --git a/scream_amd/model.py b/scream_amd/model.py
--- a/scream_amd/model.py
+++ b/scream_amd/model.py
@@ -220,6 +220,7 @@
                                     Wq_next=None if wq_next is None else f32(wq_next))
                 keep.append(img.data)
                 L.tail = img.data_ptr()
+                L.tail_wm = dev_f32(m.merge.weight)
             L.g1, L.b1 = dev_f32(m.norm1.weight), dev_f32(m.norm1.bias)
             L.g2, L.b2 = dev_f32(m.norm2.weight), dev_f32(m.norm2.bias)
         mt = _lib.ModelT()
diff --git a/scream_amd/ops.py b/scream_amd/ops.py
--- a/scream_amd/ops.py
+++ b/scream_amd/ops.py
@@ -68,6 +68,7 @@
     split: int
     exps: _lib.TailExpsT
     next_q: bool = False
+    wm: Optional[torch.Tensor] = None
 
     def data_ptr(self) -> int:
         return self.data.data_ptr()
@@ -125,7 +126,7 @@
 
 def tail_exps(**kw) -> _lib.TailExpsT:
     e = _lib.TailExpsT()
-    for k in ("e_att", "e_wm", "e_m1", "e_w1", "e_h", "e_w2", "e_y", "e_wq", "e_q"):
+    for k in ("e_att", "e_wm", "e_m1", "e_w1", "e_h", "e_w2", "e_y", "e_wq", "e_q", "e_p"):
         setattr(e, k, int(kw.get(k, 0)))
     return e
 
@@ -147,7 +148,7 @@
         raise _lib.ScreamHipError("scream_tail_image_bytes returned %d (a next-layer query projection needs an fp16 split)" % nbytes)
     out = torch.empty(nbytes, device=Wm.device, dtype=torch.uint8)
     check(lib.scream_pack_tail(_p(Wm), _p(W1), _p(W2), _p(Wq_next), split, C.byref(exps), _p(out, torch.uint8), _stream()), "scream_pack_tail")
-    return PackedTail(out, split, exps, Wq_next is not None)
+    return PackedTail(out, split, exps, Wq_next is not None, Wm)
 
 
 def kv_finalize_image(partial: torch.Tensor, cloud_row0, cloud_len, row_base: int, cloud_begin: int, n_kv: int,
@@ -164,14 +165,44 @@
     return out
 
 
+def kv_merge_image(partial: torch.Tensor, cloud_row0, cloud_len, row_base: int, cloud_begin: int, n_kv: int, n_clouds: int, wm, e_p,
+                   split: Optional[int] = None, out: Optional[torch.Tensor] = None) -> torch.Tensor:
+    split = default_split() if split is None else split
+    lib = _lib.load()
+    L = partial.shape[0] if partial.dim() == 4 else 1
+    wms = [w.detach().to(torch.float32).contiguous() for w in (wm if partial.dim() == 4 else [wm])]
+    eps = [int(e) for e in (e_p if partial.dim() == 4 else [e_p])]
+    assert len(wms) == L and len(eps) == L
+    img = lib.scream_kv_image_bytes()
+    if out is None:
+        out = torch.zeros((L, n_clouds, img) if partial.dim() == 4 else (n_clouds, img), device=partial.device, dtype=torch.uint8)
+    check(lib.scream_kv_merge_image(_p(partial), _p(cloud_row0, torch.int32), _p(cloud_len, torch.int32), row_base, cloud_begin, n_kv,
+                                    _p(out, torch.uint8), L, partial[0].numel() if L > 1 else 0, n_clouds * img if L > 1 else 0,
+                                    (C.c_void_p * L)(*[_p(w) for w in wms]), (C.c_int32 * L)(*eps), split, _stream()), "scream_kv_merge_image")
+    return out
+
+
+def merge_image(kv_sums: torch.Tensor, tail: PackedTail, out: Optional[torch.Tensor] = None) -> torch.Tensor:
+    if tail.wm is None:
+        raise ValueError("this PackedTail does not hold the merge weight it was packed from")
+    if out is None:
+        out = torch.empty_like(kv_sums)
+    check(_lib.load().scream_merge_image_from_sums(_p(kv_sums, torch.uint8), kv_sums.shape[0], _p(tail.wm), int(tail.exps.e_p),
+                                                   _p(out, torch.uint8), tail.split, _stream()), "scream_merge_image_from_sums")
+    return out
+
+
 def layer_tail(Q: torch.Tensor, kv_image: torch.Tensor, tile_cloud, kv_cloud_offset: int, cloud_len, x: torch.Tensor,
                tail: PackedTail, g1, b1, g2, b2, out: Optional[torch.Tensor] = None,
-               q_next: Optional[torch.Tensor] = None) -> torch.Tensor:
+               q_next: Optional[torch.Tensor] = None, merged: bool = False) -> torch.Tensor:
     M = x.shape[0]
     assert x.shape[1] == D_MODEL and (Q is None or x.shape == Q.shape)
     assert (q_next is not None) == tail.next_q, "q_next goes with an image that carries the next layer's query stages"
     if out is None:
         out = torch.empty(M, D_MODEL, device=x.device, dtype=torch.float32)
+    if not merged:
+        assert kv_image.dim() == 2
+        kv_image = merge_image(kv_image, tail)
     check(_lib.load().scream_layer_tail_f32(_p(Q), _p(kv_image, torch.uint8), _p(tile_cloud, torch.int32),
                                             kv_cloud_offset, _p(cloud_len, torch.int32), _p(x),
                                             tail.data_ptr(), _p(g1), _p(b1), _p(g2), _p(b2), _p(out), _p(q_next),
diff --git a/scream_amd/scales.py b/scream_amd/scales.py
--- a/scream_amd/scales.py
+++ b/scream_amd/scales.py
@@ -45,24 +45,44 @@
     return out.max().item()
 
 
-def tail_exps(Wm, W1, W2, g1, b1, v_bound: float, q_bound: float) -> Dict[str, int]:
+E_B = 15
+
+
+def merge_fold_bound(Wm: torch.Tensor, v_bound: float) -> float:
+    W = Wm.detach().double().abs()
+    return float(v_bound) * W.reshape(W.shape[0], -1, 32).sum(dim=2).max().item()
+
+
+def merge_fold_lin_bound(Wm: torch.Tensor, Wv: torch.Tensor, gamma: torch.Tensor, beta: torch.Tensor) -> float:
+    Wm, Wv = Wm.detach().double(), Wv.detach().double()
+    M = torch.einsum("ohv,hvk->hok", Wm.reshape(Wm.shape[0], -1, 32), Wv.reshape(-1, 32, Wv.shape[1]))
+    return max(lin_bound(M[h], gamma, beta) for h in range(M.shape[0]))
+
+
+def tail_exps(Wm, W1, W2, g1, b1, v_bound: float, q_bound: float, p_bound: Optional[float] = None) -> Dict[str, int]:
     e_att = exp_for(v_bound)
+    try:
+        pb = merge_fold_bound(Wm, v_bound)
+        e_p = exp_for(pb if p_bound is None else min(pb, float(p_bound)))
+    except ScaleRangeError as e:
+        raise ScaleRangeError("the per-cloud merge weights (merge.weight applied to a mean of value rows): %s" % e) from None
     e_q = exp_for(1.0 + q_bound)
     e_m1 = exp_for(ln_bound(g1, b1))
     e_h = exp_for(lin_bound(W1, g1, b1))
     e_wm, e_w1, e_w2 = w_exp(Wm), w_exp(W1), w_exp(W2)
     e_att = min(e_att, 40 - e_wm)
     e_h = min(e_h, 40 - e_w2)
-    for name, e in (("merge", e_wm + e_att), ("FFN-down", e_w2 + e_h)):
+    e_p = min(e_p, 40 - E_B)
+    for name, e in (("merge", e_p + E_B), ("FFN-down", e_w2 + e_h)):
         if e < -44:
             raise ScaleRangeError("the %s accumulators would be in units of 2^%d: outside the range the layer-tail kernel's LayerNorm "
                                   "arithmetic was checked for (use gemm_backend='x3')" % (name, e))
-    return {"e_att": e_att, "e_wm": e_wm, "e_m1": e_m1, "e_w1": e_w1, "e_h": e_h, "e_w2": e_w2, "e_q": e_q}
+    return {"e_att": e_att, "e_wm": e_wm, "e_m1": e_m1, "e_w1": e_w1, "e_h": e_h, "e_w2": e_w2, "e_q": e_q, "e_p": e_p}
 
 
 def layer_exps(m, in_q, in_kv) -> Dict[str, int]:
     ex = tail_exps(m.merge.weight, m.mlp[0].weight, m.mlp[2].weight, m.norm1.weight, m.norm1.bias, lin_bound(m.v_proj.weight, *in_kv),
-                   lin_bound(m.q_proj.weight, *in_q))
+                   lin_bound(m.q_proj.weight, *in_q), merge_fold_lin_bound(m.merge.weight, m.v_proj.weight, *in_kv))
     ex.update(e_xq=exp_for(ln_bound(*in_q)), e_xkv=exp_for(ln_bound(*in_kv)),
               e_k=exp_for(1.0 + lin_bound(m.k_proj.weight, *in_kv)), e_v=exp_for(lin_bound(m.v_proj.weight, *in_kv)))
     return ex
```

Result: no change. 1875 pairs/s (-0.1%).
